# aweisberg/cassandra-accord

Hardware: AMD Instinct MI355X
Metric: txn-key conflict pairs resolved/sec (node) (higher is better)
Workload: dtype u32/u64 (integer); 1 GPU; config2: KeyDeps batch, 1M txns x 8 keys, zipf(0.99) over 1M keys, p_write 0.5, uncommitted window 10k, per-GPU CommandStore snapshot; key_distribution=zipf, keys_permuted=True, n_txn_per_gpu=1000000, pairs_per_gpu=8000000, dep_edges_per_gpu=35349420, parallelism=keyspace shards x1 (independent CommandStores)

## Files before the change

### cassandra-accord_amd/csrc/api.hip

```cpp
#include "dict.hpp"
#include <exception>
#include <thread>

namespace acc {
void keydeps_batch(acc_ctx *ctx, const acc_batch_in *in, acc_keydeps_view *view);
void keydeps_mixed(acc_ctx *ctx, const acc_range_batch_in *in, acc_keydeps_view *view, SharedDict *shared = nullptr);
void keydeps_merge(acc_ctx *ctx, const acc_merge_in *in, acc_merge_view *view);
void levelise(acc_ctx *ctx, const acc_graph_in *in, uint32_t *level, uint32_t *order, uint32_t *n_levels);
void rangedeps_batch(acc_ctx *ctx, const acc_range_batch_in *in, acc_rangedeps_view *view, const SharedDict *shared = nullptr);
void shard_pack(acc_ctx *ctx, const acc_batch_in *in, acc_frag_streams *out, bool ctx_alloc);
void shard_merge(acc_ctx *ctx, const acc_frag_recv *in, acc_merge_view *view);
void deps_merge(acc_ctx *ctx, const acc_deps_merge_in *in, acc_deps_merge_view *view);
void rmm_invert(acc_ctx *ctx, const acc_rmm_batch *in, acc_csr_view *out);
void rmm_slice(acc_ctx *ctx, const acc_rmm_batch *in, const acc_ranges_in *select, acc_slice_view *out);
void rangedeps_stab(acc_ctx *ctx, const acc_rmm_batch *rd, const acc_stab_in *q, acc_stab_view *out);
void rmm_without(acc_ctx *ctx, const acc_rmm_batch *in, const acc_ts_cols *txn, const acc_txn_sets *set_a,
                 const acc_txn_sets *set_b, acc_without_view *out);
void recovery_deps_reduce(acc_ctx *ctx, const acc_deps_merge_in *cw, const acc_deps_merge_in *anw, acc_recovery_deps_view *view);
void map_reduce_full(acc_ctx *ctx, const acc_batch_in *in, const acc_recovery_in *q, acc_keydeps_view *view);
void map_reduce_full_ranges(acc_ctx *ctx, const acc_range_cmds_in *c, const acc_recovery_ranges_in *q, acc_rangedeps_view *view);
void latest_deps_merge(acc_ctx *ctx, const acc_latest_in *in, acc_latest_view *view);
void deps_from_json(acc_ctx *ctx, const acc_json_in *in, acc_json_deps_view *view);
void deps_to_json(acc_ctx *ctx, const acc_json_out_in *in, acc_json_out *out);
void cfk_update(acc_ctx *ctx, acc_cfk *cfk, const acc_batch_in *in);
void cfk_apply(acc_ctx *ctx, const acc_cfk_snap *in, const acc_cfk_updates *up, acc_cfk_snap_view *view);
void cfk_snap_to_batch(acc_ctx *ctx, const acc_cfk_snap *in, acc_cfk_batch_view *view, bool trusted = false);
void max_conflicts(acc_ctx *ctx, const acc_conflicts_in *u, const acc_preaccept_in *q, acc_preaccept_out *out);
acc_maxconflicts *mc_new(int device, uint32_t end_inclusive);
void mc_free(acc_maxconflicts *m);
uint64_t mc_size(const acc_maxconflicts *m);
void mc_update(acc_ctx *ctx, acc_maxconflicts *m, const acc_conflicts_in *u);
void mc_get(acc_ctx *ctx, const acc_maxconflicts *m, const acc_preaccept_in *q, acc_preaccept_out *out);
void cfk_view(acc_cfk *cfk, acc_batch_in *out);
void cfk_apply_deps(acc_ctx *ctx, acc_cfk *cfk, const acc_cfk_updates *up);
void cfk_state(acc_cfk *cfk, acc_cfk_snap *out);
void cfk_missing(acc_cfk *cfk, acc_cfk_batch_view *out);
void cfk_free(acc_cfk *cfk);
void cfk_keydeps(acc_ctx *ctx, acc_cfk *cfk, const acc_cfk_queries *q, acc_keydeps_view *view);
acc_cfk *cfk_new(int device);
}

namespace {
int ctx_create(int device, const acc_opts *opts, acc_ctx **out_ctx);
void ctx_destroy(acc_ctx *ctx);
}

extern "C" {

const char *acc_version(void) { return "accord_amd 0.1 (gfx950)"; }

int acc_create(int device, const acc_opts *opts, acc_ctx **out_ctx) { return ctx_create(device, opts, out_ctx); }

void acc_destroy(acc_ctx *ctx) { ctx_destroy(ctx); }

}

namespace {

int ctx_create(int device, const acc_opts *opts, acc_ctx **out_ctx)
{
    if (!out_ctx) return ACC_E_ARG;
    *out_ctx = nullptr;
    acc_ctx *ctx = new (std::nothrow) acc_ctx();
    if (!ctx) return ACC_E_NOMEM;
    int rc = acc_guard(ctx, [&] {
        int count = 0;
        ACC_HIP(hipGetDeviceCount(&count));
        if (device < 0 || device >= count) acc::fail(ACC_E_ARG, "no such HIP device");
        ACC_HIP(hipSetDevice(device));
        ctx->device = device;
        if (opts) ctx->opts = *opts;
        ctx->flags = ctx->opts.flags;
        ACC_HIP(hipStreamCreateWithFlags(&ctx->stream, hipStreamNonBlocking));
        ACC_HIP(hipHostMalloc((void **)&ctx->pinned, acc_ctx::PINNED_WORDS * sizeof(uint64_t), hipHostMallocDefault));
    });
    if (rc != ACC_OK) {
        ctx_destroy(ctx);
        return rc;
    }
    *out_ctx = ctx;
    return ACC_OK;
}

void ctx_destroy(acc_ctx *ctx)
{
    if (!ctx) return;
    (void)hipSetDevice(ctx->device);
    if (ctx->stream) (void)hipStreamSynchronize(ctx->stream);
    for (auto &kv : ctx->bufs)
        if (kv.second.ptr) (void)hipFree(kv.second.ptr);
    for (void *p : ctx->graveyard) (void)hipFree(p);
    for (auto &p : ctx->pending) { (void)hipEventDestroy(p.start); (void)hipEventDestroy(p.stop); }
    for (auto e : ctx->event_pool) (void)hipEventDestroy(e);
    for (int i = 0; i < acc_ctx::NAUX; ++i) {
        if (ctx->aux[i]) { (void)hipStreamSynchronize(ctx->aux[i]); (void)hipStreamDestroy(ctx->aux[i]); }
        if (ctx->join_ev[i]) (void)hipEventDestroy(ctx->join_ev[i]);
    }
    if (ctx->fork_ev) (void)hipEventDestroy(ctx->fork_ev);
    if (ctx->pinned) (void)hipHostFree(ctx->pinned);
    if (ctx->stream) (void)hipStreamDestroy(ctx->stream);
    acc_ctx *child = ctx->child;
    delete ctx;
    ctx_destroy(child);
}

}

extern "C" {

const char *acc_last_error(const acc_ctx *ctx) { return ctx ? ctx->last_error.c_str() : "null context"; }

int acc_sync(acc_ctx *ctx)
{
    if (!ctx) return ACC_E_ARG;
    return acc_guard(ctx, [&] { ctx->sync(); });
}

void *acc_stream(acc_ctx *ctx) { return ctx ? (void *)ctx->stream : nullptr; }

int acc_keydeps_batch(acc_ctx *ctx, const acc_batch_in *in, acc_keydeps_view *out_view)
{
    if (!ctx) return ACC_E_ARG;
    return acc_guard(ctx, [&] {
        ACC_HIP(hipSetDevice(ctx->device));
        acc::keydeps_batch(ctx, in, out_view);
    });
}

int acc_keydeps_mixed(acc_ctx *ctx, const acc_range_batch_in *in, acc_keydeps_view *out_view)
{
    if (!ctx) return ACC_E_ARG;
    return acc_guard(ctx, [&] {
        ACC_HIP(hipSetDevice(ctx->device));
        acc::keydeps_mixed(ctx, in, out_view);
    });
}

int acc_map_reduce_full(acc_ctx *ctx, const acc_batch_in *snapshot, const acc_recovery_in *q, acc_keydeps_view *out_view)
{
    if (!ctx) return ACC_E_ARG;
    return acc_guard(ctx, [&] {
        ACC_HIP(hipSetDevice(ctx->device));
        acc::map_reduce_full(ctx, snapshot, q, out_view);
    });
}

int acc_map_reduce_full_ranges(acc_ctx *ctx, const acc_range_cmds_in *cmds, const acc_recovery_ranges_in *q,
                               acc_rangedeps_view *out_view)
{
    if (!ctx) return ACC_E_ARG;
    return acc_guard(ctx, [&] {
        ACC_HIP(hipSetDevice(ctx->device));
        acc::map_reduce_full_ranges(ctx, cmds, q, out_view);
    });
}

int acc_latest_deps_merge(acc_ctx *ctx, const acc_latest_in *in, acc_latest_view *out_view)
{
    if (!ctx) return ACC_E_ARG;
    return acc_guard(ctx, [&] {
        ACC_HIP(hipSetDevice(ctx->device));
        acc::latest_deps_merge(ctx, in, out_view);
    });
}

int acc_partial_deps_batch(acc_ctx *ctx, const acc_range_batch_in *in, acc_keydeps_view *key_view,
                           acc_rangedeps_view *range_view)
{
    if (!ctx) return ACC_E_ARG;
    return acc_guard(ctx, [&] {
        ACC_HIP(hipSetDevice(ctx->device));
        if (!key_view || !range_view) acc::fail(ACC_E_ARG, "null argument");
        const bool serial = (ctx->flags & ACC_OPT_PD_SERIAL) != 0;
        if (!ctx->child && !serial) {
            const acc_opts o = ctx->opts;
            const int rc = ctx_create(ctx->device, &o, &ctx->child);
            if (rc != ACC_OK) acc::fail(rc, "cannot create the RangeDeps half's context");
        }
        acc_ctx *const child = serial ? nullptr : ctx->child;
        acc::SharedDict sd;
        std::thread th;
        int rrc = ACC_OK;
        hipEvent_t ev = nullptr;
        struct Join {
            std::thread &t;
            hipEvent_t &e;
            ~Join() { if (t.joinable()) t.join(); if (e) (void)hipEventDestroy(e); }
        } join{ th, ev };
        if (child) {
            child->opts = ctx->opts;
            child->flags = ctx->flags;
            child->time_only = ctx->time_only;
            sd.ready = [&](const acc::SharedDict &d) {
                ACC_HIP(hipEventCreateWithFlags(&ev, hipEventDisableTiming));
                ACC_HIP(hipEventRecord(ev, ctx->stream));
                th = std::thread([&rrc, child, in, range_view, ev, d] {
                    rrc = acc_guard(child, [&] {
                        ACC_HIP(hipSetDevice(child->device));
                        ACC_HIP(hipStreamWaitEvent(child->stream, ev, 0));
                        acc::rangedeps_batch(child, in, range_view, &d);
                        child->sync();
                    });
                });
            };
        }
        acc::keydeps_mixed(ctx, in, key_view, &sd);
        if (th.joinable()) {
            th.join();
            if (rrc != ACC_OK) acc::fail(rrc, child->last_error.c_str());
            ctx->rd_view = child->rd_view;
            ctx->rd_valid = child->rd_valid;
            ctx->rd_ent_hint = child->rd_ent_hint;
            for (const auto &kv : child->stats) ctx->stat(kv.first.c_str(), kv.second);
            for (auto &sl : child->slots) {
                if (!sl.launches) continue;
                acc::TimingSlot &d = ctx->slots[ctx->slot(sl.name.c_str())];
                d.total_ms += sl.total_ms;
                d.launches += sl.launches;
                sl.total_ms = 0;
                sl.launches = 0;
            }
        } else {
            acc::rangedeps_batch(ctx, in, range_view, &sd);
        }
        ctx->kd_valid = true;
    });
}

int acc_deps_from_json(acc_ctx *ctx, const acc_json_in *in, acc_json_deps_view *out_view)
{
    if (!ctx) return ACC_E_ARG;
    return acc_guard(ctx, [&] {
        ACC_HIP(hipSetDevice(ctx->device));
        acc::deps_from_json(ctx, in, out_view);
    });
}

int acc_deps_to_json(acc_ctx *ctx, const acc_json_out_in *in, acc_json_out *out)
{
    if (!ctx) return ACC_E_ARG;
    return acc_guard(ctx, [&] {
        ACC_HIP(hipSetDevice(ctx->device));
        acc::deps_to_json(ctx, in, out);
    });
}

int acc_cfk_create(acc_ctx *ctx, acc_cfk **out)
{
    if (!ctx || !out) return ACC_E_ARG;
    *out = nullptr;
    return acc_guard(ctx, [&] { *out = acc::cfk_new(ctx->device); });
// ... 398 lines not shown
```

### cassandra-accord_amd/csrc/ctx.hpp

```cpp
#pragma once

#include <hip/hip_runtime.h>

#include <cstdint>
#include <cstdio>
#include <cstring>
#include <string>
#include <unordered_map>
#include <vector>

#include "../../include/accord_amd.h"

namespace acc {

struct Error {
    int code;
    std::string msg;
};

[[noreturn]] inline void fail(int code, const std::string &msg) { throw Error{code, msg}; }

#define ACC_HIP(expr)                                                                          \
    do {                                                                                       \
        hipError_t e_ = (expr);                                                                \
        if (e_ != hipSuccess)                                                                  \
            ::acc::fail(e_ == hipErrorOutOfMemory ? ACC_E_NOMEM : ACC_E_DEVICE,                \
                        std::string(#expr ": ") + hipGetErrorString(e_));                      \
    } while (0)

struct Buf {
    void *ptr = nullptr;
    size_t bytes = 0;
};

struct TimingSlot {
    std::string name;
    double total_ms = 0;
    uint64_t launches = 0;
};

struct PendingEvent {
    int slot;
    hipEvent_t start, stop;
};

}

struct acc_ctx {
    int device = 0;
    hipStream_t stream = nullptr;
    static constexpr int NAUX = 3;
    hipStream_t aux[NAUX] = {};
    hipEvent_t fork_ev = nullptr, join_ev[NAUX] = {};
    hipStream_t launch_stream = nullptr;
    size_t scan_cap = 0, scan_dirty[2] = {0, 0};
    int scan_par = 0;
    struct OsState {
        size_t cap = 0, dirty[2] = {0, 0};
        int par = 0;
    };
    std::unordered_map<std::string, OsState> os_state;
    uint32_t flags = 0;
    acc_opts opts{};
    std::string last_error;
    acc_ctx *child = nullptr;
    std::unordered_map<std::string, acc::Buf> bufs;
    std::vector<void *> graveyard;
    static constexpr size_t PINNED_WORDS = 1024, PINNED_SLOTS = 512;
    uint64_t *pinned = nullptr;
    std::vector<acc::TimingSlot> slots;
    std::unordered_map<std::string, int> slot_index;
    std::vector<acc::PendingEvent> pending;
    std::vector<hipEvent_t> event_pool;
    std::vector<std::string> time_only;
    bool timed(const char *name) const
    {
        if (!(flags & ACC_OPT_TIMING)) return false;
        if (time_only.empty()) return true;
        for (const auto &t : time_only)
            if (t == name) return true;
        return false;
    }
    std::vector<std::pair<std::string, uint64_t>> stats;
    void stat(const char *name, uint64_t value)
    {
        for (auto &kv : stats)
            if (kv.first == name) { kv.second = value; return; }
        stats.emplace_back(name, value);
    }
    acc_keydeps_view kd_view{};
    acc_merge_view merge_view{};
    acc_rangedeps_view rd_view{};
    acc_deps_merge_view dm_view{};
    bool dm_valid = false;
    uint64_t rd_ent_hint = 0;
    bool rd_valid = false;
    bool kd_valid = false;
    bool merge_valid = false;
    std::vector<uint64_t> latest_suff_off, latest_suff_s, latest_suff_e;

    std::string ns;

    template <class T>
    T *get(const char *name, size_t count)
    {
        return get_raw<T>(ns.empty() ? std::string(name) : ns + name, count);
    }
    template <class T>
    T *get_raw(const std::string &name, size_t count)
    {
        size_t bytes = count * sizeof(T);
        if (bytes == 0) bytes = 16;
        acc::Buf &b = bufs[name];
        if (b.bytes < bytes) {
            if (b.ptr) graveyard.push_back(b.ptr);
            b.ptr = nullptr;
            size_t want = bytes + (bytes < (4ull << 30) ? bytes / 2 : bytes / 8);
            ACC_HIP(hipMalloc(&b.ptr, want));
            b.bytes = want;
        }
        return static_cast<T *>(b.ptr);
    }

    void swap_buf(const char *name, void *&ptr, size_t &bytes)
    {
        acc::Buf &b = bufs[ns.empty() ? std::string(name) : ns + name];
        std::swap(b.ptr, ptr);
        std::swap(b.bytes, bytes);
    }

    const void *buf_ptr(const char *name) const
    {
        auto it = bufs.find(ns.empty() ? std::string(name) : ns + name);
        return it == bufs.end() ? nullptr : it->second.ptr;
    }

    hipEvent_t take_event()
    {
        if (!event_pool.empty()) {
            hipEvent_t e = event_pool.back();
            event_pool.pop_back();
            return e;
        }
        hipEvent_t e;
        ACC_HIP(hipEventCreate(&e));
        return e;
    }

    int slot(const char *name)
    {
        auto it = slot_index.find(name);
        if (it != slot_index.end()) return it->second;
        int i = (int)slots.size();
        slots.push_back({name, 0, 0});
        slot_index[name] = i;
        return i;
    }

    void resolve_timing()
    {
        for (auto &p : pending) {
            float ms = 0;
            ACC_HIP(hipEventElapsedTime(&ms, p.start, p.stop));
            slots[p.slot].total_ms += ms;
            slots[p.slot].launches += 1;
            event_pool.push_back(p.start);
            event_pool.push_back(p.stop);
        }
        pending.clear();
    }

    hipStream_t cur() const { return launch_stream ? launch_stream : stream; }

    void fork(int k)
    {
        if (!fork_ev) {
            ACC_HIP(hipEventCreateWithFlags(&fork_ev, hipEventDisableTiming));
            for (int i = 0; i < NAUX; ++i) {
                ACC_HIP(hipStreamCreateWithFlags(&aux[i], hipStreamNonBlocking));
                ACC_HIP(hipEventCreateWithFlags(&join_ev[i], hipEventDisableTiming));
            }
        }
        ACC_HIP(hipEventRecord(fork_ev, stream));
        for (int i = 0; i < k; ++i) ACC_HIP(hipStreamWaitEvent(aux[i], fork_ev, 0));
    }
    void join(int k)
    {
        for (int i = 0; i < k; ++i) {
            ACC_HIP(hipEventRecord(join_ev[i], aux[i]));
            ACC_HIP(hipStreamWaitEvent(stream, join_ev[i], 0));
        }
        launch_stream = nullptr;
    }

    void recover() noexcept
    {
        launch_stream = nullptr;
        for (int i = 0; i < NAUX; ++i)
            if (aux[i]) (void)hipStreamSynchronize(aux[i]);
        if (stream) (void)hipStreamSynchronize(stream);
    }

    void sync()
    {
        ACC_HIP(hipStreamSynchronize(stream));
        for (void *p : graveyard) ACC_HIP(hipFree(p));
        graveyard.clear();
        if (!pending.empty()) resolve_timing();
    }
};

namespace acc {

struct NsScope {
    acc_ctx *ctx;
    std::string saved;
    NsScope(acc_ctx *c, const char *prefix) : ctx(c), saved(c->ns) { ctx->ns = saved + prefix; }
    ~NsScope() { ctx->ns = saved; }
};

template <class K, class... Args>
inline void launch(acc_ctx *ctx, const char *name, K kernel, dim3 grid, dim3 block, size_t shmem, Args... args)
{
    if (grid.x == 0 || grid.y == 0 || grid.z == 0) return;
    PendingEvent pe{};
    const bool timed = ctx->timed(name);
    if (timed) {
        pe.slot = ctx->slot(name);
        pe.start = ctx->take_event();
        pe.stop = ctx->take_event();
        ACC_HIP(hipEventRecord(pe.start, ctx->cur()));
    }
    hipLaunchKernelGGL(kernel, grid, block, shmem, ctx->cur(), args...);
    ACC_HIP(hipGetLastError());
    if (timed) {
        ACC_HIP(hipEventRecord(pe.stop, ctx->cur()));
        ctx->pending.push_back(pe);
    }
}

inline unsigned grid_for(size_t n, unsigned per_block)
{
    size_t g = (n + per_block - 1) / per_block;
    return (unsigned)(g ? g : 1);
}

template <class T>
inline const T *stage_in(acc_ctx *ctx, const char *name, const T *src, size_t count, uint32_t mem)
{
    if (count == 0) return ctx->get<T>(name, 1);
    if (!src) fail(ACC_E_ARG, std::string("null input array: ") + name);
    if (mem == ACC_MEM_DEVICE) return src;
    T *d = ctx->get<T>(name, count);
    ACC_HIP(hipMemcpyAsync(d, src, count * sizeof(T), hipMemcpyHostToDevice, ctx->stream));
    return d;
}

}

template <class F>
inline int acc_guard(acc_ctx *ctx, F &&body)
{
    try {
        body();
        if (ctx) ctx->last_error.clear();
        return ACC_OK;
    } catch (const acc::Error &e) {
        if (ctx) { ctx->recover(); ctx->last_error = e.msg; }
        return e.code;
    } catch (const std::bad_alloc &) {
        if (ctx) { ctx->recover(); ctx->last_error = "host allocation failed"; }
        return ACC_E_NOMEM;
    } catch (...) {
        if (ctx) { ctx->recover(); ctx->last_error = "unknown failure"; }
        return ACC_E_STATE;
    }
}
```

### cassandra-accord_amd/csrc/dict.hpp

```cpp
#pragma once

#include "prims.hpp"
#include "ts.hpp"
#include <functional>

namespace acc {

struct Dictionary {
    uint32_t *rank = nullptr;
    uint32_t *txn_of_rank = nullptr;
    int rbits = 0;
    bool batch_sorted = false;
    bool fast = false;
    bool ties_pending = false;
    uint64_t hg[8] = {};
};

struct DenseRank {
    uint32_t *rank = nullptr;
    uint32_t *first = nullptr;
    const uint32_t *perm = nullptr;
    uint64_t *count_dev = nullptr;
    uint64_t count = 0;
};
DenseRank dense_rank(acc_ctx *ctx, const char *tag, size_t n, int nw, const uint64_t *const *words, const uint64_t *and_mask,
                     const uint64_t *xor_mask, bool want_first);

constexpr size_t PREP_G_WORDS = 8 + 64 * 8;
void prep_dictionary(acc_ctx *ctx, uint32_t n, size_t P, const uint64_t *tm, const uint64_t *tl, const int32_t *tn,
                     const uint64_t *em, const uint64_t *el, const int32_t *en, const uint8_t *status,
                     const uint32_t *key_off, const uint64_t *key_code, uint32_t *owner, uint64_t *g, Dictionary &out,
                     bool defer_ties = false);
void redo_general_dictionary(acc_ctx *ctx, uint32_t n, const uint64_t *tm, const uint64_t *tl, const int32_t *tn,
                             const uint64_t *em, const uint64_t *el, const int32_t *en, uint64_t *g, Dictionary &d);

enum : uint32_t {
    ERR_BAD_STATUS = 1u << 0,
    ERR_BAD_KIND = 1u << 1,
    ERR_LOCAL_ONLY = 1u << 2,
    ERR_KEYS_UNSORTED = 1u << 3,
    ERR_DUP_TXNID = 1u << 4,
    ERR_KEY_OFF = 1u << 5,
    ERR_KEY_TOTAL = 1u << 6,
};
void check_errors(uint64_t errs);

struct SharedDict {
    bool valid = false;
    Dictionary dict;
    const uint32_t *owner = nullptr;
    std::function<void(const SharedDict &)> ready;
};

}
```

### cassandra-accord_amd/csrc/dictionary.hip

```cpp
#include "dict.hpp"

namespace acc {

namespace {

constexpr int DMAXW = 3;

struct DWords {
    const uint64_t *w[DMAXW];
    uint64_t xor_mask[DMAXW];
    uint64_t and_mask[DMAXW];
};

__device__ __forceinline__ uint64_t dword(const DWords &d, int k, size_t i)
{
    return (d.w[k][i] & d.and_mask[k]) ^ d.xor_mask[k];
}

__global__ __launch_bounds__(BLOCK) void k_dict_masks(size_t n, DWords d, int nw, uint64_t *__restrict__ g)
{
    uint64_t m[DMAXW] = { 0, 0, 0 };
    uint64_t ref[DMAXW];
    for (int k = 0; k < nw; ++k) ref[k] = dword(d, k, 0);
    for (size_t i = (size_t)blockIdx.x * BLOCK + threadIdx.x; i < n; i += (size_t)gridDim.x * BLOCK)
// ... 6 lines not shown
        if (lane_id() == 0) part[threadIdx.x >> 6][k] = x;
    }
    __syncthreads();
    if (threadIdx.x < (unsigned)nw) {
        uint64_t x = 0;
        for (int q = 0; q < WAVES; ++q) x |= part[q][threadIdx.x];
        if (x) atomicOr((unsigned long long *)&g[threadIdx.x], (unsigned long long)x);
    }
}

struct DPlan {
    Runs r[DMAXW];
    int shift[DMAXW];
};

__global__ __launch_bounds__(BLOCK) void k_dict_compact(size_t n, DWords d, int nw, DPlan p, int sel, const uint32_t *__restrict__ perm,
                                                        uint64_t *__restrict__ out)
{
    const size_t i = (size_t)blockIdx.x * BLOCK + threadIdx.x;
    if (i >= n) return;
    const size_t src = perm ? perm[i] : i;
    if (sel >= 0) { out[i] = pext_runs(dword(d, sel, src), p.r[sel]); return; }
    uint64_t c = 0;
    for (int k = 0; k < nw; ++k)
        if (p.r[k].bits) c |= pext_runs(dword(d, k, src), p.r[k]) << p.shift[k];
    out[i] = c;
}

__global__ __launch_bounds__(BLOCK) void k_dict_flags(size_t n, const uint64_t *__restrict__ sorted_single, const uint32_t *__restrict__ perm,
                                                      DWords d, int nw, uint32_t *__restrict__ flag)
{
    const size_t i = (size_t)blockIdx.x * BLOCK + threadIdx.x;
    if (i >= n) return;
    uint32_t f = 1;
    if (i > 0) {
        if (sorted_single) f = sorted_single[i] != sorted_single[i - 1];
        else {
            const uint32_t a = perm[i], b = perm[i - 1];
            f = 0;
            for (int k = 0; k < nw; ++k) f |= dword(d, k, a) != dword(d, k, b);
        }
    }
    flag[i] = f;
}

__global__ __launch_bounds__(BLOCK) void k_dict_scatter(size_t n, const uint32_t *__restrict__ perm, const uint32_t *__restrict__ flag,
                                                        const uint32_t *__restrict__ incl, uint32_t *__restrict__ rank,
                                                        uint32_t *__restrict__ first, uint64_t *__restrict__ count)
{
    const size_t i = (size_t)blockIdx.x * BLOCK + threadIdx.x;
    if (i >= n) return;
    const uint32_t src = perm[i], r = incl[i] - 1;
    rank[src] = r;
    if (first && flag[i]) first[r] = src;
    if (i == n - 1) *count = incl[i];
}

}

DenseRank dense_rank(acc_ctx *ctx, const char *tag, size_t n, int nw, const uint64_t *const *words, const uint64_t *and_mask,
                     const uint64_t *xor_mask, bool want_first)
{
    if (nw < 1 || nw > DMAXW) fail(ACC_E_STATE, "internal: dense_rank supports 1..3 words");
    if (n >= 0xFFFFFFFFull) fail(ACC_E_CAP, "dictionary too large (>= 2^32 keys)");
    hipStream_t st = ctx->stream;
    char nm[64];
    auto name = [&](const char *s) { snprintf(nm, sizeof nm, "%s.%s", tag, s); return nm; };
    DenseRank out;
    out.rank = ctx->get<uint32_t>(name("rank"), n);
    out.first = want_first ? ctx->get<uint32_t>(name("first"), n) : nullptr;
    out.count_dev = ctx->get<uint64_t>(name("count"), 1);
    if (n == 0) {
        ACC_HIP(hipMemsetAsync(out.count_dev, 0, 8, st));
        out.count = 0;
        return out;
    }
    DWords d{};
    for (int k = 0; k < DMAXW; ++k) {
        d.w[k] = k < nw ? words[k] : nullptr;
        d.and_mask[k] = (k < nw && and_mask) ? and_mask[k] : ~0ull;
        d.xor_mask[k] = (k < nw && xor_mask) ? xor_mask[k] : 0ull;
    }
    uint64_t *g = ctx->get<uint64_t>(name("masks"), DMAXW);
    ACC_HIP(hipMemsetAsync(g, 0, DMAXW * 8, st));
    launch(ctx, "dict_masks", k_dict_masks, dim3(std::min<unsigned>(grid_for(n, BLOCK), 1024u)), dim3(BLOCK), 0, n, d, nw, g);
    ACC_HIP(hipMemcpyAsync(ctx->pinned + 32, g, DMAXW * 8, hipMemcpyDeviceToHost, st));
    ctx->sync();
    DPlan p{};
    int total = 0;
    for (int k = nw - 1; k >= 0; --k) {
        p.r[k] = make_runs(ctx->pinned[32 + k]);
        p.shift[k] = total;
        total += p.r[k].bits;
    }
    const unsigned gn = grid_for(n, BLOCK);
    uint32_t *flag = ctx->get<uint32_t>(name("flag"), n);
    uint32_t *incl = ctx->get<uint32_t>(name("incl"), n);
    const uint32_t *perm;
    if (total <= 64) {
        uint64_t *ck = ctx->get<uint64_t>(name("ckey"), n);
        launch(ctx, "dict_compact", k_dict_compact, dim3(gn), dim3(BLOCK), 0, n, d, nw, p, -1, (const uint32_t *)nullptr, ck);
        Sorted s = radix_sort(ctx, name("rs"), ck, nullptr, n, total);
        perm = s.vals;
        launch(ctx, "dict_flags", k_dict_flags, dim3(gn), dim3(BLOCK), 0, n, (const uint64_t *)s.keys, (const uint32_t *)nullptr,
               d, nw, flag);
    } else {
        uint64_t *wk = ctx->get<uint64_t>(name("wkey"), n);
        uint32_t *pb = ctx->get<uint32_t>(name("perm"), n);
        const uint32_t *cur = nullptr;
        for (int k = nw - 1; k >= 0; --k) {
            if (!p.r[k].bits) continue;
            launch(ctx, "dict_compact", k_dict_compact, dim3(gn), dim3(BLOCK), 0, n, d, nw, p, k, cur, wk);
            Sorted s = radix_sort(ctx, name("rs"), wk, cur, n, p.r[k].bits);
            ACC_HIP(hipMemcpyAsync(pb, s.vals, n * sizeof(uint32_t), hipMemcpyDeviceToDevice, st));
            cur = pb;
        }
        perm = cur;
        launch(ctx, "dict_flags", k_dict_flags, dim3(gn), dim3(BLOCK), 0, n, (const uint64_t *)nullptr, perm, d, nw, flag);
    }
    scan<uint32_t, OpAdd<uint32_t>>(ctx, flag, incl, n, false);
    launch(ctx, "dict_scatter", k_dict_scatter, dim3(gn), dim3(BLOCK), 0, n, perm, (const uint32_t *)flag, (const uint32_t *)incl,
           out.rank, out.first, out.count_dev);
    out.count = ~0ull;
    out.perm = perm;
    return out;
}


struct TsPlan {
    Runs r0, r1, r2;
    int b0, b1, b2;
};

template <int NW>
__device__ __forceinline__ void block_or_n(uint64_t (&v)[NW], uint64_t *dst)
{
    __shared__ uint64_t part[WAVES][NW];
#pragma unroll
    for (int w = 0; w < NW; ++w) {
        uint64_t x = v[w];
#pragma unroll
        for (int d = 32; d >= 1; d >>= 1) x |= shfl_idx(x, (int)(lane_id() ^ d));
        if (lane_id() == 0) part[threadIdx.x >> 6][w] = x;
    }
    __syncthreads();
    if (threadIdx.x < NW) {
        uint64_t x = 0;
#pragma unroll
        for (int q = 0; q < WAVES; ++q) x |= part[q][threadIdx.x];
        if (x) atomicOr((unsigned long long *)&dst[threadIdx.x], (unsigned long long)x);
    }
}

constexpr uint32_t PREP_SLOTS = 64;

__global__ __launch_bounds__(BLOCK) void k_prep_txn(uint32_t n, size_t P, const uint64_t *__restrict__ tm, const uint64_t *__restrict__ tl,
                                                    const int32_t *__restrict__ tn, const uint64_t *__restrict__ em,
                                                    const uint64_t *__restrict__ el, const int32_t *__restrict__ en,
                                                    const uint8_t *__restrict__ status, const uint32_t *__restrict__ key_off,
                                                    const uint64_t *__restrict__ key_code, uint32_t *__restrict__ owner,
                                                    uint32_t *__restrict__ bflag, uint64_t *__restrict__ g)
{
    __shared__ uint32_t ko[BLOCK + 1];
    const uint32_t tid = threadIdx.x;
    uint64_t m0 = 0, m1 = 0, m2 = 0, km = 0, errs = 0, unsorted = 0, ornk = 0;
    uint32_t differs = 0;
    const uint64_t r0 = tm[0], r1 = ts_w1(tl[0]), r2 = ts_w2(tn[0]);
    const uint64_t kref = P ? key_code[0] : 0;
    if (blockIdx.x == 0 && tid == 0 && key_off[n] != P) errs |= ERR_KEY_TOTAL;
    for (uint32_t t0 = blockIdx.x * BLOCK; t0 < n; t0 += gridDim.x * BLOCK) {
        const uint32_t t = t0 + tid;
        const uint32_t tcnt = min((uint32_t)BLOCK, n - t0);
        __syncthreads();
        if (tid < tcnt) ko[tid] = key_off[t];
        if (tid == 0) ko[tcnt] = key_off[t0 + tcnt];
        if (t < n) {
            const bool d = tm[t] != em[t] || ts_w1(tl[t]) != ts_w1(el[t]) || tn[t] != en[t];
            differs += d;
            bflag[t] = (uint32_t)d;
            m0 |= (tm[t] ^ r0) | (em[t] ^ r0);
            m1 |= (ts_w1(tl[t]) ^ r1) | (ts_w1(el[t]) ^ r1);
            m2 |= (ts_w2(tn[t]) ^ r2) | (ts_w2(en[t]) ^ r2);
            if (status[t] > 7) errs |= ERR_BAD_STATUS;
            uint32_t kind = (uint32_t)(tl[t] >> 1) & 7u;
            if (kind >= 6) errs |= ERR_BAD_KIND;
            else if (kind == 5) errs |= ERR_LOCAL_ONLY;
            if (t + 1 < n && ts_cmp(tm[t], tl[t], tn[t], tm[t + 1], tl[t + 1], tn[t + 1]) >= 0) unsorted = 1;
        }
        __syncthreads();
        const bool bad = tid < tcnt && ko[tid + 1] < ko[tid];
        if (bad) errs |= ERR_KEY_OFF;
        else if (tid < tcnt) ornk |= ko[tid + 1] - ko[tid];
        if (!__syncthreads_or(bad ? 1 : 0) && P) {
            const uint32_t a = (uint32_t)min((size_t)ko[0], P), b = (uint32_t)min((size_t)ko[tcnt], P);
            for (uint32_t j = a + tid; j < b; j += BLOCK) {
                uint32_t lo = 0, hi = tcnt;
                while (hi - lo > 1) { const uint32_t m = (lo + hi) >> 1; if (ko[m] <= j) lo = m; else hi = m; }
                owner[j] = t0 + lo;
                const uint64_t kc = key_code[j];
                km |= kc ^ kref;
                if (j > ko[lo] && key_code[j - 1] >= kc) errs |= ERR_KEYS_UNSORTED;
            }
        }
    }
    uint64_t *gs = g + 8 * (blockIdx.x % PREP_SLOTS);
    uint64_t v[7] = { m0, m1, m2, km, errs, unsorted, ornk };
    block_or_n<7>(v, gs);
    __shared__ uint32_t s_nd;
    if (tid == 0) s_nd = 0;
    __syncthreads();
    if (differs) atomicAdd(&s_nd, differs);
    __syncthreads();
    if (tid == 0 && s_nd) atomicAdd((unsigned long long *)&gs[7], (unsigned long long)s_nd);
}

__global__ __launch_bounds__(BLOCK) void k_b_compact(uint32_t n, const uint32_t *__restrict__ bflag, const uint32_t *__restrict__ bidx,
                                                     const uint64_t *__restrict__ em, const uint64_t *__restrict__ el,
                                                     const int32_t *__restrict__ en, const uint64_t *__restrict__ tm,
                                                     const uint64_t *__restrict__ tl, const int32_t *__restrict__ tn,
                                                     TsPlan plan, uint64_t *__restrict__ bkey, uint32_t *__restrict__ bsrc,
                                                     uint64_t *__restrict__ tkey)
{
    uint32_t t = blockIdx.x * BLOCK + threadIdx.x;
    if (t >= n) return;
    uint64_t c0 = pext_runs(tm[t], plan.r0), c1 = pext_runs(ts_w1(tl[t]), plan.r1), c2 = pext_runs(ts_w2(tn[t]), plan.r2);
    tkey[t] = (plan.b0 ? (c0 << (plan.b1 + plan.b2)) : 0) | (plan.b1 ? (c1 << plan.b2) : 0) | c2;
    if (bflag[t]) {
        c0 = pext_runs(em[t], plan.r0); c1 = pext_runs(ts_w1(el[t]), plan.r1); c2 = pext_runs(ts_w2(en[t]), plan.r2);
        uint32_t b = bidx[t];
        bkey[b] = (plan.b0 ? (c0 << (plan.b1 + plan.b2)) : 0) | (plan.b1 ? (c1 << plan.b2) : 0) | c2;
        bsrc[b] = t;
    }
}

__device__ __forceinline__ uint32_t lower_bound_u64(const uint64_t *a, uint32_t lo, uint32_t hi, uint64_t v)
{
    while (lo < hi) {
        uint32_t mid = (lo + hi) >> 1;
        if (a[mid] < v) lo = mid + 1; else hi = mid;
    }
    return lo;
}

__global__ __launch_bounds__(BLOCK) void k_rank_txn_sorted(uint32_t n, uint32_t nb, const uint64_t *__restrict__ tkey,
                                                           const uint64_t *__restrict__ sb, const uint32_t *__restrict__ bflag,
                                                           uint32_t *__restrict__ rank, uint32_t *__restrict__ txn_of_rank,
                                                           uint64_t *__restrict__ g)
{
    uint32_t t = blockIdx.x * BLOCK + threadIdx.x;
    uint64_t tie = 0;
    if (t < n) {
        uint32_t lb = lower_bound_u64(sb, 0, nb, tkey[t]);
        if (lb < nb && sb[lb] == tkey[t]) tie = 1;
        uint32_t r = t + lb;
        rank[t] = r;
        txn_of_rank[r] = t;
        if (!bflag[t]) rank[n + t] = r;
    }
    uint64_t v[1] = { tie };
    block_or_n<1>(v, g + 6);
}

__global__ __launch_bounds__(BLOCK) void k_rank_b_sorted(uint32_t n, uint32_t nb, const uint64_t *__restrict__ tkey,
                                                         const uint64_t *__restrict__ sb, const uint32_t *__restrict__ sperm,
                                                         const uint32_t *__restrict__ bsrc, uint32_t *__restrict__ rank,
                                                         uint64_t *__restrict__ g)
{
    uint32_t k = blockIdx.x * BLOCK + threadIdx.x;
    uint64_t tie = 0;
    if (k < nb) {
        if (k > 0 && sb[k] == sb[k - 1]) tie = 1;
        uint32_t t = bsrc[sperm[k]];
        rank[n + t] = k + lower_bound_u64(tkey, 0, n, sb[k]);
    }
    uint64_t v[1] = { tie };
    block_or_n<1>(v, g + 6);
}


__global__ __launch_bounds__(BLOCK) void k_ts_compact(uint32_t n, const uint64_t *__restrict__ tm, const uint64_t *__restrict__ tl,
                                                      const int32_t *__restrict__ tn, const uint64_t *__restrict__ em,
                                                      const uint64_t *__restrict__ el, const int32_t *__restrict__ en,
                                                      TsPlan plan, int word_sel, const uint32_t *__restrict__ perm,
                                                      uint64_t *__restrict__ out)
{
    size_t i = (size_t)blockIdx.x * BLOCK + threadIdx.x;
    if (i >= 2 * (size_t)n) return;
    size_t src = perm ? perm[i] : i;
    uint32_t t = (uint32_t)(src < n ? src : src - n);
    bool is_exec = src >= n;
    uint64_t w0 = is_exec ? em[t] : tm[t];
    uint64_t w1 = ts_w1(is_exec ? el[t] : tl[t]);
    uint64_t w2 = ts_w2(is_exec ? en[t] : tn[t]);
    uint64_t c0 = pext_runs(w0, plan.r0), c1 = pext_runs(w1, plan.r1), c2 = pext_runs(w2, plan.r2);
    uint64_t k;
    if (word_sel < 0) k = (plan.b0 ? (c0 << (plan.b1 + plan.b2)) : 0) | (plan.b1 ? (c1 << plan.b2) : 0) | c2;
    else k = word_sel == 0 ? c0 : word_sel == 1 ? c1 : c2;
    out[i] = k;
}

__global__ __launch_bounds__(BLOCK) void k_rank_flags(size_t m, const uint32_t *__restrict__ perm, const uint64_t *__restrict__ c0,
                                                      const uint64_t *__restrict__ c1, const uint64_t *__restrict__ c2,
                                                      const uint64_t *__restrict__ sorted_single, uint32_t *__restrict__ flag)
{
    size_t i = (size_t)blockIdx.x * BLOCK + threadIdx.x;
    if (i >= m) return;
    uint32_t f = 1;
    if (i > 0) {
        if (sorted_single) f = sorted_single[i] != sorted_single[i - 1];
        else {
            uint32_t a = perm[i], b = perm[i - 1];
            f = (c0[a] != c0[b]) || (c1[a] != c1[b]) || (c2[a] != c2[b]);
        }
    }
    flag[i] = f;
}

__global__ __launch_bounds__(BLOCK) void k_rank_scatter(size_t m, uint32_t n, const uint32_t *__restrict__ perm,
                                                        const uint32_t *__restrict__ incl, uint32_t *__restrict__ rank,
                                                        uint32_t *__restrict__ txn_of_rank)
{
    size_t i = (size_t)blockIdx.x * BLOCK + threadIdx.x;
    if (i >= m) return;
    uint32_t src = perm[i];
    uint32_t r = incl[i] - 1;
    rank[src] = r;
    if (src < n) txn_of_rank[r] = src;
}

__global__ __launch_bounds__(BLOCK) void k_dup_txn(uint32_t n, const uint32_t *__restrict__ rank, uint32_t *__restrict__ seen,
                                                   uint64_t *__restrict__ g)
{
    uint32_t t = blockIdx.x * BLOCK + threadIdx.x;
    uint64_t err = 0;
    if (t < n) {
        if (atomicAdd(&seen[rank[t]], 1u) != 0) err = ERR_DUP_TXNID;
    }
    uint64_t v[1] = { err };
    block_or_n<1>(v, g + 4);
}

__global__ __launch_bounds__(BLOCK) void k_exec_ties(uint32_t n, const uint32_t *__restrict__ rank, uint32_t *__restrict__ seen,
                                                     uint64_t *__restrict__ g)
{
    uint32_t t = blockIdx.x * BLOCK + threadIdx.x;
    uint64_t tie = 0;
    if (t < n && rank[n + t] != rank[t]) {
        if (atomicAdd(&seen[rank[n + t]], 1u) != 0) tie = 1;
    }
    uint64_t v[1] = { tie };
    block_or_n<1>(v, g + 6);
}


void check_errors(uint64_t errs)
{
    if (errs & ERR_KEY_TOTAL) fail(ACC_E_ARG, "key_off[n_txn] must equal n_pairs");
    if (errs & ERR_BAD_STATUS) fail(ACC_E_ARG, "invalid InternalStatus ordinal (> INVALID_OR_TRUNCATED)");
    if (errs & ERR_BAD_KIND) fail(ACC_E_ARG, "Kind.ofOrdinal: invalid kind ordinal in TxnId flags");
    if (errs & ERR_KEY_OFF) fail(ACC_E_ARG, "key_off must be non-decreasing");
    if (errs & ERR_KEYS_UNSORTED) fail(ACC_E_ARG, "keys of a txn must be sorted and unique (Keys.ofSortedUnique)");
    if (errs & ERR_DUP_TXNID) fail(ACC_E_ARG, "TxnIds of a batch must be distinct (CommandsForKey txns are sorted unique)");
    if (errs & ERR_LOCAL_ONLY) fail(ACC_E_STATE, "Kind.witnesses(): unhandled kind LocalOnly (AssertionError)");
}

static void general_ranks(acc_ctx *ctx, uint32_t n, const uint64_t *tm, const uint64_t *tl, const int32_t *tn,
                          const uint64_t *em, const uint64_t *el, const int32_t *en, const TsPlan &plan, uint64_t *g,
                          uint32_t *rank, uint32_t *txn_of_rank)
{
    hipStream_t st = ctx->stream;
    const size_t m = 2 * (size_t)n;
    uint32_t *flag = ctx->get<uint32_t>("rank_flag", m);
    uint32_t *incl = ctx->get<uint32_t>("rank_incl", m);
    const unsigned gm = grid_for(m, BLOCK);
    Sorted ts_sorted;
    if (plan.b0 + plan.b1 + plan.b2 <= 64) {
        uint64_t *ck = ctx->get<uint64_t>("ts_ckey", m);
        launch(ctx, "ts_compact", k_ts_compact, dim3(gm), dim3(BLOCK), 0, n, tm, tl, tn, em, el, en, plan, -1,
               (const uint32_t *)nullptr, ck);
        ts_sorted = radix_sort(ctx, "rs_ts", ck, nullptr, m, plan.b0 + plan.b1 + plan.b2);
        launch(ctx, "rank_flags", k_rank_flags, dim3(gm), dim3(BLOCK), 0, m, (const uint32_t *)ts_sorted.vals,
               (const uint64_t *)nullptr, (const uint64_t *)nullptr, (const uint64_t *)nullptr,
               (const uint64_t *)ts_sorted.keys, flag);
    } else {
        uint64_t *c[3] = { ctx->get<uint64_t>("ts_c0", m), ctx->get<uint64_t>("ts_c1", m), ctx->get<uint64_t>("ts_c2", m) };
        for (int w = 0; w < 3; ++w)
            launch(ctx, "ts_compact", k_ts_compact, dim3(gm), dim3(BLOCK), 0, n, tm, tl, tn, em, el, en, plan, w,
                   (const uint32_t *)nullptr, c[w]);
        uint64_t *tmpk = ctx->get<uint64_t>("ts_tmpk", m);
        uint32_t *permb = ctx->get<uint32_t>("ts_perm", m);
        const uint32_t *perm = nullptr;
        const int wbits[3] = { plan.b0, plan.b1, plan.b2 };
        for (int w = 2; w >= 0; --w) {
            const uint64_t *keys = c[w];
            if (perm) {
                launch(ctx, "ts_compact", k_ts_compact, dim3(gm), dim3(BLOCK), 0, n, tm, tl, tn, em, el, en, plan, w,
                       perm, tmpk);
                keys = tmpk;
            }
            Sorted s = radix_sort(ctx, "rs_ts", keys, perm, m, wbits[w]);
            ACC_HIP(hipMemcpyAsync(permb, s.vals, m * sizeof(uint32_t), hipMemcpyDeviceToDevice, st));
            perm = permb;
        }
        ts_sorted = { nullptr, permb };
        launch(ctx, "rank_flags", k_rank_flags, dim3(gm), dim3(BLOCK), 0, m, (const uint32_t *)permb,
               (const uint64_t *)c[0], (const uint64_t *)c[1], (const uint64_t *)c[2], (const uint64_t *)nullptr, flag);
    }
    scan<uint32_t, OpAdd<uint32_t>>(ctx, flag, incl, m, false);
    launch(ctx, "rank_scatter", k_rank_scatter, dim3(gm), dim3(BLOCK), 0, m, n, (const uint32_t *)ts_sorted.vals,
           (const uint32_t *)incl, rank, txn_of_rank);
    uint32_t *seen = ctx->get<uint32_t>("dup_seen", m);
    ACC_HIP(hipMemsetAsync(seen, 0, m * sizeof(uint32_t), st));
    launch(ctx, "dup_txn", k_dup_txn, dim3(grid_for(n, BLOCK)), dim3(BLOCK), 0, n, (const uint32_t *)rank, seen, g);
    launch(ctx, "exec_ties", k_exec_ties, dim3(grid_for(n, BLOCK)), dim3(BLOCK), 0, n, (const uint32_t *)rank, seen, g);
}

static TsPlan ts_plan(const uint64_t *hg)
{
    TsPlan plan;
    plan.r0 = make_runs(hg[0]); plan.r1 = make_runs(hg[1]); plan.r2 = make_runs(hg[2]);
    plan.b0 = plan.r0.bits; plan.b1 = plan.r1.bits; plan.b2 = plan.r2.bits;
    return plan;
}

void redo_general_dictionary(acc_ctx *ctx, uint32_t n, const uint64_t *tm, const uint64_t *tl, const int32_t *tn,
                             const uint64_t *em, const uint64_t *el, const int32_t *en, uint64_t *g, Dictionary &d)
{
    ACC_HIP(hipMemsetAsync(g + 6, 0, sizeof(uint64_t), ctx->stream));
    general_ranks(ctx, n, tm, tl, tn, em, el, en, ts_plan(d.hg), g, d.rank, d.txn_of_rank);
    d.fast = false;
    d.ties_pending = false;
    ctx->stat("keydeps.fast_dictionary", 0);
}

void prep_dictionary(acc_ctx *ctx, uint32_t n, size_t P, const uint64_t *tm, const uint64_t *tl, const int32_t *tn,
                     const uint64_t *em, const uint64_t *el, const int32_t *en, const uint8_t *status,
                     const uint32_t *key_off, const uint64_t *key_code, uint32_t *owner, uint64_t *g, Dictionary &out,
                     bool defer_ties)
{
    hipStream_t st = ctx->stream;
    static_assert(8 * PREP_SLOTS <= acc_ctx::PINNED_WORDS - acc_ctx::PINNED_SLOTS, "slot rows fit the pinned area");
    static_assert(PREP_G_WORDS == 8 + 8 * PREP_SLOTS, "g and the prep slots share one buffer");
    uint64_t *gslots = g + 8;
    ACC_HIP(hipMemsetAsync(g, 0, PREP_G_WORDS * sizeof(uint64_t), st));
    uint32_t *bflag = ctx->get<uint32_t>("bflag", n);
    launch(ctx, "prep_txn", k_prep_txn, dim3(grid_for(n, BLOCK)), dim3(BLOCK), 0, n, P, tm, tl, tn, em, el, en, status,
           key_off, key_code, owner, bflag, gslots);
    uint64_t hg[8] = { 0, 0, 0, 0, 0, 0, 0, 0 };
    {
        uint64_t *hs = ctx->pinned + acc_ctx::PINNED_SLOTS;
        ACC_HIP(hipMemcpyAsync(hs, gslots, 8 * PREP_SLOTS * sizeof(uint64_t), hipMemcpyDeviceToHost, st));
        ctx->sync();
        for (uint32_t r = 0; r < PREP_SLOTS; ++r) {
            for (int w = 0; w < 7; ++w) hg[w] |= hs[8 * r + w];
            hg[7] += hs[8 * r + 7];
        }
    }
    check_errors(hg[4]);
    const bool batch_sorted = hg[5] == 0;

    const TsPlan plan = ts_plan(hg);
    const size_t m = 2 * (size_t)n;
    uint32_t *rank = ctx->get<uint32_t>("rank", m);
    uint32_t *txn_of_rank = ctx->get<uint32_t>("txn_of_rank", m);
    const uint64_t nb = hg[7];
    bool fast_dict = batch_sorted && plan.b0 + plan.b1 + plan.b2 <= 64 && nb < n;
    out.ties_pending = false;
    if (fast_dict) {
        uint32_t *bidx = ctx->get<uint32_t>("bidx", (size_t)n + 1);
        scan<uint32_t, OpAdd<uint32_t>>(ctx, bflag, bidx, n, true, bidx + n);
        uint64_t *bkey = ctx->get<uint64_t>("bkey", nb);
        uint32_t *bsrc = ctx->get<uint32_t>("bsrc", nb);
        uint64_t *tkey = ctx->get<uint64_t>("tkey", n);
        launch(ctx, "b_compact", k_b_compact, dim3(grid_for(n, BLOCK)), dim3(BLOCK), 0, n, (const uint32_t *)bflag,
               (const uint32_t *)bidx, em, el, en, tm, tl, tn, plan, bkey, bsrc, tkey);
        Sorted sb = radix_sort(ctx, "rs_b", bkey, nullptr, nb, plan.b0 + plan.b1 + plan.b2);
        launch(ctx, "rank_txn_sorted", k_rank_txn_sorted, dim3(grid_for(n, BLOCK)), dim3(BLOCK), 0, n, (uint32_t)nb,
               (const uint64_t *)tkey, (const uint64_t *)sb.keys, (const uint32_t *)bflag, rank, txn_of_rank, g);
        launch(ctx, "rank_b_sorted", k_rank_b_sorted, dim3(grid_for(nb, BLOCK)), dim3(BLOCK), 0, n, (uint32_t)nb,
               (const uint64_t *)tkey, (const uint64_t *)sb.keys, (const uint32_t *)sb.vals, (const uint32_t *)bsrc, rank, g);
        if (defer_ties) {
            out.ties_pending = true;
        } else {
            ACC_HIP(hipMemcpyAsync(ctx->pinned, g + 6, sizeof(uint64_t), hipMemcpyDeviceToHost, st));
            ctx->sync();
            if (ctx->pinned[0]) {
                ACC_HIP(hipMemsetAsync(g + 6, 0, sizeof(uint64_t), st));
                fast_dict = false;
            }
        }
    }
    if (!fast_dict) general_ranks(ctx, n, tm, tl, tn, em, el, en, plan, g, rank, txn_of_rank);
    ctx->stat("keydeps.fast_dictionary", fast_dict ? 1 : 0);
    out.rank = rank;
    out.txn_of_rank = txn_of_rank;
    out.rbits = bits_for(m - 1);
    out.batch_sorted = batch_sorted;
    out.fast = fast_dict;
    memcpy(out.hg, hg, sizeof hg);
}

}
```

### cassandra-accord_amd/csrc/keydeps.hip

```cpp
#include "keydeps.hpp"

#include <vector>

namespace acc {


struct TxnInfoArgs {
    uint32_t n = 0;
    const uint8_t *status = nullptr;
    const uint64_t *tl = nullptr;
    uint4 *tinfo = nullptr;
    uint32_t *bigflag = nullptr;
};

__device__ __forceinline__ void txn_info_one(uint32_t t, uint32_t n, const uint32_t *rank, const uint8_t *status,
                                             const uint64_t *tl, const uint32_t *key_off, uint4 *tinfo, uint32_t *bigflag)
{
    if (bigflag) bigflag[t] = 0;
    const uint32_t kind = (uint32_t)(tl[t] >> 1) & 7u;
    tinfo[t] = make_uint4(rank[t], rank[n + t], (uint32_t)status[t] | (kind << 3), key_off[t]);
}

__global__ __launch_bounds__(BLOCK) void k_pair_keys(size_t P, const uint64_t *__restrict__ key_code,
                                                     const uint32_t *__restrict__ owner, const uint32_t *__restrict__ key_off,
                                                     const uint32_t *__restrict__ rank,
                                                     const uint32_t *__restrict__ perm, PairPlan plan,
                                                     int rank_only, uint64_t *__restrict__ out, TxnInfoArgs ti)
{
    size_t i = (size_t)blockIdx.x * BLOCK + threadIdx.x;
    if (ti.tinfo && i < ti.n) txn_info_one((uint32_t)i, ti.n, rank, ti.status, ti.tl, key_off, ti.tinfo, ti.bigflag);
    if (i >= P) return;
    size_t j = perm ? perm[i] : i;
    if (rank_only) { out[i] = rank[owner[j]]; return; }
    uint64_t kc = pext_runs(key_code[j], plan.rk);
    if (plan.mode == 4) {
        const uint32_t t = owner[j];
        out[i] = (kc << 32) | ((uint64_t)t << plan.sb) | (uint64_t)(j - key_off[t]);
        return;
    }
    out[i] = plan.mode == 1 ? ((kc << plan.rbits) | rank[owner[j]]) : plan.mode == 3 ? ((kc << 32) | i) : kc;
}

__global__ __launch_bounds__(BLOCK) void k_seg_flags_packed(size_t P, const uint64_t *__restrict__ sp, uint32_t *__restrict__ flag,
                                                            uint32_t *__restrict__ perm, int sb, const uint32_t *__restrict__ key_off,
                                                            uint32_t *__restrict__ pown)
{
    size_t p = (size_t)blockIdx.x * BLOCK + threadIdx.x;
    if (p >= P) return;
    const uint64_t x = sp[p];
    flag[p] = p == 0 || (x >> 32) != (sp[p - 1] >> 32);
    if (sb < 0) { perm[p] = (uint32_t)x; return; }
    const uint32_t t = (uint32_t)x >> sb, slot = (uint32_t)x & ((1u << sb) - 1u);
    perm[p] = key_off[t] + slot;
    pown[p] = t;
}

__global__ __launch_bounds__(BLOCK) void k_seg_flags(size_t P, const uint64_t *__restrict__ skeys, int key_shift,
                                                     uint32_t *__restrict__ flag)
{
    size_t p = (size_t)blockIdx.x * BLOCK + threadIdx.x;
    if (p >= P) return;
    flag[p] = p == 0 || (skeys[p] >> key_shift) != (skeys[p - 1] >> key_shift);
}

__global__ __launch_bounds__(BLOCK) void k_txn_info(uint32_t n, const uint32_t *__restrict__ rank, const uint8_t *__restrict__ status,
                                                    const uint64_t *__restrict__ tl, const uint32_t *__restrict__ key_off,
                                                    uint4 *__restrict__ tinfo, uint32_t *__restrict__ bigflag)
{
    uint32_t t = blockIdx.x * BLOCK + threadIdx.x;
    if (t < n) txn_info_one(t, n, rank, status, tl, key_off, tinfo, bigflag);
}

__global__ __launch_bounds__(BLOCK) void k_pair_tinfo(size_t P, const uint32_t *__restrict__ owner, const uint4 *__restrict__ tinfo,
                                                      uint4 *__restrict__ ptinfo)
{
    size_t j = (size_t)blockIdx.x * BLOCK + threadIdx.x;
    if (j < P) ptinfo[j] = tinfo[owner[j]];
}

__global__ __launch_bounds__(BLOCK) void k_pair_pos(size_t P, const uint32_t *__restrict__ perm, uint32_t *__restrict__ pair_pos)
{
    size_t p = (size_t)blockIdx.x * BLOCK + threadIdx.x;
    if (p < P) pair_pos[perm[p]] = (uint32_t)p;
}


constexpr int NLIST = 6;
constexpr int NCNT = 9;
constexpr int NRD = 8;
__device__ __forceinline__ bool cnt_is_max(int q) { return q == 7; }

__device__ __forceinline__ uint32_t kind_class(uint32_t kind)
{
    return kind == 0 ? 0u : kind == 1 ? 1u : (kind == 3 || kind == 4) ? 2u : 3u;
}
__device__ __forceinline__ uint32_t wk_classes(uint32_t wk)
{
    return (wk & 1u) | (((wk >> 1) & 1u) << 1) | (((wk >> 3) & 1u) << 2);
}

__device__ __forceinline__ uint32_t v2_code(uint32_t rank, uint32_t exec, uint32_t info)
{
    uint32_t st = info & 7u, kind = info >> 3, cls = kind_class(kind);
    bool u = st >= 1 && st <= 3, c = st >= 4 && st <= 6;
    uint32_t list = cls < 3 ? (u ? cls : c ? 3 + cls : 7u) : 7u;
    uint32_t bc = (c && cls < 3 && exec != rank) ? 1u : 0u;
    uint32_t ucw = (c && kind == 1 && exec == rank) ? 1u : 0u;
    return list | (bc << 3) | (ucw << 4);
}

constexpr int V2_ITEMS = 4;
constexpr int V2_TILE = BLOCK * V2_ITEMS;

__device__ __forceinline__ void v2_codes4(size_t P, size_t base, const uint32_t *__restrict__ s_rank, const uint32_t *__restrict__ s_exec,
                                          const uint8_t *__restrict__ s_info, uint32_t (&code)[V2_ITEMS], uint32_t (&rk)[V2_ITEMS],
                                          uint32_t &bqm)
{
    uint4 r = *reinterpret_cast<const uint4 *>(s_rank + base);
    uint4 e = *reinterpret_cast<const uint4 *>(s_exec + base);
    uint32_t inf = *reinterpret_cast<const uint32_t *>(s_info + base);
    rk[0] = r.x; rk[1] = r.y; rk[2] = r.z; rk[3] = r.w;
    const uint32_t ex[4] = { e.x, e.y, e.z, e.w };
    bqm = 0;
#pragma unroll
    for (int i = 0; i < V2_ITEMS; ++i) {
        code[i] = base + i < P ? v2_code(rk[i], ex[i], (inf >> (8 * i)) & 0xFFu) : 7u;
        bqm |= (base + i < P && ex[i] != rk[i] ? 1u : 0u) << i;
    }
}

__global__ __launch_bounds__(BLOCK) void k_cfk_gather4(size_t P, uint32_t *__restrict__ perm, const uint4 *__restrict__ ptinfo,
                                                       const uint64_t *__restrict__ sp, int sb, const uint4 *__restrict__ tinfo,
                                                       uint32_t *__restrict__ seg_flag, uint32_t *__restrict__ s_rank,
                                                       uint32_t *__restrict__ s_exec, uint8_t *__restrict__ s_info,
                                                       uint32_t *__restrict__ pair_pos, uint32_t *__restrict__ tile_sums,
                                                       uint32_t ntiles)
{
    __shared__ uint32_t lds[WAVES];
    const size_t base = (size_t)blockIdx.x * V2_TILE + (size_t)threadIdx.x * V2_ITEMS;
    uint32_t c[NCNT] = {};
    if (base < P) {
        uint32_t j[V2_ITEMS], fl[V2_ITEMS];
        uint4 ti[V2_ITEMS];
        if (sp) {
            uint64_t x[V2_ITEMS];
            const uint64_t xp = base > 0 ? sp[base - 1] : 0;
#pragma unroll
            for (int i = 0; i < V2_ITEMS; ++i) x[i] = base + i < P ? sp[base + i] : 0;
            const uint32_t smask = (1u << sb) - 1u;
#pragma unroll
            for (int i = 0; i < V2_ITEMS; ++i) {
                const bool in = base + i < P;
                const uint64_t prev = i == 0 ? xp : x[i - 1];
                fl[i] = in && (base + i == 0 || (x[i] >> 32) != (prev >> 32)) ? 1u : 0u;
                ti[i] = in ? tinfo[(uint32_t)x[i] >> sb] : make_uint4(0u, 0u, 0u, 0u);
            }
#pragma unroll
            for (int i = 0; i < V2_ITEMS; ++i) j[i] = ti[i].w + ((uint32_t)x[i] & smask);
            if (base + V2_ITEMS <= P) {
                *reinterpret_cast<uint4 *>(seg_flag + base) = make_uint4(fl[0], fl[1], fl[2], fl[3]);
                *reinterpret_cast<uint4 *>(perm + base) = make_uint4(j[0], j[1], j[2], j[3]);
            } else {
#pragma unroll
                for (int i = 0; i < V2_ITEMS; ++i)
                    if (base + i < P) { seg_flag[base + i] = fl[i]; perm[base + i] = j[i]; }
            }
        } else {
#pragma unroll
            for (int i = 0; i < V2_ITEMS; ++i) {
                const bool in = base + i < P;
                j[i] = in ? perm[base + i] : 0u;
                fl[i] = in ? seg_flag[base + i] : 0u;
            }
#pragma unroll
            for (int i = 0; i < V2_ITEMS; ++i) ti[i] = base + i < P ? ptinfo[j[i]] : make_uint4(0u, 0u, 0u, 0u);
        }
        uint32_t inf = 0;
#pragma unroll
        for (int i = 0; i < V2_ITEMS; ++i) {
            const size_t p = base + i;
            if (p >= P) break;
            if (pair_pos) pair_pos[j[i]] = (uint32_t)p;
            c[8] += fl[i] != 0;
            inf |= (ti[i].z & 0xFFu) << (8 * i);
            const uint32_t code = v2_code(ti[i].x, ti[i].y, ti[i].z & 0xFFu);
            const uint32_t l = code & 7u;
#pragma unroll
            for (int q = 0; q < NLIST; ++q) c[q] += l == (uint32_t)q;
            c[6] += (code >> 3) & 1u;
            if ((code >> 4) & 1u) c[7] = (uint32_t)p + 1;
        }
        *reinterpret_cast<uint4 *>(s_rank + base) = make_uint4(ti[0].x, ti[1].x, ti[2].x, ti[3].x);
        *reinterpret_cast<uint4 *>(s_exec + base) = make_uint4(ti[0].y, ti[1].y, ti[2].y, ti[3].y);
        *reinterpret_cast<uint32_t *>(s_info + base) = inf;
    }
#pragma unroll
    for (int q = 0; q < NCNT; ++q) {
        uint32_t total;
        if (!cnt_is_max(q)) block_exclusive(c[q], OpAdd<uint32_t>(), lds, total);
        else block_exclusive(c[q], OpMax<uint32_t>(), lds, total);
        if (threadIdx.x == 0) tile_sums[(size_t)q * ntiles + blockIdx.x] = total;
    }
}

constexpr int RW_CBC = 6, RW_LUCW = 7;
constexpr uint32_t RD_W = 32;

__global__ __launch_bounds__(BLOCK) void k_v2_apply(size_t P, const uint32_t *__restrict__ s_rank, const uint32_t *__restrict__ s_exec,
                                                    const uint8_t *__restrict__ s_info, const uint32_t *__restrict__ seg_flag,
                                                    const uint32_t *__restrict__ tile_pref, const uint32_t *__restrict__ totals,
                                                    uint32_t ntiles, int rbits, V2Cols o, uint32_t *__restrict__ seg_incl,
                                                    uint32_t *__restrict__ seg_start, const uint32_t *__restrict__ perm,
                                                    const uint64_t *__restrict__ key_code, uint64_t *__restrict__ seg_key,
                                                    const uint64_t *__restrict__ sp, Runs krun, uint64_t rk_mask,
                                                    uint32_t *__restrict__ bases, uint64_t *__restrict__ z0, uint32_t nz0,
                                                    uint64_t *__restrict__ z1, uint32_t nz1, const uint64_t *__restrict__ g,
                                                    uint64_t *__restrict__ stage)
{
    __shared__ uint32_t lds[WAVES];
    if (blockIdx.x == 0) {
        if (threadIdx.x == 0) {
            uint32_t b = 0;
            for (int l = 0; l < NLIST; ++l) { bases[l] = b; b += totals[l]; }
            bases[NLIST] = b;
        }
        for (uint32_t i = threadIdx.x; i < nz0; i += BLOCK) z0[i] = 0;
        for (uint32_t i = threadIdx.x; i < nz1; i += BLOCK) z1[i] = 0;
        if (threadIdx.x < 3) stage[threadIdx.x] = g[4 + threadIdx.x];
    }
    const size_t base = (size_t)blockIdx.x * V2_TILE + (size_t)threadIdx.x * V2_ITEMS;
    uint32_t code[V2_ITEMS] = { 7u, 7u, 7u, 7u }, rk[V2_ITEMS] = {};
    uint32_t c[NCNT] = {};
    uint32_t fl[V2_ITEMS] = {};
    uint64_t kc[V2_ITEMS] = {};
    uint32_t bqm = 0;
    if (base < P) {
        v2_codes4(P, base, s_rank, s_exec, s_info, code, rk, bqm);
#pragma unroll
        for (int i = 0; i < V2_ITEMS; ++i) {
            uint32_t l = code[i] & 7u;
#pragma unroll
            for (int q = 0; q < NLIST; ++q) c[q] += l == (uint32_t)q;
            c[6] += (code[i] >> 3) & 1u;
            if ((code[i] >> 4) & 1u) c[7] = (uint32_t)(base + i) + 1;
            fl[i] = base + i < P ? seg_flag[base + i] : 0u;
            c[8] += fl[i] != 0;
        }
        if (seg_key && sp) {
            const uint64_t kconst = key_code[0] & ~rk_mask;
#pragma unroll
            for (int i = 0; i < V2_ITEMS; ++i)
                if (fl[i]) {
                    const uint64_t c = sp[base + i] >> 32;
                    uint64_t w = kconst;
                    for (int r = 0; r < krun.n; ++r) {
                        const uint64_t m = krun.len[r] >= 64 ? ~0ull : ((1ull << krun.len[r]) - 1);
                        w |= ((c >> krun.dst[r]) & m) << krun.lo[r];
                    }
                    kc[i] = w;
                }
        } else if (seg_key) {
            uint32_t pi[V2_ITEMS] = {};
            if (base + V2_ITEMS <= P) {
                const uint4 pv = *reinterpret_cast<const uint4 *>(perm + base);
                pi[0] = pv.x; pi[1] = pv.y; pi[2] = pv.z; pi[3] = pv.w;
            } else {
                for (int i = 0; i < V2_ITEMS; ++i) if (base + i < P) pi[i] = perm[base + i];
            }
#pragma unroll
            for (int i = 0; i < V2_ITEMS; ++i) if (fl[i]) kc[i] = key_code[pi[i]];
        }
    }
    uint32_t run[NCNT];
#pragma unroll
    for (int q = 0; q < NCNT; ++q) {
        uint32_t total;
        uint32_t pre = tile_pref[(size_t)q * ntiles + blockIdx.x];
        if (!cnt_is_max(q)) run[q] = pre + block_exclusive(c[q], OpAdd<uint32_t>(), lds, total);
        else { uint32_t e = block_exclusive(c[q], OpMax<uint32_t>(), lds, total); run[q] = e > pre ? e : pre; }
    }
    static_assert(RD_W == 8 * V2_ITEMS, "eight threads per directory chunk");
    {
        uint32_t pl[NRD] = {};
#pragma unroll
        for (int i = 0; i < V2_ITEMS; ++i) {
            const uint32_t l = code[i] & 7u;
#pragma unroll
            for (int q = 0; q < NLIST; ++q) pl[q] |= (l == (uint32_t)q ? 1u : 0u) << i;
            pl[6] |= ((code[i] >> 3) & 1u) << i;
            pl[7] |= ((code[i] >> 4) & 1u) << i;
        }
        const uint32_t sh = V2_ITEMS * (threadIdx.x & 7u);
#pragma unroll
        for (int q = 0; q < NRD; ++q) {
            uint32_t x = pl[q] << sh;
            x |= __shfl_xor(x, 1, 64);
            x |= __shfl_xor(x, 2, 64);
            x |= __shfl_xor(x, 4, 64);
            pl[q] = x;
        }
        if ((threadIdx.x & 7u) == 0 && base < P) {
            uint4 *ch = o.rdir + 4 * (base / RD_W);
            ch[0] = make_uint4(run[0], run[1], run[2], run[3]);
            ch[1] = make_uint4(run[4], run[5], run[6], run[7]);
            ch[2] = make_uint4(pl[0], pl[1], pl[2], pl[3]);
            ch[3] = make_uint4(pl[4], pl[5], pl[6], pl[7]);
        }
    }
    if (base >= P) return;
    uint32_t lb[NLIST];
    {
        uint32_t b = 0;
#pragma unroll
        for (int l = 0; l < NLIST; ++l) { lb[l] = b; b += totals[l]; }
    }
    uint32_t segi[V2_ITEMS];
#pragma unroll
    for (int i = 0; i < V2_ITEMS; ++i) {
        const size_t p = base + i;
        if (p >= P) break;
        if (fl[i]) {
            seg_start[run[8]] = (uint32_t)p;
            if (seg_key) seg_key[run[8]] = kc[i];
        }
        run[8] += fl[i] != 0;
        segi[i] = run[8];
        if (p == P - 1) seg_start[run[8]] = (uint32_t)P;
    }
    if (base + V2_ITEMS <= P) *reinterpret_cast<uint4 *>(seg_incl + base) = make_uint4(segi[0], segi[1], segi[2], segi[3]);
    else for (int i = 0; i < V2_ITEMS; ++i) if (base + i < P) seg_incl[base + i] = segi[i];
#pragma unroll
    for (int i = 0; i < V2_ITEMS; ++i) {
        size_t p = base + i;
        if (p >= P) break;
        uint32_t l = code[i] & 7u;
        uint32_t r = rk[i];
        if (l < NLIST) {
            uint32_t idx = 0;
#pragma unroll
            for (int q = 0; q < NLIST; ++q) if ((uint32_t)q == l) idx = lb[q] + run[q];
            o.list_rank[idx] = r;
#pragma unroll
            for (int q = 0; q < NLIST; ++q) run[q] += (uint32_t)q == l;
        }
        if ((code[i] >> 3) & 1u) {
            uint32_t b = run[6]++;
            uint32_t seg = segi[i] - 1, e = s_exec[p];
            o.bc_rank[b] = r;
            o.bc_exec[b] = e;
            o.bc_kind[b] = (uint8_t)(s_info[p] >> 3);
            o.bc_pm_in[b] = ((uint64_t)seg << 32) | ((uint64_t)e + 1);
            o.bc_key[b] = ((uint64_t)seg << rbits) | e;
        }
        if ((code[i] >> 4) & 1u) run[7] = (uint32_t)p + 1;
        if (p == P - 1 && P % RD_W == 0) {
            uint4 *ch = o.rdir + 4 * (P / RD_W);
            ch[0] = make_uint4(run[0], run[1], run[2], run[3]);
            ch[1] = make_uint4(run[4], run[5], run[6], run[7]);
            ch[2] = make_uint4(0u, 0u, 0u, 0u);
            ch[3] = make_uint4(0u, 0u, 0u, 0u);
        }
    }
}

__global__ __launch_bounds__(BLOCK) void k_v2_bcs_cols(uint32_t nbc, const uint64_t *__restrict__ skeys, const uint32_t *__restrict__ svals,
                                                       const uint8_t *__restrict__ bc_kind, uint64_t rmask,
                                                       uint32_t *__restrict__ bcs_exec, uint64_t *__restrict__ lastw_in)
{
    uint32_t i = blockIdx.x * BLOCK + threadIdx.x;
    if (i >= nbc) return;
    bcs_exec[i] = (uint32_t)(skeys[i] & rmask);
    lastw_in[i] = bc_kind[svals[i]] == 1 ? i + 1 : 0;
}

__device__ __forceinline__ uint32_t rd_cbc(const uint4 *rdir, uint32_t p);

constexpr int V2TS_ITEMS = 32;
__global__ __launch_bounds__(BLOCK) void k_v2_tile_scans(const uint32_t *__restrict__ in, uint32_t *__restrict__ out, uint32_t nt,
                                                         uint32_t *__restrict__ totals)
{
    __shared__ uint32_t red[WAVES];
    const uint32_t q = blockIdx.x, tid = threadIdx.x;
    const bool mx = q == 7;
    const uint32_t *a = in + (size_t)q * nt;
    uint32_t *o = out + (size_t)q * nt;
    uint32_t carry = 0;
    for (uint32_t base = 0; base < nt; base += BLOCK * V2TS_ITEMS) {
        uint32_t v[V2TS_ITEMS];
        uint32_t acc = 0;
#pragma unroll
        for (int i = 0; i < V2TS_ITEMS; ++i) {
            const uint32_t idx = base + tid * V2TS_ITEMS + i;
            v[i] = idx < nt ? a[idx] : 0u;
            acc = mx ? max(acc, v[i]) : acc + v[i];
        }
        uint32_t tot;
        const uint32_t pre = mx ? block_exclusive(acc, OpMax<uint32_t>(), red, tot) : block_exclusive(acc, OpAdd<uint32_t>(), red, tot);
        uint32_t run = mx ? max(carry, pre) : carry + pre;
#pragma unroll
        for (int i = 0; i < V2TS_ITEMS; ++i) {
            const uint32_t idx = base + tid * V2TS_ITEMS + i;
            if (idx < nt) o[idx] = run;
            run = mx ? max(run, v[i]) : run + v[i];
        }
        carry = mx ? max(carry, tot) : carry + tot;
    }
    if (tid == 0) totals[q] = carry;
}

struct V2View {
    const uint32_t *perm, *pair_pos, *seg_incl, *seg_start, *s_rank, *s_exec;
    const uint8_t *s_info;
    const uint4 *rdir;
    const uint32_t *list_rank, *bases;
    const uint32_t *bc_rank, *bc_exec;
    const uint64_t *bc_pm;
    const uint8_t *bc_kind;
    const uint32_t *bcs_exec;
    const uint64_t *bcs_lastw;
    const uint4 *tinfo;
    const uint32_t *irec32;
    const uint4 *rec;
};

struct Row { uint32_t c[8]; };

__device__ __forceinline__ Row ld_row(const V2View &v, uint32_t p)
{
    const uint4 *ch = v.rdir + 4 * (size_t)(p / RD_W);
    const uint4 a = ch[0], b = ch[1], c = ch[2], d = ch[3];
    const uint32_t r = p % RD_W, mask = (1u << r) - 1u;
    Row o;
    o.c[0] = a.x + __popc(c.x & mask); o.c[1] = a.y + __popc(c.y & mask);
    o.c[2] = a.z + __popc(c.z & mask); o.c[3] = a.w + __popc(c.w & mask);
    o.c[4] = b.x + __popc(d.x & mask); o.c[5] = b.y + __popc(d.y & mask);
    o.c[6] = b.z + __popc(d.z & mask);
    const uint32_t w = d.w & mask;
    o.c[7] = w ? (p - r) + (31u - (uint32_t)__clz(w)) + 1u : b.w;
    return o;
}
__device__ __forceinline__ uint32_t rd_cbc(const uint4 *rdir, uint32_t p)
{
    const uint32_t *ch = reinterpret_cast<const uint32_t *>(rdir) + 16 * (size_t)(p / RD_W);
    const uint32_t r = p % RD_W;
    return ch[RW_CBC] + __popc(ch[8 + RW_CBC] & ((1u << r) - 1u));
}
__device__ __forceinline__ uint32_t ld_cbc(const V2View &v, uint32_t p) { return rd_cbc(v.rdir, p); }

struct V2Query {
    uint32_t trank, info, wk, wc, s0, pos, posm, m, bstart, bend;
    bool bq, has_m;
    Row r0, rp, rm;
};

__device__ __forceinline__ V2Query v2_query(const V2View &v, uint32_t p)
{
    V2Query q;
    const Row rpp = ld_row(v, p);
    const uint32_t seg = v.seg_incl[p] - 1;
    q.trank = v.s_rank[p];
    const uint32_t S = v.s_exec[p];
    q.info = v.s_info[p];
    q.s0 = v.seg_start[seg];
    const uint32_t s1 = v.seg_start[seg + 1];
    q.wk = witnesses(q.info >> 3);
    q.wc = wk_classes(q.wk);
    q.bq = S != q.trank;
    const uint32_t lu0 = rpp.c[RW_LUCW];
    const bool spec = !q.bq && lu0 > q.s0;
    q.r0 = ld_row(v, q.s0);
    const uint32_t b1 = ld_cbc(v, s1);
    uint32_t mu = 0;
    Row rms = q.r0;
    if (spec) { mu = v.s_rank[lu0 - 1]; rms = ld_row(v, lu0 - 1); }
    const uint32_t b0 = q.r0.c[RW_CBC];
    if (!q.bq && b1 == b0) {
        q.pos = p;
        q.rp = rpp;
        q.has_m = spec;
        q.m = mu;
        q.posm = spec ? lu0 - 1 : q.s0;
        q.rm = rms;
        q.bend = q.rm.c[RW_CBC];
        q.bstart = q.bend;
        return q;
    }
    q.pos = q.bq ? lower_bound_u32(v.s_rank, p + 1, s1, S) : p;
    q.rp = q.bq ? ld_row(v, q.pos) : rpp;
    const uint32_t lu = q.rp.c[RW_LUCW];
    const bool has_mu = lu > q.s0;
    if (q.bq) mu = has_mu ? v.s_rank[lu - 1] : 0;
    bool has_mb = false;
    uint32_t mb = 0;
    if (b1 > b0) {
        uint32_t i = lower_bound_u32(v.bcs_exec, b0, b1, S);
        if (i > b0) {
            uint32_t w = (uint32_t)v.bcs_lastw[i - 1];
            if (w > b0) { has_mb = true; mb = v.bcs_exec[w - 1]; }
        }
    }
    q.has_m = has_mu || has_mb;
    q.m = (has_mb && (!has_mu || mb > mu)) ? mb : mu;
    if (!q.has_m) q.posm = q.s0;
    else if (has_mu && q.m == mu) q.posm = lu - 1;
    else q.posm = lower_bound_u32(v.s_rank, q.s0, q.pos, q.m);
    q.rm = q.posm == q.s0 ? q.r0 : (spec && q.posm == lu0 - 1) ? rms : ld_row(v, q.posm);
    q.bend = q.rm.c[RW_CBC];
    q.bstart = q.has_m ? lower_bound_lo32(v.bc_pm, b0, q.bend, q.m + 1) : q.bend;
    return q;
}

constexpr uint32_t NO_M = 0xFFFFFFFFu;
constexpr uint32_t INLINE_M = 0xFFFFFFFEu;
constexpr uint32_t REC_INLINE = 15;
constexpr uint32_t IREC_W = 8;
constexpr uint32_t IREC_N = 7;
constexpr uint32_t REC_INLINE_FLAG = 0x80000000u;

__device__ __forceinline__ uint32_t inl_entry(const uint32_t *irec32, const uint4 *rec, uint32_t idx)
{
    const uint32_t j = idx >> 4, off = idx & 15u;
    return off < IREC_N ? irec32[IREC_W * (size_t)j + off] : reinterpret_cast<const uint32_t *>(rec)[16 * (size_t)j + off - IREC_N];
}

__device__ __forceinline__ void inl_put(uint32_t (&buf)[16], uint32_t &n, uint32_t x)
// ... 1488 lines not shown
                        const uint32_t l = i | jj;
                        const EntT xa = buf[i], ya = buf[l];
                        const bool up = (i & k) == 0;
                        if ((xa > ya) == up) { buf[i] = ya; buf[l] = xa; }
                    }
                }
                __builtin_amdgcn_wave_barrier();
                __builtin_amdgcn_fence(__ATOMIC_RELEASE, "wavefront");
            }
        }
    }
    __builtin_amdgcn_wave_barrier();
    __builtin_amdgcn_fence(__ATOMIC_RELEASE, "wavefront");
    ST_PH(4);
    uint32_t distinct = 0;
    if (ok && e != 0) stA[grp][(uint32_t)__popcll(nzb & lt)] = (uint16_t)(Kd + e_incl);
    for (uint32_t q0 = 0; q0 < wE; q0 += G) {
        const uint32_t q = q0 + sub;
        const bool in = ok && q < E;
        const EntT x = in ? buf[q] : (EntT)0;
        const EntT pv = (in && q > 0) ? buf[q - 1] : (EntT)0;
        const uint32_t kj = (uint32_t)(x & ((1u << KB) - 1u));
        const bool nw = in && (q == 0 || (x >> KB) != (pv >> KB));
        const uint64_t bal = __ballot(nw) & gmask;
        const uint32_t idx = distinct + (uint32_t)__popcll(bal & lt) + (nw ? 1u : 0u) - 1u;
        uint64_t peers = __ballot(in) & gmask;
#pragma unroll
        for (uint32_t bb = 0; bb < KB; ++bb) {
            const uint64_t m = __ballot((kj >> bb) & 1u);
            peers &= ((kj >> bb) & 1u) ? m : ~m;
        }
        const uint32_t before = (uint32_t)__popcll(peers & lt);
        if (in) {
            stA[grp][Kd + kbase[grp][kj] + kc[grp][kj] + before] = (uint16_t)idx;
            if (nw) s.dep_scr[(size_t)t * ST_SLOT + idx] = s.txn_of_rank[(uint32_t)(x >> KB)];
        }
        __builtin_amdgcn_wave_barrier();
        if (in && before == 0) kc[grp][kj] += (uint32_t)__popcll(peers);
        __builtin_amdgcn_wave_barrier();
        __builtin_amdgcn_fence(__ATOMIC_RELEASE, "wavefront");
        distinct += (uint32_t)__popcll(bal);
    }
    if (ok && sub == 0) s.u_cnt_out[t] = distinct;
    ST_PH(5);
    if (!valid) return;
    if (ok) {
        for (uint32_t q = sub; q < (uint32_t)A; q += G) s.arena[aoff + q] = (int32_t)stA[grp][q];
        if (e != 0) s.key_idx[koff + (uint32_t)__popcll(nzb & lt)] = sub;
    }
#ifdef ACC_PHASE_PROF
    ST_PH(6);
    if (lane == 0 && !LIST) {
        unsigned long long *row = g_st_prof + 8 * (size_t)tile;
        for (int i = 0; i < 6; ++i) row[i] = ph[i + 1] - ph[i];
        row[7] = 1;
    }
#endif
}

__global__ __launch_bounds__(BLOCK) void k_v3_neflag(uint32_t n, const uint64_t *__restrict__ u_cnt, uint32_t *__restrict__ flag)
{
    const uint32_t t = blockIdx.x * BLOCK + threadIdx.x;
    if (t < n) flag[t] = u_cnt[t] != 0;
}

__global__ __launch_bounds__(BLOCK) void k_v3_nelist(uint32_t n, const uint32_t *__restrict__ flag, const uint32_t *__restrict__ pos,
                                                     const uint32_t *__restrict__ cnt, const uint64_t *__restrict__ u_off,
                                                     uint32_t *__restrict__ ne_t, uint64_t *__restrict__ ne_uoff)
{
    const uint32_t t = blockIdx.x * BLOCK + threadIdx.x;
    if (t < n && flag[t]) { ne_t[pos[t]] = t; ne_uoff[pos[t]] = u_off[t]; }
    if (t == 0) ne_uoff[*cnt] = u_off[n];
}

constexpr uint32_t UC_CHUNK = 4096;

__device__ __forceinline__ uint32_t last_le(const uint64_t *a, uint32_t n, uint64_t x)
{
    uint32_t lo = 0, hi = n;
    while (hi - lo > 1) { const uint32_t m = (lo + hi) >> 1; if (a[m] <= x) lo = m; else hi = m; }
    return lo;
}

__global__ __launch_bounds__(BLOCK) void k_v3_ucompact(uint32_t n, const uint64_t *__restrict__ u_off,
                                                       const uint64_t *__restrict__ arena_off, const uint64_t *__restrict__ kd_off,
                                                       const uint32_t *__restrict__ bigflag, const uint32_t *__restrict__ key_off,
                                                       const uint64_t *__restrict__ vdep_off, const uint32_t *__restrict__ dep_scr,
                                                       const uint32_t *__restrict__ dep_big,
                                                       const uint32_t *__restrict__ tmap, const uint32_t *__restrict__ n_dev,
                                                       uint32_t *__restrict__ dep_txn, const uint64_t *__restrict__ u_all,
                                                       uint64_t *__restrict__ totals)
{
    __shared__ uint64_t uo[BLOCK + 1];
    __shared__ uint64_t src[BLOCK];
    __shared__ uint32_t s_t[2];
    const uint32_t tid = threadIdx.x;
    if (tid == 0 && blockIdx.x == gridDim.x - 1) {
        totals[0] = arena_off[n]; totals[1] = kd_off[n]; totals[2] = u_all[n];
    }
    if (tmap) n = *n_dev;
    const uint64_t total = u_off[n];
    const uint64_t c0 = (uint64_t)blockIdx.x * UC_CHUNK;
    if (c0 >= total) return;
    const uint64_t c1 = min(total, c0 + UC_CHUNK);
    if (tid == 0) { s_t[0] = last_le(u_off, n, c0); s_t[1] = last_le(u_off, n, c1 - 1); }
    __syncthreads();
    const uint32_t tlo = s_t[0], thi = s_t[1];
    auto source = [&](uint32_t j) {
        const uint32_t t = tmap ? tmap[j] : j;
        return bigflag[t] ? (vdep_off[key_off[t]] | (1ull << 63)) : (uint64_t)t * ST_SLOT;
    };
    if (thi - tlo >= 8 * BLOCK) {
        for (uint64_t i = c0 + tid; i < c1; i += BLOCK) {
            uint32_t lo = tlo, hi = thi + 1;
            while (hi - lo > 1) { const uint32_t m = (lo + hi) >> 1; if (u_off[m] <= i) lo = m; else hi = m; }
            const uint64_t sb = source(lo), off = i - u_off[lo];
            dep_txn[i] = (sb >> 63) ? dep_big[(sb & ~(1ull << 63)) + off] : dep_scr[sb + off];
        }
        return;
    }
    for (uint32_t tw = tlo; tw <= thi; tw += BLOCK) {
        const uint32_t nt = min((uint32_t)BLOCK, thi + 1 - tw);
        __syncthreads();
        if (tid < nt) {
            uo[tid] = u_off[tw + tid];
            src[tid] = source(tw + tid);
        }
        if (tid == 0) uo[nt] = u_off[tw + nt];
        __syncthreads();
        const uint64_t lo = max(c0, uo[0]), hi = min(c1, uo[nt]);
        constexpr int U = 4;
        for (uint64_t i0 = lo + tid; i0 < hi; i0 += U * BLOCK) {
            uint32_t x[U];
            bool big[U];
#pragma unroll
            for (int u = 0; u < U; ++u) {
                const uint64_t i = i0 + (uint64_t)u * BLOCK;
                x[u] = 0; big[u] = false;
                if (i < hi) {
                    const uint32_t a = last_le(uo, nt, i);
                    const uint64_t sb = src[a], off = i - uo[a];
                    big[u] = (sb >> 63) != 0;
                    x[u] = big[u] ? dep_big[(sb & ~(1ull << 63)) + off] : dep_scr[sb + off];
                }
            }
#pragma unroll
            for (int u = 0; u < U; ++u)
                if (i0 + (uint64_t)u * BLOCK < hi) dep_txn[i0 + (uint64_t)u * BLOCK] = x[u];
        }
    }
}


struct PairSort {
    Sorted ps{ nullptr, nullptr };
    const uint64_t *sp_m4 = nullptr;
    int key_shift = 0;
    uint32_t *seg_flag = nullptr;
    bool flags_done = false;
    bool tinfo_done = false;
};

static PairSort sort_pairs(acc_ctx *ctx, CfkBuild &cb)
{
    const uint32_t n = cb.n;
    const size_t P = cb.P;
    const uint32_t *key_off = cb.key_off;
    const uint64_t *key_code = cb.key_code;
    const uint32_t *owner = cb.owner, *rank = cb.dict.rank;
    const int rbits = cb.dict.rbits;
    PairPlan &pp = cb.pp;
    pp.rk = make_runs(cb.dict.hg[3]);
    pp.rbits = rbits;
    pp.sb = std::max(1, bits_for(cb.dict.hg[6]));
    uint64_t *pkey = ctx->get<uint64_t>("pair_key", P);
    const unsigned gP = grid_for(P, BLOCK);
    PairSort s;
    s.seg_flag = ctx->get<uint32_t>("seg_flag", P);
    if (cb.dict.batch_sorted && pp.rk.bits <= 32) {
        const bool m4 = bits_for((uint64_t)n - 1) + pp.sb <= 32;
        pp.mode = m4 ? 4 : 3;
        TxnInfoArgs ti;
        ti.n = n; ti.status = cb.status; ti.tl = cb.tl; ti.tinfo = cb.tinfo; ti.bigflag = cb.bigflag;
        launch(ctx, "pair_keys", k_pair_keys, dim3(grid_for(std::max<size_t>(P, n), BLOCK)), dim3(BLOCK), 0, P, key_code,
               owner, key_off, rank, (const uint32_t *)nullptr, pp, 0, pkey, ti);
        s.tinfo_done = true;
        const uint64_t *sp = radix_sort_keys(ctx, "rs_pair", pkey, P, 32, pp.rk.bits);
        uint32_t *perm = ctx->get<uint32_t>("pair_perm", P + V2_ITEMS);
        if (m4) s.sp_m4 = sp;
        else launch(ctx, "seg_flags", k_seg_flags_packed, dim3(gP), dim3(BLOCK), 0, P, sp, s.seg_flag, perm, -1, key_off,
                    (uint32_t *)nullptr);
        s.ps = { nullptr, perm };
        s.flags_done = true;
    } else if (cb.dict.batch_sorted) {
        pp.mode = 0;
        launch(ctx, "pair_keys", k_pair_keys, dim3(gP), dim3(BLOCK), 0, P, key_code, owner, key_off, rank,
               (const uint32_t *)nullptr, pp, 0, pkey, TxnInfoArgs{});
        s.ps = radix_sort(ctx, "rs_pair", pkey, nullptr, P, pp.rk.bits);
    } else if (pp.rk.bits + rbits <= 64) {
        pp.mode = 1;
        launch(ctx, "pair_keys", k_pair_keys, dim3(gP), dim3(BLOCK), 0, P, key_code, owner, key_off, rank,
               (const uint32_t *)nullptr, pp, 0, pkey, TxnInfoArgs{});
        s.ps = radix_sort(ctx, "rs_pair", pkey, nullptr, P, pp.rk.bits + rbits);
        s.key_shift = rbits;
    } else {
        pp.mode = 2;
        launch(ctx, "pair_keys", k_pair_keys, dim3(gP), dim3(BLOCK), 0, P, key_code, owner, key_off, rank,
               (const uint32_t *)nullptr, pp, 1, pkey, TxnInfoArgs{});
        Sorted byrank = radix_sort(ctx, "rs_pair_r", pkey, nullptr, P, rbits);
        launch(ctx, "pair_keys", k_pair_keys, dim3(gP), dim3(BLOCK), 0, P, key_code, owner, key_off, rank,
               (const uint32_t *)byrank.vals, pp, 0, pkey, TxnInfoArgs{});
        s.ps = radix_sort(ctx, "rs_pair", pkey, byrank.vals, P, pp.rk.bits);
    }
    return s;
}

static void build_columns(acc_ctx *ctx, CfkBuild &cb, const PairSort &s, bool tinfo_done)
{
    const uint32_t n = cb.n;
    const size_t P = cb.P;
    const uint32_t *rank = cb.dict.rank;
    const PairPlan &pp = cb.pp;
    const unsigned gP = grid_for(P, BLOCK);
    const uint32_t nt = (uint32_t)((P + V2_TILE - 1) / V2_TILE);
    uint4 *ptinfo = s.sp_m4 ? nullptr : ctx->get<uint4>("pair_tinfo", P);
    uint32_t *tile_sums = ctx->get<uint32_t>("v2_tile_sums", (size_t)NCNT * nt);
    uint32_t *tile_pref = ctx->get<uint32_t>("v2_tile_pref", (size_t)NCNT * nt);
    uint32_t *totals = ctx->get<uint32_t>("v2_totals", 16);
    uint64_t rk_mask = 0;
    for (int r = 0; r < pp.rk.n; ++r) rk_mask |= (pp.rk.len[r] >= 64 ? ~0ull : ((1ull << pp.rk.len[r]) - 1)) << pp.rk.lo[r];
    if (!tinfo_done)
        launch(ctx, "txn_info", k_txn_info, dim3(grid_for(n, BLOCK)), dim3(BLOCK), 0, n, rank, cb.status, cb.tl, cb.key_off,
               cb.tinfo, cb.bigflag);
    if (!s.sp_m4)
        launch(ctx, "pair_tinfo", k_pair_tinfo, dim3(gP), dim3(BLOCK), 0, P, (const uint32_t *)cb.owner, (const uint4 *)cb.tinfo,
               ptinfo);
    launch(ctx, "cfk_gather", k_cfk_gather4, dim3(nt), dim3(BLOCK), 0, P, s.ps.vals, (const uint4 *)ptinfo, s.sp_m4, pp.sb,
           (const uint4 *)cb.tinfo, s.seg_flag, cb.s_rank, cb.s_exec, cb.s_info,
           cb.opts.seg_keys ? cb.pair_pos : (uint32_t *)nullptr, tile_sums, nt);
    launch(ctx, "v2_tile_scans", k_v2_tile_scans, dim3(NCNT), dim3(BLOCK), 0, (const uint32_t *)tile_sums, tile_pref, nt, totals);
    launch(ctx, "v2_apply", k_v2_apply, dim3(nt), dim3(BLOCK), 0, P, (const uint32_t *)cb.s_rank, (const uint32_t *)cb.s_exec,
           (const uint8_t *)cb.s_info, (const uint32_t *)s.seg_flag, (const uint32_t *)tile_pref, (const uint32_t *)totals, nt,
           cb.dict.rbits, cb.cols, cb.seg_incl, cb.seg_start, (const uint32_t *)s.ps.vals, cb.key_code, cb.seg_key, s.sp_m4,
           pp.rk, rk_mask, cb.bases, cb.tot, 4u, cb.gstat, (uint32_t)GSTAT_N, (const uint64_t *)cb.g,
           reinterpret_cast<uint64_t *>(totals) + 4);
    ACC_HIP(hipMemcpyAsync(ctx->pinned, totals, 8 * sizeof(uint64_t), hipMemcpyDeviceToHost, ctx->stream));
    ctx->sync();
}

static void need_pair_pos(acc_ctx *ctx, CfkBuild &cb)
{
    if (cb.have_pair_pos) return;
    launch(ctx, "pair_pos", k_pair_pos, dim3(grid_for(cb.P, BLOCK)), dim3(BLOCK), 0, cb.P, (const uint32_t *)cb.perm, cb.pair_pos);
    cb.have_pair_pos = true;
}

CfkBuild build_cfk(acc_ctx *ctx, const acc_batch_in *in, CfkOpts opts)
{
    if (!in) fail(ACC_E_ARG, "null argument");
    if (in->mem != ACC_MEM_HOST && in->mem != ACC_MEM_DEVICE) fail(ACC_E_ARG, "mem must be ACC_MEM_HOST or ACC_MEM_DEVICE");
    CfkBuild cb;
    cb.opts = opts;
    const uint32_t n = cb.n = in->n_txn;
    const size_t P = cb.P = (size_t)in->n_pairs;
    if (P >= 0xFFFFFFFFull) fail(ACC_E_ARG, "n_pairs must be < 2^32");
    hipStream_t st = ctx->stream;
    ctx->kd_valid = false;

    cb.key_off = stage_in(ctx, "in_key_off", in->key_off, (size_t)n + 1, in->mem);
    if (n == 0 || P == 0) {
        uint64_t *arena_off = ctx->get<uint64_t>("arena_off", (size_t)n + 1);
        uint64_t *kd_off = ctx->get<uint64_t>("kd_off", (size_t)n + 1);
        uint64_t *u_off = ctx->get<uint64_t>("u_off", (size_t)n + 1);
        ACC_HIP(hipMemsetAsync(arena_off, 0, ((size_t)n + 1) * 8, st));
        ACC_HIP(hipMemsetAsync(kd_off, 0, ((size_t)n + 1) * 8, st));
        ACC_HIP(hipMemsetAsync(u_off, 0, ((size_t)n + 1) * 8, st));
        ctx->kd_view = acc_keydeps_view{ n, 0, 0, 0, 0, arena_off, ctx->get<int32_t>("arena", 1), kd_off,
                                         ctx->get<uint32_t>("key_idx", 1), u_off, ctx->get<uint32_t>("dep_txn", 1) };
        ctx->kd_valid = true;
        ctx->sync();
        return cb;
    }
    cb.tm = stage_in(ctx, "in_tm", in->txn_id.msb, n, in->mem);
    cb.tl = stage_in(ctx, "in_tl", in->txn_id.lsb, n, in->mem);
    cb.tn = stage_in(ctx, "in_tn", in->txn_id.node, n, in->mem);
    cb.em = stage_in(ctx, "in_em", in->execute_at.msb, n, in->mem);
    cb.el = stage_in(ctx, "in_el", in->execute_at.lsb, n, in->mem);
    cb.en = stage_in(ctx, "in_en", in->execute_at.node, n, in->mem);
    cb.status = stage_in(ctx, "in_status", in->status, n, in->mem);
    cb.key_code = stage_in(ctx, "in_key_code", in->key_code, P, in->mem);

    cb.g = ctx->get<uint64_t>("g", PREP_G_WORDS);
    cb.owner = ctx->get<uint32_t>("owner", P);
    prep_dictionary(ctx, n, P, cb.tm, cb.tl, cb.tn, cb.em, cb.el, cb.en, cb.status, cb.key_off, cb.key_code, cb.owner, cb.g,
                    cb.dict, true);

    cb.tinfo = ctx->get<uint4>("tinfo", n);
    cb.bigflag = ctx->get<uint32_t>("v3_bigflag", n);
    const PairSort ps = sort_pairs(ctx, cb);
    cb.perm = ps.ps.vals;
    if (!ps.flags_done)
        launch(ctx, "seg_flags", k_seg_flags, dim3(grid_for(P, BLOCK)), dim3(BLOCK), 0, P, (const uint64_t *)ps.ps.keys,
               ps.key_shift, ps.seg_flag);

    cb.seg_incl = ctx->get<uint32_t>("seg_incl", P + V2_ITEMS);
    cb.seg_start = ctx->get<uint32_t>("seg_start", P + 1);
    cb.seg_key = opts.seg_keys ? ctx->get<uint64_t>("seg_key", P + 1) : nullptr;
    cb.s_rank = ctx->get<uint32_t>("s_rank", P + V2_ITEMS);
    cb.s_exec = ctx->get<uint32_t>("s_exec", P + V2_ITEMS);
    cb.s_info = ctx->get<uint8_t>("s_info", P + V2_ITEMS);
    cb.pair_pos = ctx->get<uint32_t>("pair_pos", P);
    cb.have_pair_pos = opts.seg_keys;
    cb.bases = ctx->get<uint32_t>("v2_bases", 16);
    cb.cols.rdir = ctx->get<uint4>("v2_rdir", 4 * (P / RD_W + 1));
    cb.cols.list_rank = ctx->get<uint32_t>("v2_list_rank", P);
    cb.cols.bc_rank = ctx->get<uint32_t>("v2_bc_rank", P);
    cb.cols.bc_exec = ctx->get<uint32_t>("v2_bc_exec", P);
    cb.cols.bc_kind = ctx->get<uint8_t>("v2_bc_kind", P);
    cb.cols.bc_pm_in = ctx->get<uint64_t>("v2_bc_pm_in", P);
    cb.cols.bc_key = ctx->get<uint64_t>("v2_bc_key", P);
    cb.tot = ctx->get<uint64_t>("v3_tot", 4);
    cb.gstat = ctx->get<uint64_t>("v2_gstat", GSTAT_N + 6);
    build_columns(ctx, cb, ps, ps.tinfo_done);
    if (cb.dict.ties_pending && ctx->pinned[6]) {
        check_errors(ctx->pinned[4]);
        redo_general_dictionary(ctx, n, cb.tm, cb.tl, cb.tn, cb.em, cb.el, cb.en, cb.g, cb.dict);
        build_columns(ctx, cb, ps, false);
    }
    cb.dict.ties_pending = false;
    memcpy(cb.htot, ctx->pinned, sizeof cb.htot);
    check_errors(ctx->pinned[4]);
    cb.ties = ctx->pinned[6] != 0;
    ctx->stat("keydeps.path_replay", cb.ties || (ctx->flags & ACC_OPT_FORCE_REPLAY) ? 1 : 0);
    ctx->stat("keydeps.exec_ties", cb.ties ? 1 : 0);
    ctx->stat("keydeps.batch_sorted", cb.dict.batch_sorted ? 1 : 0);
    ctx->stat("keydeps.pair_sort_mode", (uint64_t)cb.pp.mode);
    cb.cfk = true;
    return cb;
}

static void global_fallback(acc_ctx *ctx, CfkBuild &cb, const V2View &vv, const V2Out &wo, uint64_t nfb, uint64_t efb)
{
    hipStream_t st = ctx->stream;
    const int rbits = cb.dict.rbits;
    const uint32_t *key_off = cb.key_off, *txn_of_rank = cb.dict.txn_of_rank, *fb_list = wo.fb_list, *vcnz = wo.cnz;
    const uint64_t *vdep_off = wo.dep_off, *arena_off = wo.arena_off;
    uint32_t *const dep_scr = wo.dep_scratch;
    uint64_t *const u_cnt = wo.u_cnt;
    int32_t *const arena = wo.arena;
    need_pair_pos(ctx, cb);
    uint64_t *vcnt = ctx->get<uint64_t>("cnt", cb.P);
    uint64_t *fb_e = ctx->get<uint64_t>("v2_fb_e", nfb);
    uint64_t *fb_off = ctx->get<uint64_t>("v2_fb_off", nfb + 1);
    uint64_t *fb_maxk = ctx->get<uint64_t>("v2_fb_maxk", 1);
    ACC_HIP(hipMemsetAsync(fb_maxk, 0, sizeof(uint64_t), st));
    launch(ctx, "v2_fb_sizes", k_fb_sizes, dim3(grid_for(nfb, BLOCK)), dim3(BLOCK), 0, (uint32_t)nfb,
           (const uint32_t *)fb_list, key_off, (const uint64_t *)vdep_off, fb_e, fb_maxk);
    scan<uint64_t, OpAdd<uint64_t>>(ctx, fb_e, fb_off, nfb, true, fb_off + nfb);
    ACC_HIP(hipMemcpyAsync(ctx->pinned, fb_maxk, sizeof(uint64_t), hipMemcpyDeviceToHost, st));
    ctx->sync();
    const int bbits = bits_for(nfb - 1);
    const int kbits = std::max(1, bits_for(ctx->pinned[0] - 1));
    if (bbits + rbits + kbits > 64) fail(ACC_E_CAP, "too many oversized txns for the global KeyDeps path");
    uint64_t *gkey = ctx->get<uint64_t>("v2_gkey", efb);
    launch(ctx, "v2_big_gather", k_v2_big_gather, dim3((unsigned)((nfb + WAVES - 1) / WAVES)), dim3(BLOCK), 0,
           (uint32_t)nfb, (const uint32_t *)fb_list, (const uint64_t *)fb_off, vv, (const uint64_t *)vcnt, key_off,
           rbits, kbits, gkey);
    Sorted s1 = radix_sort(ctx, "rs_big1", gkey, nullptr, efb, bbits + rbits + kbits);
    uint32_t *nflag = ctx->get<uint32_t>("v2_big_nflag", efb);
    uint32_t *nincl = ctx->get<uint32_t>("v2_big_nincl", efb);
    launch(ctx, "v2_big_newflag", k_v2_big_newflag, dim3(grid_for(efb, BLOCK)), dim3(BLOCK), 0, efb,
           (const uint64_t *)s1.keys, kbits, nflag);
    scan<uint32_t, OpAdd<uint32_t>>(ctx, nflag, nincl, efb, false);
    uint32_t *idx1 = ctx->get<uint32_t>("v2_big_idx1", efb);
    uint64_t *key2 = ctx->get<uint64_t>("v2_big_key2", efb);
    launch(ctx, "v2_big_rank", k_v2_big_rank, dim3(grid_for(efb, BLOCK)), dim3(BLOCK), 0, efb, (const uint64_t *)s1.keys,
           (const uint32_t *)nincl, (const uint32_t *)fb_list, (const uint64_t *)fb_off, rbits, kbits, key_off,
           (const uint64_t *)vdep_off, (const uint32_t *)txn_of_rank, dep_scr, u_cnt, idx1, key2);
    Sorted s2 = radix_sort(ctx, "rs_big2", key2, nullptr, efb, bbits + kbits + rbits);
    launch(ctx, "v2_big_arena", k_v2_big_arena, dim3(grid_for(efb, BLOCK)), dim3(BLOCK), 0, efb,
           (const uint32_t *)s2.vals, (const uint64_t *)s2.keys, (const uint32_t *)idx1, (const uint32_t *)fb_list,
           (const uint64_t *)fb_off, rbits, kbits, key_off, (const uint32_t *)vcnz, (const uint64_t *)arena_off, arena);
}

static void keydeps_runs(acc_ctx *ctx, CfkBuild &cb, acc_keydeps_view *view)
{
    hipStream_t st = ctx->stream;
    const uint32_t n = cb.n;
    const size_t P = cb.P;
    const unsigned gP = grid_for(P, BLOCK);
    const int rbits = cb.dict.rbits, segbits = bits_for(P);
    const uint32_t *key_off = cb.key_off, *owner = cb.owner, *txn_of_rank = cb.dict.txn_of_rank;
    const V2Cols &cols = cb.cols;
    uint32_t *const bigflag = cb.bigflag;
    uint64_t *const tot = cb.tot, *const gstat = cb.gstat;
    const uint32_t nbc = cb.htot[6];
    if (segbits + rbits > 64) fail(ACC_E_ARG, "batch too large for the (segment, executeAt) composite key");
    Sorted bcs = radix_sort(ctx, "rs_bc", cols.bc_key, nullptr, nbc, segbits + rbits);
    uint32_t *bcs_exec = ctx->get<uint32_t>("v2_bcs_exec", nbc);
    uint64_t *bcs_lw_in = ctx->get<uint64_t>("v2_bcs_lw_in64", nbc), *bcs_lw64 = ctx->get<uint64_t>("v2_bcs_lastw64", nbc);
    launch(ctx, "v2_bcs_cols", k_v2_bcs_cols, dim3(grid_for(nbc, BLOCK)), dim3(BLOCK), 0, nbc, (const uint64_t *)bcs.keys,
           (const uint32_t *)bcs.vals, (const uint8_t *)cols.bc_kind, (uint64_t)((1ull << rbits) - 1), bcs_exec, bcs_lw_in);
    uint64_t *bc_pm64 = ctx->get<uint64_t>("v2_bc_pm64", nbc);
    {
        const uint64_t *si[2] = { bcs_lw_in, cols.bc_pm_in };
        uint64_t *so[2] = { bcs_lw64, bc_pm64 };
        const size_t sn[2] = { nbc, nbc };
        scan_multi<uint64_t, OpMax<uint64_t>>(ctx, 2, si, so, sn, false, (uint64_t *const *)nullptr);
    }

    V2View vv{};
    vv.perm = cb.perm; vv.pair_pos = cb.pair_pos; vv.seg_incl = cb.seg_incl; vv.seg_start = cb.seg_start;
    vv.s_rank = cb.s_rank; vv.s_exec = cb.s_exec; vv.s_info = cb.s_info; vv.rdir = cols.rdir; vv.tinfo = cb.tinfo;
    vv.list_rank = cols.list_rank; vv.bases = cb.bases; vv.bc_rank = cols.bc_rank; vv.bc_exec = cols.bc_exec; vv.bc_pm = bc_pm64;
    vv.bc_kind = cols.bc_kind; vv.bcs_exec = bcs_exec; vv.bcs_lastw = bcs_lw64;
    if (P >= 0x80000000ull) fail(ACC_E_CAP, "n_pairs must be < 2^31 (count-pass record format)");
    RecOut ro;
    ro.rec = ctx->get<uint4>("v2_rec", 4 * P);
    ro.irec = ctx->get<uint4>("v2_irec", 2 * P);
    uint4 *rec = ro.rec;
    vv.irec32 = reinterpret_cast<const uint32_t *>(ro.irec);
    vv.rec = ro.rec;

    uint32_t *bpos = ctx->get<uint32_t>("v3_bpos", n);
    uint64_t *blk_e = ctx->get<uint64_t>("v3_blk_e", gP);
    uint32_t *psz = ctx->get<uint32_t>("v3_psz", P);
#ifdef ACC_PHASE_PROF
    const size_t ct_rows = (size_t)gP * WAVES;
    unsigned long long *ct_buf = prof_arm(ctx, "v2_ct_prof", HIP_SYMBOL(g_ct_prof), 8 * ct_rows, st);
#endif
    launch(ctx, "v2_count", k_v2_count, dim3(gP), dim3(BLOCK), 0, P, vv, (const uint32_t *)owner, ro, bigflag, blk_e);
#ifdef ACC_PHASE_PROF
    {
        const std::vector<unsigned long long> h = prof_read(ct_buf, 8 * ct_rows, st);
        double sum[8] = {}, mx[3] = {};
        size_t w = 0;
        for (size_t r = 0; r < ct_rows; ++r) {
            if (!(h[8 * r + 7] >> 32)) continue;
            ++w;
            for (int i = 0; i < 7; ++i) sum[i] += (double)h[8 * r + i];
            sum[7] += (double)(h[8 * r + 7] & 0xFFFFFFFFu);
            for (int i = 0; i < 3; ++i) mx[i] = std::max(mx[i], (double)h[8 * r + i]);
        }
        const double d = w ? (double)w : 1.0;
        fprintf(stderr, "[ct_phase] waves=%zu avg cycles: query %.0f r3count %.0f inline+write %.0f | max %.0f %.0f %.0f | "
                "per pair: bumped %.4f seg-with-bc %.4f posM-search %.4f r3-candidates %.3f run-records %.4f\n",
                w, sum[0] / d, sum[1] / d, sum[2] / d, mx[0], mx[1], mx[2], sum[3] / P, sum[4] / P, sum[5] / P, sum[6] / P,
                sum[7] / P);
    }
#endif
    const uint32_t raw_cap = ST_RAW;
    uint64_t *kd_off = ctx->get<uint64_t>("kd_off", (size_t)n + 1);
    uint64_t *arena_off = ctx->get<uint64_t>("arena_off", (size_t)n + 1);
    uint64_t *szA = ctx->get<uint64_t>("v3_szA", n), *szK = ctx->get<uint64_t>("v3_szK", n);
    uint64_t *eb = ctx->get<uint64_t>("v3_eb", n), *dB = ctx->get<uint64_t>("v3_dB", (size_t)n + 1);
    uint32_t *runflag = ctx->get<uint32_t>("v3_runflag", n);
    launch(ctx, "v3_mark", k_v3_mark, dim3(grid_for((size_t)n * MK_G, BLOCK)), dim3(BLOCK), 0, n, key_off,
           (const uint32_t *)ro.irec, (const uint4 *)rec, psz, raw_cap, bigflag, szA, szK, tot + 2, eb, runflag);
    uint64_t *blk_pre = ctx->get<uint64_t>("v3_blk_pre", gP);
    {
        const uint64_t *si[4] = { szA, szK, blk_e, eb };
        uint64_t *so[4] = { arena_off, kd_off, blk_pre, dB }, *stot[4] = { arena_off + n, kd_off + n, tot, dB + n };
        const size_t sn[4] = { n, n, gP, n };
        scan_multi<uint64_t, OpAdd<uint64_t>>(ctx, 4, si, so, sn, true, stot);
    }
    scan<uint32_t, OpAdd<uint32_t>>(ctx, bigflag, bpos, n, true, reinterpret_cast<uint32_t *>(tot + 1));
    uint32_t *blist = ctx->get<uint32_t>("v3_blist", n);
    launch(ctx, "v3_compact", k_v3_compact, dim3(grid_for(n, BLOCK)), dim3(BLOCK), 0, n, (const uint32_t *)bigflag,
           (const uint32_t *)bpos, blist);
    uint32_t *rpos = ctx->get<uint32_t>("v3_rpos", n), *rlist = ctx->get<uint32_t>("v3_rlist", n);
    scan<uint32_t, OpAdd<uint32_t>>(ctx, runflag, rpos, n, true, reinterpret_cast<uint32_t *>(tot + 3));
    launch(ctx, "v3_compact", k_v3_compact, dim3(grid_for(n, BLOCK)), dim3(BLOCK), 0, n, (const uint32_t *)runflag,
           (const uint32_t *)rpos, rlist);
    ACC_HIP(hipMemcpyAsync(ctx->pinned, tot, 4 * sizeof(uint64_t), hipMemcpyDeviceToHost, st));
    ctx->sync();
    const uint64_t E = ctx->pinned[0];
    const uint32_t nbig = (uint32_t)ctx->pinned[1];
    const bool any16 = ctx->pinned[2] != 0;
    const uint32_t nrun = (uint32_t)ctx->pinned[3];
    if (E >= 0xFFFFFFFFull) fail(ACC_E_CAP, "more than 2^32-1 dependency entries in one batch");
    uint64_t *u_off = ctx->get<uint64_t>("u_off", (size_t)n + 1);
    uint64_t *u_cnt = ctx->get<uint64_t>("u_cnt", n);
    uint64_t *vdep_off = nullptr;
    uint32_t *dep_scr = nullptr;
    uint64_t nfb = 0, efb = 0, nmed = 0, nbig2 = 0;
    ctx->stat("keydeps.huge_txns", 0);
    V2Out wo{};
    bool win_ok = false;
#ifdef ACC_PHASE_PROF
    unsigned long long *win_buf = nullptr;
#endif
    uint64_t *vcnt = nullptr;
    uint32_t *med_list = nullptr, *big_list = nullptr, *fb_list = nullptr;
    auto sort_tiers = [&](bool with_med) {
        if (with_med)
            launch(ctx, "v2_write_med", k_v2_write_big<MED_CAP, BLOCK>, dim3(std::min<unsigned>(nbig, 2048)), dim3(BLOCK), 0,
                   (const uint32_t *)med_list, vv, (const uint64_t *)vcnt, wo);
        launch(ctx, "v2_write_big", k_v2_write_big<BIG_E, 512>, dim3(std::min<unsigned>(nbig, 1024)), dim3(512), 0,
               (const uint32_t *)big_list, vv, (const uint64_t *)vcnt, wo);
        launch(ctx, "v2_write_huge", k_v2_write_big<HUGE_E, 1024>, dim3(std::min<unsigned>(nbig, 64)), dim3(1024), 0,
               (const uint32_t *)wo.huge_list, vv, (const uint64_t *)vcnt, wo);
    };
    uint32_t *dep_st = ctx->get<uint32_t>("v3_dep_stream", (size_t)n * ST_SLOT);
    int32_t *const arena = ctx->get<int32_t>("arena", P + E);
    uint32_t *const key_idx = ctx->get<uint32_t>("key_idx", P);
    uint32_t *const dep_txn = ctx->get<uint32_t>("dep_txn", std::max<uint64_t>(E, 1));
    auto finish = [&]() {
        scan<uint64_t, OpAdd<uint64_t>>(ctx, u_cnt, u_off, n, true, u_off + n);
        const uint32_t *tmap = nullptr, *ne_cnt = nullptr;
        const uint64_t *uo = u_off;
        if (cb.opts.sparse) {
            uint32_t *flag = ctx->get<uint32_t>("v3_ne_flag", n), *pos = ctx->get<uint32_t>("v3_ne_pos", n);
            uint32_t *cnt = ctx->get<uint32_t>("v3_ne_cnt", 1), *ne_t = ctx->get<uint32_t>("v3_ne_t", n);
            uint64_t *ne_uoff = ctx->get<uint64_t>("v3_ne_uoff", (size_t)n + 1);
            launch(ctx, "v3_neflag", k_v3_neflag, dim3(grid_for(n, BLOCK)), dim3(BLOCK), 0, n, (const uint64_t *)u_cnt, flag);
            scan<uint32_t, OpAdd<uint32_t>>(ctx, flag, pos, n, true, cnt);
            launch(ctx, "v3_nelist", k_v3_nelist, dim3(grid_for(n, BLOCK)), dim3(BLOCK), 0, n, (const uint32_t *)flag,
                   (const uint32_t *)pos, (const uint32_t *)cnt, (const uint64_t *)u_off, ne_t, ne_uoff);
            tmap = ne_t; ne_cnt = cnt; uo = ne_uoff;
        }
        launch(ctx, "v3_ucompact", k_v3_ucompact, dim3((unsigned)((E + UC_CHUNK - 1) / UC_CHUNK) + 1), dim3(BLOCK), 0, n,
               uo, (const uint64_t *)arena_off, (const uint64_t *)kd_off, (const uint32_t *)bigflag, key_off,
               (const uint64_t *)vdep_off, (const uint32_t *)dep_st, (const uint32_t *)dep_scr,
               tmap, ne_cnt, dep_txn, (const uint64_t *)u_off, gstat + GSTAT_N);
        ACC_HIP(hipMemcpyAsync(ctx->pinned, gstat, (GSTAT_N + 6) * sizeof(uint64_t), hipMemcpyDeviceToHost, st));
        ctx->sync();
    };
    if (nbig) {
        const unsigned gB = (nbig + WAVES - 1) / WAVES;
        vdep_off = ctx->get<uint64_t>("dep_off", P + 1);
        vcnt = ctx->get<uint64_t>("cnt", P);
        uint32_t *vcnz = ctx->get<uint32_t>("cnz", P + 1);
        dep_scr = ctx->get<uint32_t>("v2_dep_scratch", std::max<uint64_t>(E, 1));
        med_list = ctx->get<uint32_t>("v2_med_list", nbig);
        big_list = ctx->get<uint32_t>("v2_big_list", nbig);
        fb_list = ctx->get<uint32_t>("v2_fb_list", nbig);
        V3Big bg;
        bg.blist = blist; bg.key_off = key_off; bg.psz = psz; bg.dB = dB; bg.arena_off = arena_off; bg.kd_off = kd_off;
        bg.vdep_off = vdep_off; bg.vcnt = vcnt; bg.vcnz = vcnz; bg.u_cnt = u_cnt; bg.arena = arena; bg.key_idx = key_idx;
        const bool big_ok = rbits + 6 <= 31;
        win_ok = big_ok && !(ctx->flags & ACC_OPT_NO_WINDOW_TIER);
        launch(ctx, "v3_route", k_v3_route, dim3(grid_for(nbig, BLOCK)), dim3(BLOCK), 0, nbig, (const uint32_t *)blist,
               key_off, (const uint64_t *)eb, (int)big_ok, (int)win_ok, med_list, big_list, fb_list,
               ctx->get<uint32_t>("v2_w8_list", nbig), ctx->get<uint32_t>("v2_w16_list", nbig), gstat);
        launch(ctx, "v3_bigfill", k_v3_bigfill, dim3(gB), dim3(BLOCK), 0, nbig, bg);
        wo.key_off = key_off; wo.dep_off = vdep_off; wo.arena_off = arena_off; wo.cnz = vcnz; wo.txn_of_rank = txn_of_rank;
        wo.arena = arena; wo.dep_scratch = dep_scr; wo.u_cnt = u_cnt; wo.gstat = gstat;
        wo.rec = rec; wo.irec32 = vv.irec32; wo.med_list = med_list; wo.big_list = big_list; wo.fb_list = fb_list;
        wo.huge_list = ctx->get<uint32_t>("v2_huge_list", nbig);
        ctx->fork(nrun ? 2 : 1);
        ctx->launch_stream = ctx->aux[0];
        if (win_ok) {
#ifdef ACC_PHASE_PROF
            win_buf = prof_arm(ctx, "v2_win_prof", HIP_SYMBOL(g_win_prof), 10, ctx->aux[0]);
#endif
            launch(ctx, "v2_write_win", k_v2_write_win<8>, dim3(std::min<unsigned>(nbig, 2048)), dim3(BLOCK), 0,
                   (const uint32_t *)ctx->get<uint32_t>("v2_w8_list", nbig), (const uint64_t *)(gstat + 7), vv,
                   (const uint64_t *)vcnt, wo);
            if (any16)
                launch(ctx, "v2_write_win16", k_v2_write_win<16>, dim3(std::min<unsigned>(nbig, 256)), dim3(BLOCK), 0,
                       (const uint32_t *)ctx->get<uint32_t>("v2_w16_list", nbig), (const uint64_t *)(gstat + 8), vv,
                       (const uint64_t *)vcnt, wo);
        } else if (big_ok) {
            sort_tiers(true);
        } else {
            launch(ctx, "v2_write_medium", k_v2_write_medium, dim3(std::min<unsigned>(gB, 2048)), dim3(BLOCK), 0,
                   (const uint64_t *)gstat, (const uint32_t *)med_list, vv, (const uint64_t *)vcnt, wo);
        }
        ctx->launch_stream = nullptr;
    }
    {
        constexpr int st_nt = 256;
        const uint32_t tt = (uint32_t)st_nt / ST_G;
        const uint32_t nblocks = (n + tt - 1) / tt;
        const uint32_t ntiles = nblocks * (uint32_t)(st_nt / 64);
        V3Stream sp;
        sp.v = vv; sp.err = gstat + 5;
        sp.key_off = key_off; sp.bigflag = bigflag; sp.list = nullptr; sp.txn_of_rank = txn_of_rank;
        sp.rec = rec; sp.irec = ro.irec;
        sp.arena_off = arena_off; sp.kd_off = kd_off; sp.u_cnt_out = u_cnt; sp.arena = arena; sp.key_idx = key_idx;
        sp.dep_scr = dep_st; sp.n = n; sp.ntiles = ntiles;
#ifdef ACC_PHASE_PROF
        const size_t prof_rows = (size_t)ntiles;
        unsigned long long *prof_buf = prof_arm(ctx, "v3_prof", HIP_SYMBOL(g_st_prof), 8 * prof_rows, st);
#endif
        if (nrun) {
            if (!nbig) ctx->fork(2);
            V3Stream sr = sp;
            sr.list = rlist; sr.n = nrun;
            const uint32_t rblocks = (nrun + tt - 1) / tt;
            ctx->launch_stream = ctx->aux[1];
            if (rbits <= 28) launch(ctx, "v3_stream_runs", k_v3_stream<uint32_t, st_nt, ST_G, ST_N2, true, true>, dim3(rblocks), dim3(st_nt), 0, sr);
            else launch(ctx, "v3_stream_runs", k_v3_stream<uint64_t, st_nt, ST_G, ST_N2, true, true>, dim3(rblocks), dim3(st_nt), 0, sr);
            ctx->launch_stream = nullptr;
        }
        if (rbits <= 28) launch(ctx, "v3_stream", k_v3_stream<uint32_t, st_nt, ST_G, ST_N2, false, false>, dim3(nblocks), dim3(st_nt), 0, sp);
        else launch(ctx, "v3_stream", k_v3_stream<uint64_t, st_nt, ST_G, ST_N2, false, false>, dim3(nblocks), dim3(st_nt), 0, sp);
#ifdef ACC_PHASE_PROF
        {
            const std::vector<unsigned long long> h = prof_read(prof_buf, 8 * prof_rows, st);
            double sum[6] = {}, mx[6] = {};
            size_t w = 0;
            for (size_t r = 0; r < prof_rows; ++r) {
                if (!h[8 * r + 7]) continue;
                ++w;
                for (int i = 0; i < 6; ++i) { sum[i] += (double)h[8 * r + i]; mx[i] = std::max(mx[i], (double)h[8 * r + i]); }
            }
            const double d = w ? (double)w : 1.0;
            fprintf(stderr, "[st_phase] waves=%zu avg cycles: setup %.0f records %.0f gather %.0f sort %.0f emit-lds %.0f lookback+copy %.0f | max: %.0f %.0f %.0f %.0f %.0f %.0f\n",
                    w, sum[0] / d, sum[1] / d, sum[2] / d, sum[3] / d, sum[4] / d, sum[5] / d, mx[0], mx[1], mx[2], mx[3], mx[4], mx[5]);
        }
#endif
    }
    if (nbig || nrun) ctx->join(nrun ? 2 : 1);
#ifdef ACC_PHASE_PROF
    if (nbig && win_ok) {
        const std::vector<unsigned long long> h = prof_read(win_buf, 10, st);
        const double nt = h[6] ? (double)h[6] : 1.0;
        fprintf(stderr, "[win_phase] txns=%llu avg cycles per txn (thread 0 of each block): runs+lowend %.0f gather %.0f "
                "below-sort %.0f prefix %.0f span-writes %.0f rank-map %.0f list-wait %.0f | avg E %.1f span words %.1f below %.1f\n",
                h[6], h[0] / nt, h[1] / nt, h[2] / nt, h[3] / nt, h[4] / nt, h[5] / nt, h[9] / nt, h[7] / nt,
                (double)(h[8] >> 32) / nt, (double)(h[8] & 0xFFFFFFFFull) / nt);
    }
#endif
    finish();
    if (ctx->pinned[5]) fail(ACC_E_STATE, "internal: stream gather count differs from the count pass");
    if (ctx->pinned[2]) fail(ACC_E_STATE, "internal: v2 gather count differs from the count pass");
    if (nbig && win_ok && (ctx->pinned[0] || ctx->pinned[1])) {
        sort_tiers(ctx->pinned[0] != 0);
        finish();
        if (ctx->pinned[2]) fail(ACC_E_STATE, "internal: v2 gather count differs from the count pass");
    }
    if (nbig) {
        nmed = ctx->pinned[0]; nbig2 = ctx->pinned[1];
        nfb = ctx->pinned[3]; efb = ctx->pinned[4];
        ctx->stat("keydeps.huge_txns", ctx->pinned[6]);
        ctx->stat("keydeps.window_txns", ctx->pinned[7] + ctx->pinned[8]);
    }
    if (nfb) {
        global_fallback(ctx, cb, vv, wo, nfb, efb);
        finish();
    }
    ctx->stat("keydeps.stream_txns", n - nbig);
    ctx->stat("keydeps.stream_run_txns", nrun);
    ctx->stat("keydeps.big_path_txns", nbig);
    ctx->stat("keydeps.medium_txns", nmed);
    ctx->stat("keydeps.big_txns", nbig2);
    ctx->stat("keydeps.fallback_txns", nfb);
    ctx->stat("keydeps.fallback_entries", efb);
    ctx->stat("keydeps.bumped_committed", nbc);
    *view = acc_keydeps_view{ n, ctx->pinned[GSTAT_N], ctx->pinned[GSTAT_N + 1], ctx->pinned[GSTAT_N + 2], E, arena_off,
                              arena, kd_off, key_idx, u_off, dep_txn };
    ctx->kd_view = *view;
    ctx->kd_valid = true;
}

void keydeps_of(acc_ctx *ctx, CfkBuild &cb, acc_keydeps_view *view)
{
    if (!cb.cfk) {
        *view = ctx->kd_view;
    } else if (cb.ties || (ctx->flags & ACC_OPT_FORCE_REPLAY)) {
        need_pair_pos(ctx, cb);
        keydeps_replay(ctx, cb, view);
    } else {
        keydeps_runs(ctx, cb, view);
    }
}

void keydeps_batch(acc_ctx *ctx, const acc_batch_in *in, acc_keydeps_view *view)
{
    if (!in || !view) fail(ACC_E_ARG, "null argument");
    CfkBuild cb = build_cfk(ctx, in, CfkOpts{});
    keydeps_of(ctx, cb, view);
}


uint32_t cfk_nseg(acc_ctx *ctx, const CfkBuild &cb)
{
    ACC_HIP(hipMemcpyAsync(ctx->pinned, cb.seg_incl + cb.P - 1, sizeof(uint32_t), hipMemcpyDeviceToHost, ctx->stream));
    ctx->sync();
    return (uint32_t)(ctx->pinned[0] & 0xFFFFFFFFu);
}

CfkBuild cfk_snapshot(acc_ctx *ctx, const acc_batch_in *in)
{
    CfkOpts opts;
    opts.seg_keys = true;
    CfkBuild cb = build_cfk(ctx, in, opts);
    ctx->kd_valid = false;
    if (cb.cfk) cb.nseg = cfk_nseg(ctx, cb);
    return cb;
}

}
```

### cassandra-accord_amd/csrc/keydeps.hpp

```cpp
#pragma once

#include "dict.hpp"

namespace acc {

struct PairPlan {
    Runs rk;
    int rbits;
    int mode;
    int sb;
};

struct V2Cols {
    uint4 *rdir;
    uint32_t *list_rank;
    uint32_t *bc_rank, *bc_exec;
    uint8_t *bc_kind;
    uint64_t *bc_pm_in;
    uint64_t *bc_key;
};

__device__ __forceinline__ uint32_t lower_bound_u32(const uint32_t *a, uint32_t lo, uint32_t hi, uint32_t v)
{
    while (lo < hi) {
// ... 8 lines not shown
    while (lo < hi) {
        const uint32_t m = (lo + hi) >> 1;
        if ((uint32_t)a[m] < v) lo = m + 1; else hi = m;
    }
    return lo;
}

__device__ __forceinline__ uint64_t shfl_xor64(uint64_t v, int m)
{
    uint32_t lo = __shfl_xor((uint32_t)v, m, 64), hi = __shfl_xor((uint32_t)(v >> 32), m, 64);
    return ((uint64_t)hi << 32) | lo;
}

__device__ __forceinline__ void wave_bitonic_lds(uint64_t *buf, uint32_t n2)
{
    const uint32_t lane = lane_id();
    for (uint32_t k = 2; k <= n2; k <<= 1) {
        for (uint32_t jj = k >> 1; jj > 0; jj >>= 1) {
            for (uint32_t i = lane; i < n2; i += 64) {
                uint32_t l = i ^ jj;
                if (l > i) {
                    uint64_t a = buf[i], b = buf[l];
                    bool up = (i & k) == 0;
                    if ((a > b) == up) { buf[i] = b; buf[l] = a; }
                }
            }
            __builtin_amdgcn_wave_barrier();
            __builtin_amdgcn_fence(__ATOMIC_RELEASE, "wavefront");
        }
    }
}


struct CfkView {
    const uint32_t *seg_start, *s_rank, *s_exec, *seg_incl, *pair_pos, *owner, *rank;
    const uint8_t *s_info;
    const uint32_t *cl_start, *cl_exec, *lastw;
    const uint32_t *pmax;
    const uint32_t *cum_u, *u_pos;
    const uint64_t *tl;
    uint32_t n;
    const uint32_t *vseg;
};

struct Query {
    uint32_t s0, pos, scan_start, ub, ue, trank, wk;
    bool p1, has_m;
    uint32_t m;
};

__device__ __forceinline__ Query make_query_ts(const CfkView &v, uint32_t t, uint32_t seg);

__device__ __forceinline__ Query make_query(const CfkView &v, uint32_t j)
{
    return make_query_ts(v, v.owner[j], v.vseg ? v.vseg[j] : v.seg_incl[v.pair_pos[j]] - 1);
}

__device__ __forceinline__ Query make_query_ts(const CfkView &v, uint32_t t, uint32_t seg)
{
    Query q;
    uint32_t s0 = v.seg_start[seg], s1 = v.seg_start[seg + 1];
    uint32_t S = v.rank[v.n + t];
    q.trank = v.rank[t];
    q.p1 = S != q.trank;
    q.wk = witnesses((uint32_t)(v.tl[t] >> 1) & 7u);
    q.s0 = s0;
    q.pos = lower_bound_u32(v.s_rank, s0, s1, S);
    uint32_t c0 = v.cl_start[seg], c1 = v.cl_start[seg + 1];
    uint32_t from = c0, to = c1;
    long i = -1;
    bool found = false;
    while (from < to) {
        uint32_t mid = (from + to) >> 1;
        uint32_t e = v.cl_exec[mid];
        if (S < e) to = mid;
        else if (S > e) from = mid + 1;
        else { i = (long)mid - 1; found = true; break; }
    }
    if (!found) i = (long)to - 1;
    q.has_m = false;
    q.m = 0;
    if (i >= (long)c0) {
        uint32_t w = v.lastw[i];
        if (w != 0 && w - 1 >= c0) { q.has_m = true; q.m = v.cl_exec[w - 1]; }
    }
    q.scan_start = q.has_m ? lower_bound_u32(v.pmax, s0, q.pos, q.m + 1) : s0;
    q.ub = v.cum_u[s0];
    q.ue = v.cum_u[q.scan_start];
    return q;
}

template <bool EMIT, bool FIRST = false>
__device__ __forceinline__ uint32_t run_query(const CfkView &v, const Query &q, uint32_t *__restrict__ out)
{
    uint32_t c = 0;
    for (uint32_t u = q.ub; u < q.ue; ++u) {
        uint32_t p = v.u_pos[u];
        uint32_t kind = v.s_info[p] >> 3;
        if (!((q.wk >> kind) & 1u)) continue;
        uint32_t r = v.s_rank[p];
        if (q.p1 && r == q.trank) continue;
        if (EMIT) out[c] = r;
        else if (FIRST && c == 0) out[0] = r;
        ++c;
    }
    for (uint32_t p = q.scan_start; p < q.pos; ++p) {
        uint32_t info = v.s_info[p];
        uint32_t st = info & 7u, kind = info >> 3;
        if (!((q.wk >> kind) & 1u)) continue;
        if (st == 0 || st == 7) continue;
        if (st >= 4 && st <= 6 && q.has_m && v.s_exec[p] < q.m) continue;
        uint32_t r = v.s_rank[p];
        if (q.p1 && r == q.trank) continue;
        if (EMIT) out[c] = r;
        else if (FIRST && c == 0) out[0] = r;
        ++c;
    }
    return c;
}


struct CfkOpts {
    bool seg_keys = false;
    bool sparse = false;
};

struct CfkBuild {
    bool cfk = false;
    CfkOpts opts;
    uint32_t n = 0;
    size_t P = 0;
    const uint64_t *tm = nullptr, *tl = nullptr, *em = nullptr, *el = nullptr;
    const int32_t *tn = nullptr, *en = nullptr;
    const uint8_t *status = nullptr;
    const uint32_t *key_off = nullptr;
    const uint64_t *key_code = nullptr;
    Dictionary dict;
    uint32_t *owner = nullptr;
    uint64_t *g = nullptr;
    bool ties = false;
    PairPlan pp{};
    uint32_t *perm = nullptr;
    uint32_t *pair_pos = nullptr;
    bool have_pair_pos = false;
    uint32_t *seg_incl = nullptr;
    uint32_t *seg_start = nullptr;
    uint64_t *seg_key = nullptr;
    uint32_t nseg = 0;
    uint32_t *s_rank = nullptr, *s_exec = nullptr;
    uint8_t *s_info = nullptr;
    uint4 *tinfo = nullptr;
    uint32_t *bigflag = nullptr;
    uint32_t htot[16] = {};
    V2Cols cols{};
    uint32_t *bases = nullptr;
    uint64_t *tot = nullptr;
    uint64_t *gstat = nullptr;
    bool v1 = false;
    CfkView v1view{};
};

CfkBuild build_cfk(acc_ctx *ctx, const acc_batch_in *in, CfkOpts opts);
void keydeps_of(acc_ctx *ctx, CfkBuild &cb, acc_keydeps_view *view);
uint32_t cfk_nseg(acc_ctx *ctx, const CfkBuild &cb);
CfkBuild cfk_snapshot(acc_ctx *ctx, const acc_batch_in *in);
CfkView build_v1_cfk(acc_ctx *ctx, const CfkBuild &cb, bool multi_only = false);
void keydeps_replay(acc_ctx *ctx, CfkBuild &cb, acc_keydeps_view *view);

}
```

### cassandra-accord_amd/csrc/prims.hpp

```cpp
#pragma once

#include "ctx.hpp"

#include <algorithm>
#include <vector>

namespace acc {

constexpr int BLOCK = 256;
constexpr int WAVES = BLOCK / 64;


__device__ __forceinline__ uint32_t lane_id() { return threadIdx.x & 63u; }

template <class T>
__device__ __forceinline__ T shfl_up(T v, unsigned d)
{
    if constexpr (sizeof(T) == 8) {
        uint64_t u = (uint64_t)v;
        uint32_t lo = __shfl_up((uint32_t)u, d, 64), hi = __shfl_up((uint32_t)(u >> 32), d, 64);
        return (T)(((uint64_t)hi << 32) | lo);
    } else {
        return (T)__shfl_up((uint32_t)v, d, 64);
    }
// ... 145 lines not shown
    }
    return x;
}

template <class T, int NT = BLOCK>
__device__ void block_bitonic(T *a, uint32_t n2)
{
    for (uint32_t k = 2; k <= n2; k <<= 1) {
        for (uint32_t jj = k >> 1; jj > 0; jj >>= 1) {
            for (uint32_t i = threadIdx.x; i < n2; i += NT) {
                const uint32_t l = i ^ jj;
                if (l > i) {
                    const T x = a[i], y = a[l];
                    const bool up = (i & k) == 0;
                    if ((x > y) == up) { a[i] = y; a[l] = x; }
                }
            }
            __syncthreads();
        }
    }
}


constexpr uint64_t SCAN_AGG = 1ull << 62, SCAN_INC = 2ull << 62, SCAN_VAL = (1ull << 62) - 1;

__device__ __forceinline__ void scan_status_store(uint64_t *p, uint64_t w)
{
    __hip_atomic_store(p, w, __ATOMIC_RELAXED, __HIP_MEMORY_SCOPE_AGENT);
}
__device__ __forceinline__ uint64_t scan_status_load(const uint64_t *p)
{
    return __hip_atomic_load(p, __ATOMIC_RELAXED, __HIP_MEMORY_SCOPE_AGENT);
}

constexpr int SCAN_MAXA = 4;
template <class T>
struct ScanArgs {
    const T *in[SCAN_MAXA];
    T *out[SCAN_MAXA];
    T *total[SCAN_MAXA];
    uint64_t n[SCAN_MAXA];
    uint32_t cum[SCAN_MAXA + 1];
    int k;
};

template <class T, class Op, int ITEMS>
__global__ __launch_bounds__(BLOCK) void k_scan_1p(ScanArgs<T> a, int exclusive, uint32_t *__restrict__ ticket,
                                                 uint64_t *__restrict__ status, uint64_t *__restrict__ other, uint32_t other_n)
{
    constexpr int TILE = BLOCK * ITEMS;
    __shared__ T tile[TILE + TILE / 32];
    __shared__ T lds[WAVES];
    __shared__ uint32_t s_b;
    __shared__ T s_prefix;
    const uint32_t tid = threadIdx.x, lane = lane_id();
    if (other_n) {
        const uint32_t chunk = (other_n + gridDim.x - 1) / gridDim.x;
        const uint32_t lo = blockIdx.x * chunk, hi = min(other_n, lo + chunk);
        for (uint32_t i = lo + tid; i < hi; i += BLOCK) other[i] = 0;
    }
    if (tid == 0) s_b = atomicAdd(ticket, 1u);
    __syncthreads();
    const uint32_t tk = s_b;
    int ai = 0;
#pragma unroll
    for (int q = 1; q < SCAN_MAXA; ++q) ai += (q < a.k && tk >= a.cum[q]) ? 1 : 0;
    const uint32_t b = tk - a.cum[ai];
    const T *__restrict__ in = a.in[ai];
    T *__restrict__ out = a.out[ai];
    T *__restrict__ total_out = a.total[ai];
    const size_t n = a.n[ai];
    uint64_t *const st = status + a.cum[ai];
    const size_t base = (size_t)b * TILE;
    Op op;
#pragma unroll
    for (int i = 0; i < ITEMS; ++i) {
        const uint32_t li = i * BLOCK + tid;
        const size_t g = base + li;
        tile[li + li / 32] = g < n ? in[g] : Op::identity();
    }
    __syncthreads();
    T v[ITEMS];
    T acc = Op::identity();
#pragma unroll
    for (int i = 0; i < ITEMS; ++i) {
        const uint32_t li = tid * ITEMS + i;
        v[i] = tile[li + li / 32];
        acc = op(acc, v[i]);
    }
    T total;
    T run = block_exclusive(acc, op, lds, total);
    if (b == 0) {
        if (tid == 0) scan_status_store(&st[0], (uint64_t)total | SCAN_INC);
    } else {
        if (tid == 0) scan_status_store(&st[b], (uint64_t)total | SCAN_AGG);
        if (tid < 64) {
            T pre = Op::identity();
            int64_t j = (int64_t)b - 1;
            while (true) {
                const int64_t idx = j - (int64_t)lane;
                uint64_t w = (uint64_t)Op::identity() | SCAN_INC;
                if (idx >= 0) {
                    w = scan_status_load(&st[idx]);
                    while ((w >> 62) == 0) {
                        __builtin_amdgcn_s_sleep(1);
                        w = scan_status_load(&st[idx]);
                    }
                }
                const uint64_t inc = __ballot((w >> 62) == 2);
                const uint32_t stop = inc ? (uint32_t)__builtin_ctzll(inc) : 63u;
                T x = lane <= stop ? (T)(w & SCAN_VAL) : Op::identity();
#pragma unroll
                for (int d = 32; d >= 1; d >>= 1) x = op(x, shfl_xor(x, d));
                pre = op(pre, x);
                if (inc) break;
                j -= 64;
            }
            if (tid == 0) {
                scan_status_store(&st[b], (uint64_t)op(pre, total) | SCAN_INC);
                s_prefix = pre;
            }
        }
        __syncthreads();
        run = op(s_prefix, run);
    }
#pragma unroll
    for (int i = 0; i < ITEMS; ++i) {
        const uint32_t li = tid * ITEMS + i;
        const T incl = op(run, v[i]);
        tile[li + li / 32] = exclusive ? run : incl;
        if (total_out && base + li == n - 1) *total_out = incl;
        run = incl;
    }
    __syncthreads();
#pragma unroll
    for (int i = 0; i < ITEMS; ++i) {
        const uint32_t li = i * BLOCK + tid;
        const size_t g = base + li;
        if (g < n) out[g] = tile[li + li / 32];
    }
}

template <class T, class Op>
void scan_multi(acc_ctx *ctx, int k, const T *const *in, T *const *out, const size_t *n, bool exclusive, T *const *total_out)
{
    constexpr int ITEMS = sizeof(T) == 8 ? 16 : 32;
    constexpr size_t TILE = (size_t)BLOCK * ITEMS;
    if (k < 1 || k > SCAN_MAXA) fail(ACC_E_STATE, "internal: scan_multi array count");
    ScanArgs<T> a{};
    size_t nb = 0;
    int m = 0;
    for (int i = 0; i < k; ++i) {
        if (n[i] == 0) {
            if (total_out && total_out[i]) ACC_HIP(hipMemsetAsync(total_out[i], 0, sizeof(T), ctx->stream));
            continue;
        }
        a.in[m] = in[i]; a.out[m] = out[i]; a.total[m] = total_out ? total_out[i] : nullptr; a.n[m] = n[i];
        a.cum[m] = (uint32_t)nb;
        nb += (n[i] + TILE - 1) / TILE;
        if (nb > 0xFFFFFFF0ull) fail(ACC_E_CAP, "scan too large");
        ++m;
    }
    if (m == 0) return;
    a.k = m;
    for (int i = m; i <= SCAN_MAXA; ++i) a.cum[i] = (uint32_t)nb;
    if (ctx->launch_stream) fail(ACC_E_STATE, "internal: scan launched on a side stream");
    const size_t need = nb + 1;
    uint64_t *buf[2];
    if (need > ctx->scan_cap) {
        for (int i = 0; i < 2; ++i) {
            buf[i] = ctx->get_raw<uint64_t>(i ? "scan_status1" : "scan_status0", need);
            ACC_HIP(hipMemsetAsync(buf[i], 0, need * sizeof(uint64_t), ctx->stream));
        }
        ctx->scan_cap = need;
        ctx->scan_dirty[0] = ctx->scan_dirty[1] = 0;
    } else {
        for (int i = 0; i < 2; ++i) buf[i] = ctx->get_raw<uint64_t>(i ? "scan_status1" : "scan_status0", need);
    }
    const int p = ctx->scan_par;
    uint64_t *status = buf[p];
    uint32_t *ticket = reinterpret_cast<uint32_t *>(status + nb);
    launch(ctx, "scan", k_scan_1p<T, Op, ITEMS>, dim3((unsigned)nb), dim3(BLOCK), 0, a, (int)exclusive, ticket, status,
           buf[p ^ 1], (uint32_t)ctx->scan_dirty[p ^ 1]);
    ctx->scan_dirty[p] = need;
    ctx->scan_dirty[p ^ 1] = 0;
    ctx->scan_par = p ^ 1;
}

template <class T, class Op>
void scan(acc_ctx *ctx, const T *in, T *out, size_t n, bool exclusive, T *total_out = nullptr)
{
    T *const tot[1] = { total_out };
    scan_multi<T, Op>(ctx, 1, &in, &out, &n, exclusive, tot);
}

static __global__ __launch_bounds__(BLOCK) void k_sum_u32(const uint32_t *__restrict__ in, size_t n, uint64_t *__restrict__ out)
{
    __shared__ uint64_t lds[WAVES];
    uint64_t x = 0;
    for (size_t i = (size_t)blockIdx.x * BLOCK + threadIdx.x; i < n; i += (size_t)gridDim.x * BLOCK) x += in[i];
    uint64_t total;
    block_exclusive(x, OpAdd<uint64_t>(), lds, total);
    if (threadIdx.x == 0 && total) atomicAdd((unsigned long long *)out, (unsigned long long)total);
}

inline void sum_u32(acc_ctx *ctx, const uint32_t *in, size_t n, uint64_t *out)
{
    ACC_HIP(hipMemsetAsync(out, 0, 8, ctx->stream));
    if (n) launch(ctx, "sum_u32", k_sum_u32, dim3((unsigned)std::min<size_t>(1024, (n + BLOCK - 1) / BLOCK)), dim3(BLOCK), 0,
                  in, n, out);
}


struct Runs {
    static constexpr int MAX_RUNS = 12;
    int n = 0;
    int bits = 0;
    uint8_t lo[MAX_RUNS] = {}, len[MAX_RUNS] = {}, dst[MAX_RUNS] = {};
};

inline Runs make_runs(uint64_t mask)
{
    Runs r;
    int b = 0;
    int count = 0;
    for (int i = 0; i < 64;) {
        if (!((mask >> i) & 1)) { ++i; continue; }
        int j = i;
        while (j < 64 && ((mask >> j) & 1)) ++j;
        ++count;
        i = j;
    }
    if (count > Runs::MAX_RUNS) {
        int lo = __builtin_ctzll(mask), hi = 63 - __builtin_clzll(mask);
        r.n = 1; r.lo[0] = (uint8_t)lo; r.len[0] = (uint8_t)(hi - lo + 1); r.dst[0] = 0; r.bits = hi - lo + 1;
        return r;
    }
    for (int i = 0; i < 64;) {
        if (!((mask >> i) & 1)) { ++i; continue; }
        int j = i;
        while (j < 64 && ((mask >> j) & 1)) ++j;
        r.lo[r.n] = (uint8_t)i; r.len[r.n] = (uint8_t)(j - i); r.dst[r.n] = (uint8_t)b;
        b += j - i; ++r.n;
        i = j;
    }
    r.bits = b;
    return r;
}

__device__ __forceinline__ uint64_t pext_runs(uint64_t w, const Runs &r)
{
    uint64_t o = 0;
    for (int i = 0; i < r.n; ++i) {
        uint64_t m = r.len[i] >= 64 ? ~0ull : ((1ull << r.len[i]) - 1);
        o |= ((w >> r.lo[i]) & m) << r.dst[i];
    }
    return o;
}


constexpr int RS_ITEMS = 16;
constexpr int RS_TILE = BLOCK * RS_ITEMS;
constexpr int RS_ITEMS_S = 4;
constexpr int RS_TILE_S = BLOCK * RS_ITEMS_S;
constexpr size_t rs_small_n() { return (size_t)256 << 10; }

static __global__ __launch_bounds__(BLOCK) void k_rs_hist(const uint64_t *__restrict__ keys, size_t n, int shift,
                                                   uint32_t *__restrict__ hist, uint32_t ntiles)
{
    __shared__ uint32_t h[256];
    h[threadIdx.x] = 0;
    __syncthreads();
    const size_t base = (size_t)blockIdx.x * RS_TILE;
#pragma unroll 4
    for (int k = 0; k < RS_ITEMS; ++k) {
        size_t e = base + (size_t)k * BLOCK + threadIdx.x;
        if (e < n) atomicAdd(&h[(keys[e] >> shift) & 255u], 1u);
    }
    __syncthreads();
    hist[(size_t)threadIdx.x * ntiles + blockIdx.x] = h[threadIdx.x];
}

static __global__ __launch_bounds__(BLOCK) void k_rs_colscan(uint32_t *__restrict__ hist, uint32_t ntiles,
                                                      uint32_t *__restrict__ total)
{
    __shared__ uint32_t red[WAVES];
    uint32_t *col = hist + (size_t)blockIdx.x * ntiles;
    constexpr uint32_t PER = 8;
    uint32_t carry = 0;
    for (uint32_t base = 0; base < ntiles; base += BLOCK * PER) {
        const uint32_t i0 = base + threadIdx.x * PER;
        uint32_t v[PER], sum = 0;
#pragma unroll
        for (uint32_t j = 0; j < PER; ++j) { v[j] = i0 + j < ntiles ? col[i0 + j] : 0u; sum += v[j]; }
        uint32_t tot;
        uint32_t run = carry + block_exclusive(sum, OpAdd<uint32_t>(), red, tot);
#pragma unroll
        for (uint32_t j = 0; j < PER; ++j) if (i0 + j < ntiles) { col[i0 + j] = run; run += v[j]; }
        carry += tot;
    }
    if (threadIdx.x == 0) total[blockIdx.x] = carry;
}

static __global__ __launch_bounds__(BLOCK) void k_rs_scatter(const uint64_t *__restrict__ kin, const uint32_t *__restrict__ vin,
                                                      uint64_t *__restrict__ kout, uint32_t *__restrict__ vout,
                                                      size_t n, int shift, const uint32_t *__restrict__ colpre,
                                                      const uint32_t *__restrict__ dtotal, uint32_t ntiles, int iota_vals)
{
    __shared__ uint64_t sk[RS_TILE];
    __shared__ uint32_t sv[RS_TILE];
    __shared__ uint32_t cnt[WAVES][256];
    __shared__ uint32_t wpre[WAVES][256];
    __shared__ uint32_t run[256], lbase[256], gbase[256];
    __shared__ uint32_t red[WAVES];
    const uint32_t tid = threadIdx.x, lane = lane_id(), wave = tid >> 6;
    const uint64_t lt_mask = (lane == 0) ? 0ull : ((~0ull) >> (64 - lane));
    const size_t hi = (size_t)tid * ntiles + blockIdx.x;
    const uint32_t dt = dtotal[tid];
    const uint32_t c0 = colpre[hi];
    const uint32_t c1 = blockIdx.x + 1 < ntiles ? colpre[hi + 1] : dt;
    uint32_t all;
    const uint32_t dbase = block_exclusive(dt, OpAdd<uint32_t>(), red, all);
    const uint32_t g0 = dbase + c0;
    uint32_t tile_total;
    const uint32_t lb = block_exclusive(c1 - c0, OpAdd<uint32_t>(), red, tile_total);
    lbase[tid] = lb;
    gbase[tid] = g0;
    run[tid] = lb;
#pragma unroll
    for (int w = 0; w < WAVES; ++w) cnt[w][tid] = 0;
    __syncthreads();
    const size_t base = (size_t)blockIdx.x * RS_TILE;
    for (int k = 0; k < RS_ITEMS; ++k) {
        size_t e = base + (size_t)k * BLOCK + tid;
        bool valid = e < n;
        uint64_t key = valid ? kin[e] : 0;
        uint32_t val = valid ? (iota_vals ? (uint32_t)e : vin[e]) : 0;
        uint32_t d = (uint32_t)(key >> shift) & 255u;
        uint64_t peers = __ballot(valid);
#pragma unroll
        for (int b = 0; b < 8; ++b) {
            uint64_t bal = __ballot((d >> b) & 1u);
            peers &= ((d >> b) & 1u) ? bal : ~bal;
        }
        uint32_t rank = (uint32_t)__popcll(peers & lt_mask);
        if (valid && rank == 0) cnt[wave][d] = (uint32_t)__popcll(peers);
        __syncthreads();
        {
            uint32_t r = run[tid];
#pragma unroll
            for (int w = 0; w < WAVES; ++w) {
                wpre[w][tid] = r;
                r += cnt[w][tid];
                cnt[w][tid] = 0;
            }
            run[tid] = r;
        }
        __syncthreads();
        if (valid) {
            uint32_t dst = wpre[wave][d] + rank;
            sk[dst] = key;
// ... 66 lines not shown
    __shared__ uint32_t sv[KO ? 1 : (BLOCK * ITEMS)];
    __shared__ uint32_t cnt[WAVES][256];
    __shared__ uint32_t wpre[WAVES][256];
    __shared__ uint32_t run[256], lbase[256], gbase[256];
    __shared__ uint32_t red[WAVES];
    __shared__ uint32_t s_b;
    const uint32_t tid = threadIdx.x, lane = lane_id(), wave = tid >> 6;
    const uint64_t lt_mask = (lane == 0) ? 0ull : ((~0ull) >> (64 - lane));
    if (tid == 0) s_b = atomicAdd(ticket, 1u);
    run[tid] = 0;
#pragma unroll
    for (int w = 0; w < WAVES; ++w) cnt[w][tid] = 0;
    __syncthreads();
    const uint32_t b = s_b;
    const size_t base = (size_t)b * (BLOCK * ITEMS);
    uint64_t key[ITEMS];
    uint32_t val[ITEMS], lr[ITEMS], pk[ITEMS];
#pragma unroll
    for (int k = 0; k < ITEMS; ++k) {
        const size_t e = base + (size_t)k * BLOCK + tid;
        const bool valid = e < n;
        key[k] = valid ? kin[e] : 0;
        if constexpr (!KO) val[k] = valid ? (iota_vals ? (uint32_t)e : vin[e]) : 0;
    }
#pragma unroll
    for (int k = 0; k < ITEMS; ++k) {
        const bool valid = base + (size_t)k * BLOCK + tid < n;
        const uint32_t d = (uint32_t)(key[k] >> shift) & 255u;
        uint64_t peers = __ballot(valid);
#pragma unroll
        for (int bb = 0; bb < 8; ++bb) {
            const uint64_t bal = __ballot((d >> bb) & 1u);
            peers &= ((d >> bb) & 1u) ? bal : ~bal;
        }
        const uint32_t rank = (uint32_t)__popcll(peers & lt_mask);
        pk[k] = rank | ((uint32_t)__popcll(peers) << 16);
        if (valid && rank == 0) atomicAdd(&run[d], (uint32_t)__popcll(peers));
    }
    __syncthreads();
    const uint32_t c = run[tid];
    uint32_t *st = status + (size_t)b * 256;
    os_store(&st[tid], b == 0 ? (c | OS_INC) : (c | OS_AGG));
    uint32_t tile_total;
    const uint32_t lb = block_exclusive(c, OpAdd<uint32_t>(), red, tile_total);
    run[tid] = 0;
    lbase[tid] = lb;
    __syncthreads();
#pragma unroll
    for (int k = 0; k < ITEMS; ++k) {
        const bool valid = base + (size_t)k * BLOCK + tid < n;
        const uint32_t d = (uint32_t)(key[k] >> shift) & 255u;
        const uint32_t rank = pk[k] & 0xFFFFu;
        if (valid && rank == 0) cnt[wave][d] = pk[k] >> 16;
        __syncthreads();
        {
            uint32_t r = run[tid];
#pragma unroll
            for (int w = 0; w < WAVES; ++w) {
                wpre[w][tid] = r;
                r += cnt[w][tid];
                cnt[w][tid] = 0;
            }
            run[tid] = r;
        }
        __syncthreads();
        lr[k] = wpre[wave][d] + rank;
    }
#pragma unroll
    for (int k = 0; k < ITEMS; ++k) {
        const size_t e = base + (size_t)k * BLOCK + tid;
        if (e < n) {
            const uint32_t d = (uint32_t)(key[k] >> shift) & 255u;
            const uint32_t dst = lbase[d] + lr[k];
            sk[dst] = key[k];
            if constexpr (!KO) sv[dst] = val[k];
        }
    }
    uint32_t all;
    const uint32_t dbase = block_exclusive(dtotal[tid], OpAdd<uint32_t>(), red, all);
    uint32_t pre = 0;
    if (b > 0) {
#ifndef ACC_OS_LB
#define ACC_OS_LB 8
#endif
        constexpr int LB = ACC_OS_LB;
        for (int64_t j = (int64_t)b - 1;; j -= LB) {
            uint32_t w[LB];
#pragma unroll
            for (int u = 0; u < LB; ++u) w[u] = j - u >= 0 ? os_load(&status[(size_t)(j - u) * 256 + tid]) : OS_INC;
            bool done = false;
#pragma unroll
            for (int u = 0; u < LB; ++u) {
                if (done) continue;
                while ((w[u] >> 30) == 0) {
                    __builtin_amdgcn_s_sleep(1);
                    w[u] = os_load(&status[(size_t)(j - u) * 256 + tid]);
                }
                pre += w[u] & OS_VAL;
                done = (w[u] >> 30) == 2;
            }
            if (done) break;
        }
        os_store(&st[tid], (pre + c) | OS_INC);
    }
    gbase[tid] = dbase + pre;
    __syncthreads();
    for (uint32_t i = tid; i < tile_total; i += BLOCK) {
        const uint64_t k2 = sk[i];
        const uint32_t d = (uint32_t)(k2 >> shift) & 255u;
        const uint32_t dst = gbase[d] + (i - lbase[d]);
        kout[dst] = k2;
        if constexpr (!KO) vout[dst] = sv[i];
    }
}

static __global__ void k_iota(uint32_t *__restrict__ out, size_t n)
{
    size_t i = (size_t)blockIdx.x * blockDim.x + threadIdx.x;
    if (i < n) out[i] = (uint32_t)i;
}

[[maybe_unused]] static __global__ __launch_bounds__(BLOCK) void k_widen_u32(size_t n, const uint32_t *__restrict__ in, uint64_t *__restrict__ out)
{
    const size_t p = (size_t)blockIdx.x * BLOCK + threadIdx.x;
    if (p < n) out[p] = in[p];
}

[[maybe_unused]] static __global__ __launch_bounds__(BLOCK) void k_permute_u64(size_t n, const uint32_t *__restrict__ perm,
                                                              const uint64_t *__restrict__ in, uint64_t *__restrict__ out)
{
    const size_t p = (size_t)blockIdx.x * BLOCK + threadIdx.x;
    if (p < n) out[p] = in[perm[p]];
}

struct Sorted {
    uint64_t *keys;
    uint32_t *vals;
};

struct OsWords {
    uint32_t *cur, *other;
    uint32_t other_n;
    acc_ctx::OsState *st;
    size_t words;
    void commit() const
    {
        st->dirty[st->par] = words;
        st->dirty[st->par ^ 1] = 0;
        st->par ^= 1;
    }
};
static inline OsWords os_words(acc_ctx *ctx, const char *tag, size_t words)
{
    if (ctx->launch_stream) fail(ACC_E_STATE, "internal: radix sort launched on a side stream");
    if (words >= 0xFFFFFFFFull) fail(ACC_E_CAP, "internal: radix sort status beyond 2^32 words");
    acc_ctx::OsState &s = ctx->os_state[ctx->ns + tag];
    char n0[56], n1[56];
    snprintf(n0, sizeof n0, "%s_os0", tag);
    snprintf(n1, sizeof n1, "%s_os1", tag);
    uint32_t *b[2] = { ctx->get<uint32_t>(n0, std::max(words, s.cap)), ctx->get<uint32_t>(n1, std::max(words, s.cap)) };
    if (words > s.cap) {
        for (int i = 0; i < 2; ++i) ACC_HIP(hipMemsetAsync(b[i], 0, words * sizeof(uint32_t), ctx->stream));
        s.cap = words;
        s.dirty[0] = s.dirty[1] = 0;
    }
    return OsWords{ b[s.par], b[s.par ^ 1], (uint32_t)s.dirty[s.par ^ 1], &s, words };
}

static inline Sorted radix_sort(acc_ctx *ctx, const char *tag, const uint64_t *keys, const uint32_t *vals, size_t n, int bits)
{
    char nk0[40], nk1[40], nv0[40], nv1[40], nh[40], th[48], ts[48];
    snprintf(th, sizeof th, "%s.hist", tag);
    snprintf(ts, sizeof ts, "%s.scatter", tag);
    snprintf(nk0, sizeof nk0, "%s_k0", tag); snprintf(nk1, sizeof nk1, "%s_k1", tag);
    snprintf(nv0, sizeof nv0, "%s_v0", tag); snprintf(nv1, sizeof nv1, "%s_v1", tag);
    snprintf(nh, sizeof nh, "%s_hist", tag);
    uint64_t *k[2] = { ctx->get<uint64_t>(nk0, n), ctx->get<uint64_t>(nk1, n) };
    uint32_t *v[2] = { ctx->get<uint32_t>(nv0, n), ctx->get<uint32_t>(nv1, n) };
    int passes = (bits + 7) / 8;
    if (n == 0) return { k[0], v[0] };
    if (passes == 0) {
        ACC_HIP(hipMemcpyAsync(k[0], keys, n * sizeof(uint64_t), hipMemcpyDeviceToDevice, ctx->stream));
        if (vals) ACC_HIP(hipMemcpyAsync(v[0], vals, n * sizeof(uint32_t), hipMemcpyDeviceToDevice, ctx->stream));
        else launch(ctx, "iota", k_iota, dim3(grid_for(n, BLOCK)), dim3(BLOCK), 0, v[0], n);
        return { k[0], v[0] };
    }
    if (n < (size_t)OS_VAL && passes <= OS_MAXP) {
        const bool small = n < rs_small_n();
        const uint32_t ntiles = (uint32_t)((n + (small ? RS_TILE_S : RS_TILE) - 1) / (small ? RS_TILE_S : RS_TILE));
        const size_t words = (size_t)passes * 256 + passes + (size_t)passes * ntiles * 256;
        const OsWords ow = os_words(ctx, tag, words);
        uint32_t *ghist = ow.cur, *tickets = ow.cur + (size_t)passes * 256, *status = tickets + passes;
        snprintf(th, sizeof th, "%s.ghist", tag);
        launch(ctx, th, k_rs_ghist, dim3(std::min<unsigned>(ntiles, 1024u)), dim3(BLOCK), 0, keys, n, 0, passes, ghist, ow.other,
               ow.other_n);
        ow.commit();
        const uint64_t *kin = keys;
        const uint32_t *vin = vals;
        int cur = 0;
        for (int p = 0; p < passes; ++p) {
            if (small)
                launch(ctx, ts, k_rs_onesweep<false, RS_ITEMS_S>, dim3(ntiles), dim3(BLOCK), 0, kin, vin, k[cur], v[cur], n, 8 * p,
                       (const uint32_t *)(ghist + (size_t)p * 256), status + (size_t)p * ntiles * 256, tickets + p,
                       (p == 0 && !vals) ? 1 : 0);
            else
                launch(ctx, ts, k_rs_onesweep<false, RS_ITEMS>, dim3(ntiles), dim3(BLOCK), 0, kin, vin, k[cur], v[cur], n, 8 * p,
                       (const uint32_t *)(ghist + (size_t)p * 256), status + (size_t)p * ntiles * 256, tickets + p,
                       (p == 0 && !vals) ? 1 : 0);
            kin = k[cur];
            vin = v[cur];
            cur ^= 1;
        }
        return { (uint64_t *)kin, (uint32_t *)vin };
    }
    const uint32_t ntiles = (uint32_t)((n + RS_TILE - 1) / RS_TILE);
    uint32_t *hist = ctx->get<uint32_t>(nh, (size_t)256 * ntiles);
    char nt[48];
    snprintf(nt, sizeof nt, "%s_dtot", tag);
    uint32_t *dtot = ctx->get<uint32_t>(nt, 256);
    const uint64_t *kin = keys;
    const uint32_t *vin = vals;
    int cur = 0;
    for (int p = 0; p < passes; ++p) {
        int shift = 8 * p;
        launch(ctx, th, k_rs_hist, dim3(ntiles), dim3(BLOCK), 0, kin, n, shift, hist, ntiles);
        launch(ctx, "rs_colscan", k_rs_colscan, dim3(256), dim3(BLOCK), 0, hist, ntiles, dtot);
        launch(ctx, ts, k_rs_scatter, dim3(ntiles), dim3(BLOCK), 0, kin, vin, k[cur], v[cur], n, shift,
               (const uint32_t *)hist, (const uint32_t *)dtot, ntiles, (p == 0 && !vals) ? 1 : 0);
        kin = k[cur];
        vin = v[cur];
        cur ^= 1;
    }
    return { (uint64_t *)kin, (uint32_t *)vin };
}

static inline uint64_t *radix_sort_keys(acc_ctx *ctx, const char *tag, const uint64_t *keys, size_t n, int lo, int bits)
{
    char nk0[40], nk1[40], th[48], ts[48];
    snprintf(nk0, sizeof nk0, "%s_k0", tag); snprintf(nk1, sizeof nk1, "%s_k1", tag);
    snprintf(th, sizeof th, "%s.ghist", tag);
    snprintf(ts, sizeof ts, "%s.scatter", tag);
    uint64_t *k[2] = { ctx->get<uint64_t>(nk0, n), ctx->get<uint64_t>(nk1, n) };
    const int passes = (bits + 7) / 8;
    if (n >= (size_t)OS_VAL || passes > OS_MAXP) fail(ACC_E_CAP, "internal: keys-only radix sort beyond its limits");
    if (n == 0 || passes == 0) {
        if (n) ACC_HIP(hipMemcpyAsync(k[0], keys, n * sizeof(uint64_t), hipMemcpyDeviceToDevice, ctx->cur()));
        return k[0];
    }
    const bool small = n < rs_small_n();
    const uint32_t ntiles = (uint32_t)((n + (small ? RS_TILE_S : RS_TILE) - 1) / (small ? RS_TILE_S : RS_TILE));
    const size_t words = (size_t)passes * 256 + passes + (size_t)passes * ntiles * 256;
    const OsWords ow = os_words(ctx, tag, words);
    uint32_t *ghist = ow.cur, *tickets = ow.cur + (size_t)passes * 256, *status = tickets + passes;
    launch(ctx, th, k_rs_ghist, dim3(std::min<unsigned>(ntiles, 1024u)), dim3(BLOCK), 0, keys, n, lo, passes, ghist, ow.other,
           ow.other_n);
    ow.commit();
    const uint64_t *kin = keys;
    int cur = 0;
    for (int p = 0; p < passes; ++p) {
        if (small)
            launch(ctx, ts, k_rs_onesweep<true, RS_ITEMS_S>, dim3(ntiles), dim3(BLOCK), 0, kin, (const uint32_t *)nullptr, k[cur],
                   (uint32_t *)nullptr, n, lo + 8 * p, (const uint32_t *)(ghist + (size_t)p * 256),
                   status + (size_t)p * ntiles * 256, tickets + p, 0);
        else
            launch(ctx, ts, k_rs_onesweep<true, RS_ITEMS>, dim3(ntiles), dim3(BLOCK), 0, kin, (const uint32_t *)nullptr, k[cur],
                   (uint32_t *)nullptr, n, lo + 8 * p, (const uint32_t *)(ghist + (size_t)p * 256),
                   status + (size_t)p * ntiles * 256, tickets + p, 0);
        kin = k[cur];
        cur ^= 1;
    }
    return (uint64_t *)kin;
}

inline int bits_for(uint64_t max_value)
{
    return max_value == 0 ? 0 : 64 - __builtin_clzll(max_value);
}

#ifdef ACC_PHASE_PROF
template <class Sym>
inline unsigned long long *prof_arm(acc_ctx *ctx, const char *name, const Sym &symbol, size_t words, hipStream_t st)
{
    unsigned long long *buf = ctx->get<unsigned long long>(name, words);
    ACC_HIP(hipMemsetAsync(buf, 0, words * sizeof(unsigned long long), st));
    ACC_HIP(hipMemcpyToSymbolAsync(symbol, &buf, sizeof buf, 0, hipMemcpyHostToDevice, st));
    return buf;
}
inline std::vector<unsigned long long> prof_read(const unsigned long long *buf, size_t words, hipStream_t st)
{
    std::vector<unsigned long long> h(words);
    ACC_HIP(hipMemcpyAsync(h.data(), buf, words * sizeof(unsigned long long), hipMemcpyDeviceToHost, st));
    ACC_HIP(hipStreamSynchronize(st));
    return h;
}
#endif

}
```

### cassandra-accord_amd/csrc/ts.hpp

```cpp
#pragma once

#include <hip/hip_runtime.h>
#include <stdint.h>

namespace acc {

constexpr uint64_t IDENTITY_LSB = 0xFFFFFFFFFFFF001EULL;

__device__ __forceinline__ uint64_t ts_w1(uint64_t lsb) { return lsb & IDENTITY_LSB; }
__device__ __forceinline__ uint64_t ts_w2(int32_t node) { return (uint64_t)((uint32_t)node ^ 0x80000000u); }

__device__ __forceinline__ int ts_cmp(uint64_t am, uint64_t al, int32_t an, uint64_t bm, uint64_t bl, int32_t bn)
{
    if (am != bm) return am < bm ? -1 : 1;
    uint64_t a1 = ts_w1(al), b1 = ts_w1(bl);
    if (a1 != b1) return a1 < b1 ? -1 : 1;
    if (an != bn) return an < bn ? -1 : 1;
    return 0;
}

__device__ __forceinline__ uint32_t witnesses(uint32_t kind)
{
    switch (kind) {
    case 0: case 2: return 1u << 1;
    case 1: case 3: return (1u << 0) | (1u << 1);
    case 4:         return (1u << 0) | (1u << 1) | (1u << 3) | (1u << 4);
    default:        return 0;
    }
}

}
```

Before: 3.276 billion txn-key pairs/s.

## Build bumped-committed sorted columns on a side lane concurrent with main pipeline

Splits dictionary prep from dictionary build and counts bumped-committed key entries in the prep kernel. The bumped-committed (key, executeAt) sort keys are then built directly from the sorted bumped list and sorted on an auxiliary stream lane, overlapping with the main keydeps work. Scan and radix-sort state is duplicated per lane so these primitives can run on that lane. This adds event fork/join bookkeeping, a deferred graveyard free while the lane is open, and a consistency check between the two counts.

```diff
diff --git a/cassandra-accord_amd/csrc/api.hip b/cassandra-accord_amd/csrc/api.hip
--- a/cassandra-accord_amd/csrc/api.hip
+++ b/cassandra-accord_amd/csrc/api.hip
@@ -97,6 +97,7 @@
         if (ctx->join_ev[i]) (void)hipEventDestroy(ctx->join_ev[i]);
     }
     if (ctx->fork_ev) (void)hipEventDestroy(ctx->fork_ev);
+    if (ctx->lane_ev) (void)hipEventDestroy(ctx->lane_ev);
     if (ctx->pinned) (void)hipHostFree(ctx->pinned);
     if (ctx->stream) (void)hipStreamDestroy(ctx->stream);
     acc_ctx *child = ctx->child;
diff --git a/cassandra-accord_amd/csrc/ctx.hpp b/cassandra-accord_amd/csrc/ctx.hpp
--- a/cassandra-accord_amd/csrc/ctx.hpp
+++ b/cassandra-accord_amd/csrc/ctx.hpp
@@ -52,9 +52,15 @@
     static constexpr int NAUX = 3;
     hipStream_t aux[NAUX] = {};
     hipEvent_t fork_ev = nullptr, join_ev[NAUX] = {};
+    hipEvent_t lane_ev = nullptr;
+    bool lane_open = false;
     hipStream_t launch_stream = nullptr;
-    size_t scan_cap = 0, scan_dirty[2] = {0, 0};
-    int scan_par = 0;
+    struct ScanState {
+        size_t cap = 0, dirty[2] = {0, 0};
+        int par = 0;
+    };
+    ScanState scan_st[2];
+    int scan_lane() const { return !launch_stream ? 0 : launch_stream == aux[0] ? 1 : -1; }
     struct OsState {
         size_t cap = 0, dirty[2] = {0, 0};
         int par = 0;
@@ -66,7 +72,7 @@
     acc_ctx *child = nullptr;
     std::unordered_map<std::string, acc::Buf> bufs;
     std::vector<void *> graveyard;
-    static constexpr size_t PINNED_WORDS = 1024, PINNED_SLOTS = 512;
+    static constexpr size_t PINNED_WORDS = 1536, PINNED_SLOTS = 512;
     uint64_t *pinned = nullptr;
     std::vector<acc::TimingSlot> slots;
     std::unordered_map<std::string, int> slot_index;
@@ -176,6 +182,7 @@
     {
         if (!fork_ev) {
             ACC_HIP(hipEventCreateWithFlags(&fork_ev, hipEventDisableTiming));
+            ACC_HIP(hipEventCreateWithFlags(&lane_ev, hipEventDisableTiming));
             for (int i = 0; i < NAUX; ++i) {
                 ACC_HIP(hipStreamCreateWithFlags(&aux[i], hipStreamNonBlocking));
                 ACC_HIP(hipEventCreateWithFlags(&join_ev[i], hipEventDisableTiming));
@@ -193,17 +200,24 @@
         launch_stream = nullptr;
     }
 
+    void lane_fork() { fork(1); lane_open = true; }
+    void lane_join() { if (lane_open) { join(1); lane_open = false; } }
+    void lane_mark() { ACC_HIP(hipEventRecord(lane_ev, aux[0])); }
+    void lane_wait() { ACC_HIP(hipStreamWaitEvent(stream, lane_ev, 0)); }
+
     void recover() noexcept
     {
         launch_stream = nullptr;
         for (int i = 0; i < NAUX; ++i)
             if (aux[i]) (void)hipStreamSynchronize(aux[i]);
         if (stream) (void)hipStreamSynchronize(stream);
+        lane_open = false;
     }
 
     void sync()
     {
         ACC_HIP(hipStreamSynchronize(stream));
+        if (lane_open) return;
         for (void *p : graveyard) ACC_HIP(hipFree(p));
         graveyard.clear();
         if (!pending.empty()) resolve_timing();
diff --git a/cassandra-accord_amd/csrc/dict.hpp b/cassandra-accord_amd/csrc/dict.hpp
--- a/cassandra-accord_amd/csrc/dict.hpp
+++ b/cassandra-accord_amd/csrc/dict.hpp
@@ -14,6 +14,10 @@
     bool fast = false;
     bool ties_pending = false;
     uint64_t hg[8] = {};
+    uint64_t nbc = 0;
+    bool fast_ok = false;
+    uint32_t nb = 0;
+    const uint32_t *sb_vals = nullptr, *bsrc = nullptr;
 };
 
 struct DenseRank {
@@ -26,7 +30,13 @@
 DenseRank dense_rank(acc_ctx *ctx, const char *tag, size_t n, int nw, const uint64_t *const *words, const uint64_t *and_mask,
                      const uint64_t *xor_mask, bool want_first);
 
-constexpr size_t PREP_G_WORDS = 8 + 64 * 8;
+constexpr uint32_t PREP_SLOTS = 64, PREP_ROW = 16;
+constexpr size_t PREP_G_WORDS = 8 + (size_t)PREP_SLOTS * PREP_ROW;
+void prep_batch(acc_ctx *ctx, uint32_t n, size_t P, const uint64_t *tm, const uint64_t *tl, const int32_t *tn,
+                const uint64_t *em, const uint64_t *el, const int32_t *en, const uint8_t *status, const uint32_t *key_off,
+                const uint64_t *key_code, uint32_t *owner, uint64_t *g, Dictionary &out);
+void build_dictionary(acc_ctx *ctx, uint32_t n, const uint64_t *tm, const uint64_t *tl, const int32_t *tn,
+                      const uint64_t *em, const uint64_t *el, const int32_t *en, uint64_t *g, Dictionary &out, bool defer_ties);
 void prep_dictionary(acc_ctx *ctx, uint32_t n, size_t P, const uint64_t *tm, const uint64_t *tl, const int32_t *tn,
                      const uint64_t *em, const uint64_t *el, const int32_t *en, const uint8_t *status,
                      const uint32_t *key_off, const uint64_t *key_code, uint32_t *owner, uint64_t *g, Dictionary &out,
diff --git a/cassandra-accord_amd/csrc/dictionary.hip b/cassandra-accord_amd/csrc/dictionary.hip
--- a/cassandra-accord_amd/csrc/dictionary.hip
+++ b/cassandra-accord_amd/csrc/dictionary.hip
@@ -182,7 +182,6 @@
     }
 }
 
-constexpr uint32_t PREP_SLOTS = 64;
 
 __global__ __launch_bounds__(BLOCK) void k_prep_txn(uint32_t n, size_t P, const uint64_t *__restrict__ tm, const uint64_t *__restrict__ tl,
                                                     const int32_t *__restrict__ tn, const uint64_t *__restrict__ em,
@@ -195,6 +194,7 @@
     const uint32_t tid = threadIdx.x;
     uint64_t m0 = 0, m1 = 0, m2 = 0, km = 0, errs = 0, unsorted = 0, ornk = 0;
     uint32_t differs = 0;
+    unsigned long long bckeys = 0;
     const uint64_t r0 = tm[0], r1 = ts_w1(tl[0]), r2 = ts_w2(tn[0]);
     const uint64_t kref = P ? key_code[0] : 0;
     if (blockIdx.x == 0 && tid == 0 && key_off[n] != P) errs |= ERR_KEY_TOTAL;
@@ -204,6 +204,7 @@
         __syncthreads();
         if (tid < tcnt) ko[tid] = key_off[t];
         if (tid == 0) ko[tcnt] = key_off[t0 + tcnt];
+        bool bc = false;
         if (t < n) {
             const bool d = tm[t] != em[t] || ts_w1(tl[t]) != ts_w1(el[t]) || tn[t] != en[t];
             differs += d;
@@ -215,12 +216,16 @@
             uint32_t kind = (uint32_t)(tl[t] >> 1) & 7u;
             if (kind >= 6) errs |= ERR_BAD_KIND;
             else if (kind == 5) errs |= ERR_LOCAL_ONLY;
+            bc = bumped_committed(status[t], kind, d);
             if (t + 1 < n && ts_cmp(tm[t], tl[t], tn[t], tm[t + 1], tl[t + 1], tn[t + 1]) >= 0) unsorted = 1;
         }
         __syncthreads();
         const bool bad = tid < tcnt && ko[tid + 1] < ko[tid];
         if (bad) errs |= ERR_KEY_OFF;
-        else if (tid < tcnt) ornk |= ko[tid + 1] - ko[tid];
+        else if (tid < tcnt) {
+            ornk |= ko[tid + 1] - ko[tid];
+            if (bc) bckeys += ko[tid + 1] - ko[tid];
+        }
         if (!__syncthreads_or(bad ? 1 : 0) && P) {
             const uint32_t a = (uint32_t)min((size_t)ko[0], P), b = (uint32_t)min((size_t)ko[tcnt], P);
             for (uint32_t j = a + tid; j < b; j += BLOCK) {
@@ -233,15 +238,18 @@
             }
         }
     }
-    uint64_t *gs = g + 8 * (blockIdx.x % PREP_SLOTS);
+    uint64_t *gs = g + PREP_ROW * (blockIdx.x % PREP_SLOTS);
     uint64_t v[7] = { m0, m1, m2, km, errs, unsorted, ornk };
     block_or_n<7>(v, gs);
     __shared__ uint32_t s_nd;
-    if (tid == 0) s_nd = 0;
+    __shared__ unsigned long long s_bck;
+    if (tid == 0) { s_nd = 0; s_bck = 0; }
     __syncthreads();
     if (differs) atomicAdd(&s_nd, differs);
+    if (bckeys) atomicAdd(&s_bck, bckeys);
     __syncthreads();
     if (tid == 0 && s_nd) atomicAdd((unsigned long long *)&gs[7], (unsigned long long)s_nd);
+    if (tid == 0 && s_bck) atomicAdd((unsigned long long *)&gs[8], s_bck);
 }
 
 __global__ __launch_bounds__(BLOCK) void k_b_compact(uint32_t n, const uint32_t *__restrict__ bflag, const uint32_t *__restrict__ bidx,
@@ -463,40 +471,57 @@
     ctx->stat("keydeps.fast_dictionary", 0);
 }
 
-void prep_dictionary(acc_ctx *ctx, uint32_t n, size_t P, const uint64_t *tm, const uint64_t *tl, const int32_t *tn,
-                     const uint64_t *em, const uint64_t *el, const int32_t *en, const uint8_t *status,
-                     const uint32_t *key_off, const uint64_t *key_code, uint32_t *owner, uint64_t *g, Dictionary &out,
-                     bool defer_ties)
+void prep_batch(acc_ctx *ctx, uint32_t n, size_t P, const uint64_t *tm, const uint64_t *tl, const int32_t *tn,
+                const uint64_t *em, const uint64_t *el, const int32_t *en, const uint8_t *status, const uint32_t *key_off,
+                const uint64_t *key_code, uint32_t *owner, uint64_t *g, Dictionary &out)
 {
     hipStream_t st = ctx->stream;
-    static_assert(8 * PREP_SLOTS <= acc_ctx::PINNED_WORDS - acc_ctx::PINNED_SLOTS, "slot rows fit the pinned area");
-    static_assert(PREP_G_WORDS == 8 + 8 * PREP_SLOTS, "g and the prep slots share one buffer");
+    static_assert(PREP_ROW * PREP_SLOTS <= acc_ctx::PINNED_WORDS - acc_ctx::PINNED_SLOTS, "slot rows fit the pinned area");
+    static_assert(PREP_G_WORDS == 8 + PREP_ROW * PREP_SLOTS, "g and the prep slots share one buffer");
+    static_assert(PREP_ROW >= 9, "seven OR words and two sums per slot row");
     uint64_t *gslots = g + 8;
     ACC_HIP(hipMemsetAsync(g, 0, PREP_G_WORDS * sizeof(uint64_t), st));
     uint32_t *bflag = ctx->get<uint32_t>("bflag", n);
     launch(ctx, "prep_txn", k_prep_txn, dim3(grid_for(n, BLOCK)), dim3(BLOCK), 0, n, P, tm, tl, tn, em, el, en, status,
            key_off, key_code, owner, bflag, gslots);
-    uint64_t hg[8] = { 0, 0, 0, 0, 0, 0, 0, 0 };
+    uint64_t hg[8] = { 0, 0, 0, 0, 0, 0, 0, 0 }, nbc = 0;
     {
         uint64_t *hs = ctx->pinned + acc_ctx::PINNED_SLOTS;
-        ACC_HIP(hipMemcpyAsync(hs, gslots, 8 * PREP_SLOTS * sizeof(uint64_t), hipMemcpyDeviceToHost, st));
+        ACC_HIP(hipMemcpyAsync(hs, gslots, PREP_ROW * PREP_SLOTS * sizeof(uint64_t), hipMemcpyDeviceToHost, st));
         ctx->sync();
         for (uint32_t r = 0; r < PREP_SLOTS; ++r) {
-            for (int w = 0; w < 7; ++w) hg[w] |= hs[8 * r + w];
-            hg[7] += hs[8 * r + 7];
+            for (int w = 0; w < 7; ++w) hg[w] |= hs[PREP_ROW * r + w];
+            hg[7] += hs[PREP_ROW * r + 7];
+            nbc += hs[PREP_ROW * r + 8];
         }
     }
     check_errors(hg[4]);
-    const bool batch_sorted = hg[5] == 0;
-
     const TsPlan plan = ts_plan(hg);
     const size_t m = 2 * (size_t)n;
-    uint32_t *rank = ctx->get<uint32_t>("rank", m);
-    uint32_t *txn_of_rank = ctx->get<uint32_t>("txn_of_rank", m);
-    const uint64_t nb = hg[7];
-    bool fast_dict = batch_sorted && plan.b0 + plan.b1 + plan.b2 <= 64 && nb < n;
+    out.rank = ctx->get<uint32_t>("rank", m);
+    out.txn_of_rank = ctx->get<uint32_t>("txn_of_rank", m);
+    out.rbits = bits_for(m - 1);
+    out.batch_sorted = hg[5] == 0;
+    out.fast_ok = out.batch_sorted && plan.b0 + plan.b1 + plan.b2 <= 64 && hg[7] < n;
+    out.fast = false;
+    out.ties_pending = false;
+    out.nbc = nbc;
+    out.nb = 0;
+    out.sb_vals = out.bsrc = nullptr;
+    memcpy(out.hg, hg, sizeof hg);
+}
+
+void build_dictionary(acc_ctx *ctx, uint32_t n, const uint64_t *tm, const uint64_t *tl, const int32_t *tn,
+                      const uint64_t *em, const uint64_t *el, const int32_t *en, uint64_t *g, Dictionary &out, bool defer_ties)
+{
+    const TsPlan plan = ts_plan(out.hg);
+    uint32_t *rank = out.rank, *txn_of_rank = out.txn_of_rank;
+    const uint64_t nb = out.hg[7];
+    bool fast_dict = out.fast_ok;
+    if (ctx->launch_stream && !(fast_dict && defer_ties)) fail(ACC_E_STATE, "internal: this dictionary syncs the context stream");
     out.ties_pending = false;
     if (fast_dict) {
+        const uint32_t *bflag = ctx->get<uint32_t>("bflag", n);
         uint32_t *bidx = ctx->get<uint32_t>("bidx", (size_t)n + 1);
         scan<uint32_t, OpAdd<uint32_t>>(ctx, bflag, bidx, n, true, bidx + n);
         uint64_t *bkey = ctx->get<uint64_t>("bkey", nb);
@@ -509,9 +534,13 @@
                (const uint64_t *)tkey, (const uint64_t *)sb.keys, (const uint32_t *)bflag, rank, txn_of_rank, g);
         launch(ctx, "rank_b_sorted", k_rank_b_sorted, dim3(grid_for(nb, BLOCK)), dim3(BLOCK), 0, n, (uint32_t)nb,
                (const uint64_t *)tkey, (const uint64_t *)sb.keys, (const uint32_t *)sb.vals, (const uint32_t *)bsrc, rank, g);
+        out.nb = (uint32_t)nb;
+        out.sb_vals = sb.vals;
+        out.bsrc = bsrc;
         if (defer_ties) {
             out.ties_pending = true;
         } else {
+            hipStream_t st = ctx->stream;
             ACC_HIP(hipMemcpyAsync(ctx->pinned, g + 6, sizeof(uint64_t), hipMemcpyDeviceToHost, st));
             ctx->sync();
             if (ctx->pinned[0]) {
@@ -522,12 +551,16 @@
     }
     if (!fast_dict) general_ranks(ctx, n, tm, tl, tn, em, el, en, plan, g, rank, txn_of_rank);
     ctx->stat("keydeps.fast_dictionary", fast_dict ? 1 : 0);
-    out.rank = rank;
-    out.txn_of_rank = txn_of_rank;
-    out.rbits = bits_for(m - 1);
-    out.batch_sorted = batch_sorted;
     out.fast = fast_dict;
-    memcpy(out.hg, hg, sizeof hg);
-}
-
-}
+}
+
+void prep_dictionary(acc_ctx *ctx, uint32_t n, size_t P, const uint64_t *tm, const uint64_t *tl, const int32_t *tn,
+                     const uint64_t *em, const uint64_t *el, const int32_t *en, const uint8_t *status,
+                     const uint32_t *key_off, const uint64_t *key_code, uint32_t *owner, uint64_t *g, Dictionary &out,
+                     bool defer_ties)
+{
+    prep_batch(ctx, n, P, tm, tl, tn, em, el, en, status, key_off, key_code, owner, g, out);
+    build_dictionary(ctx, n, tm, tl, tn, em, el, en, g, out, defer_ties);
+}
+
+}
diff --git a/cassandra-accord_amd/csrc/keydeps.hip b/cassandra-accord_amd/csrc/keydeps.hip
--- a/cassandra-accord_amd/csrc/keydeps.hip
+++ b/cassandra-accord_amd/csrc/keydeps.hip
@@ -90,10 +90,6 @@
 constexpr int NRD = 8;
 __device__ __forceinline__ bool cnt_is_max(int q) { return q == 7; }
 
-__device__ __forceinline__ uint32_t kind_class(uint32_t kind)
-{
-    return kind == 0 ? 0u : kind == 1 ? 1u : (kind == 3 || kind == 4) ? 2u : 3u;
-}
 __device__ __forceinline__ uint32_t wk_classes(uint32_t wk)
 {
     return (wk & 1u) | (((wk >> 1) & 1u) << 1) | (((wk >> 3) & 1u) << 2);
@@ -350,7 +346,7 @@
             o.bc_exec[b] = e;
             o.bc_kind[b] = (uint8_t)(s_info[p] >> 3);
             o.bc_pm_in[b] = ((uint64_t)seg << 32) | ((uint64_t)e + 1);
-            o.bc_key[b] = ((uint64_t)seg << rbits) | e;
+            if (o.bc_key) o.bc_key[b] = ((uint64_t)seg << rbits) | e;
         }
         if ((code[i] >> 4) & 1u) run[7] = (uint32_t)p + 1;
         if (p == P - 1 && P % RD_W == 0) {
@@ -371,6 +367,52 @@
     if (i >= nbc) return;
     bcs_exec[i] = (uint32_t)(skeys[i] & rmask);
     lastw_in[i] = bc_kind[svals[i]] == 1 ? i + 1 : 0;
+}
+
+
+__global__ __launch_bounds__(BLOCK) void k_bcx_counts(uint32_t nb, const uint32_t *__restrict__ sperm, const uint32_t *__restrict__ bsrc,
+                                                      const uint8_t *__restrict__ status, const uint64_t *__restrict__ tl,
+                                                      const uint32_t *__restrict__ key_off, uint32_t *__restrict__ bt,
+                                                      uint32_t *__restrict__ cnt)
+{
+    const uint32_t k = blockIdx.x * BLOCK + threadIdx.x;
+    if (k >= nb) return;
+    const uint32_t t = bsrc[sperm[k]];
+    bt[k] = t;
+    cnt[k] = bumped_committed(status[t], (uint32_t)(tl[t] >> 1) & 7u, true) ? key_off[t + 1] - key_off[t] : 0u;
+}
+
+__global__ __launch_bounds__(BLOCK) void k_bcx_expand(uint32_t nb, uint32_t n, const uint32_t *__restrict__ bt, const uint32_t *__restrict__ off,
+                                                      const uint32_t *__restrict__ key_off, const uint64_t *__restrict__ key_code,
+                                                      const uint32_t *__restrict__ rank, const uint64_t *__restrict__ tl, Runs rk,
+                                                      int rbits, uint64_t nout, uint64_t *__restrict__ out)
+{
+    __shared__ uint32_t so[BLOCK + 1], st[BLOCK];
+    const uint32_t tid = threadIdx.x, k0 = blockIdx.x * BLOCK;
+    if (k0 >= nb) return;
+    const uint32_t cnt = min((uint32_t)BLOCK, nb - k0);
+    if (tid < cnt) { so[tid] = off[k0 + tid]; st[tid] = bt[k0 + tid]; }
+    if (tid == 0) so[cnt] = off[k0 + cnt];
+    __syncthreads();
+    const uint64_t hi = min((uint64_t)so[cnt], nout);
+    for (uint64_t j = (uint64_t)so[0] + tid; j < hi; j += BLOCK) {
+        uint32_t lo = 0, up = cnt;
+        while (up - lo > 1) { const uint32_t m = (lo + up) >> 1; if (so[m] <= j) lo = m; else up = m; }
+        const uint32_t t = st[lo];
+        const uint64_t kc = pext_runs(key_code[key_off[t] + (uint32_t)(j - so[lo])], rk);
+        const uint64_t w = ((uint32_t)(tl[t] >> 1) & 7u) == 1u ? 1u : 0u;
+        out[j] = (kc << (rbits + 1)) | ((uint64_t)rank[n + t] << 1) | w;
+    }
+}
+
+__global__ __launch_bounds__(BLOCK) void k_bcx_cols(uint32_t nbc, const uint64_t *__restrict__ skeys, uint64_t rmask,
+                                                    uint32_t *__restrict__ bcs_exec, uint64_t *__restrict__ lastw_in)
+{
+    const uint32_t i = blockIdx.x * BLOCK + threadIdx.x;
+    if (i >= nbc) return;
+    const uint64_t x = skeys[i];
+    bcs_exec[i] = (uint32_t)((x >> 1) & rmask);
+    lastw_in[i] = (x & 1u) ? i + 1 : 0;
 }
 
 __device__ __forceinline__ uint32_t rd_cbc(const uint4 *rdir, uint32_t p);
@@ -2165,6 +2207,42 @@
 }
 
 
+static bool pair_plan(CfkBuild &cb)
+{
+    PairPlan &pp = cb.pp;
+    pp.rk = make_runs(cb.dict.hg[3]);
+    pp.rbits = cb.dict.rbits;
+    pp.sb = std::max(1, bits_for(cb.dict.hg[6]));
+    return cb.dict.batch_sorted && pp.rk.bits <= 32;
+}
+
+static void bc_from_txns(acc_ctx *ctx, CfkBuild &cb)
+{
+    const uint32_t n = cb.n, nb = cb.dict.nb;
+    const uint64_t nbc = cb.dict.nbc;
+    const PairPlan &pp = cb.pp;
+    const int rbits = cb.dict.rbits;
+    uint32_t *bt = ctx->get<uint32_t>("bcx_txn", nb);
+    uint32_t *cnt = ctx->get<uint32_t>("bcx_cnt", nb);
+    uint32_t *off = ctx->get<uint32_t>("bcx_off", (size_t)nb + 1);
+    uint64_t *keys = ctx->get<uint64_t>("bcx_key", nbc);
+    cb.bcs_exec = ctx->get<uint32_t>("v2_bcs_exec", nbc);
+    uint64_t *lw_in = ctx->get<uint64_t>("v2_bcs_lw_in64", nbc);
+    cb.bcs_lastw64 = ctx->get<uint64_t>("v2_bcs_lastw64", nbc);
+    cb.bc_side = true;
+    if (nbc == 0) return;
+    ctx->stat("keydeps.bc_sort_passes", (uint64_t)((pp.rk.bits + 7) / 8));
+    launch(ctx, "bcx_counts", k_bcx_counts, dim3(grid_for(nb, BLOCK)), dim3(BLOCK), 0, nb, cb.dict.sb_vals, cb.dict.bsrc, cb.status,
+           cb.tl, cb.key_off, bt, cnt);
+    scan<uint32_t, OpAdd<uint32_t>>(ctx, cnt, off, nb, true, off + nb);
+    launch(ctx, "bcx_expand", k_bcx_expand, dim3(grid_for(nb, BLOCK)), dim3(BLOCK), 0, nb, n, (const uint32_t *)bt,
+           (const uint32_t *)off, cb.key_off, cb.key_code, (const uint32_t *)cb.dict.rank, cb.tl, pp.rk, rbits, nbc, keys);
+    const uint64_t *sk = radix_sort_keys(ctx, "rs_bcx", keys, nbc, rbits + 1, pp.rk.bits);
+    launch(ctx, "bcx_cols", k_bcx_cols, dim3(grid_for(nbc, BLOCK)), dim3(BLOCK), 0, (uint32_t)nbc, sk,
+           (uint64_t)((1ull << rbits) - 1), cb.bcs_exec, lw_in);
+    scan<uint64_t, OpMax<uint64_t>>(ctx, lw_in, cb.bcs_lastw64, nbc, false);
+}
+
 struct PairSort {
     Sorted ps{ nullptr, nullptr };
     const uint64_t *sp_m4 = nullptr;
@@ -2174,7 +2252,7 @@
     bool tinfo_done = false;
 };
 
-static PairSort sort_pairs(acc_ctx *ctx, CfkBuild &cb)
+static PairSort sort_pairs(acc_ctx *ctx, CfkBuild &cb, bool keys_only)
 {
     const uint32_t n = cb.n;
     const size_t P = cb.P;
@@ -2183,9 +2261,6 @@
     const uint32_t *owner = cb.owner, *rank = cb.dict.rank;
     const int rbits = cb.dict.rbits;
     PairPlan &pp = cb.pp;
-    pp.rk = make_runs(cb.dict.hg[3]);
-    pp.rbits = rbits;
-    pp.sb = std::max(1, bits_for(cb.dict.hg[6]));
     uint64_t *pkey = ctx->get<uint64_t>("pair_key", P);
     const unsigned gP = grid_for(P, BLOCK);
     PairSort s;
@@ -2194,10 +2269,10 @@
         const bool m4 = bits_for((uint64_t)n - 1) + pp.sb <= 32;
         pp.mode = m4 ? 4 : 3;
         TxnInfoArgs ti;
-        ti.n = n; ti.status = cb.status; ti.tl = cb.tl; ti.tinfo = cb.tinfo; ti.bigflag = cb.bigflag;
+        if (!keys_only) { ti.n = n; ti.status = cb.status; ti.tl = cb.tl; ti.tinfo = cb.tinfo; ti.bigflag = cb.bigflag; }
         launch(ctx, "pair_keys", k_pair_keys, dim3(grid_for(std::max<size_t>(P, n), BLOCK)), dim3(BLOCK), 0, P, key_code,
                owner, key_off, rank, (const uint32_t *)nullptr, pp, 0, pkey, ti);
-        s.tinfo_done = true;
+        s.tinfo_done = !keys_only;
         const uint64_t *sp = radix_sort_keys(ctx, "rs_pair", pkey, P, 32, pp.rk.bits);
         uint32_t *perm = ctx->get<uint32_t>("pair_perm", P + V2_ITEMS);
         if (m4) s.sp_m4 = sp;
@@ -2228,7 +2303,7 @@
     return s;
 }
 
-static void build_columns(acc_ctx *ctx, CfkBuild &cb, const PairSort &s, bool tinfo_done)
+static void build_columns(acc_ctx *ctx, CfkBuild &cb, const PairSort &s, bool tinfo_done, bool lane_open)
 {
     const uint32_t n = cb.n;
     const size_t P = cb.P;
@@ -2242,6 +2317,7 @@
     uint32_t *totals = ctx->get<uint32_t>("v2_totals", 16);
     uint64_t rk_mask = 0;
     for (int r = 0; r < pp.rk.n; ++r) rk_mask |= (pp.rk.len[r] >= 64 ? ~0ull : ((1ull << pp.rk.len[r]) - 1)) << pp.rk.lo[r];
+    if (lane_open) ctx->lane_wait();
     if (!tinfo_done)
         launch(ctx, "txn_info", k_txn_info, dim3(grid_for(n, BLOCK)), dim3(BLOCK), 0, n, rank, cb.status, cb.tl, cb.key_off,
                cb.tinfo, cb.bigflag);
@@ -2305,12 +2381,23 @@
 
     cb.g = ctx->get<uint64_t>("g", PREP_G_WORDS);
     cb.owner = ctx->get<uint32_t>("owner", P);
-    prep_dictionary(ctx, n, P, cb.tm, cb.tl, cb.tn, cb.em, cb.el, cb.en, cb.status, cb.key_off, cb.key_code, cb.owner, cb.g,
-                    cb.dict, true);
+    prep_batch(ctx, n, P, cb.tm, cb.tl, cb.tn, cb.em, cb.el, cb.en, cb.status, cb.key_off, cb.key_code, cb.owner, cb.g, cb.dict);
+    const bool overlap = pair_plan(cb) && cb.dict.fast_ok && cb.pp.rk.bits + cb.dict.rbits + 1 <= 64;
+    ctx->stat("keydeps.build_overlap", overlap ? 1 : 0);
+    ctx->stat("keydeps.bc_sort_passes", 0);
+    if (overlap) ctx->lane_fork();
+    else build_dictionary(ctx, n, cb.tm, cb.tl, cb.tn, cb.em, cb.el, cb.en, cb.g, cb.dict, true);
 
     cb.tinfo = ctx->get<uint4>("tinfo", n);
     cb.bigflag = ctx->get<uint32_t>("v3_bigflag", n);
-    const PairSort ps = sort_pairs(ctx, cb);
+    const PairSort ps = sort_pairs(ctx, cb, overlap);
+    if (overlap) {
+        ctx->launch_stream = ctx->aux[0];
+        build_dictionary(ctx, n, cb.tm, cb.tl, cb.tn, cb.em, cb.el, cb.en, cb.g, cb.dict, true);
+        ctx->lane_mark();
+        bc_from_txns(ctx, cb);
+        ctx->launch_stream = nullptr;
+    }
     cb.perm = ps.ps.vals;
     if (!ps.flags_done)
         launch(ctx, "seg_flags", k_seg_flags, dim3(grid_for(P, BLOCK)), dim3(BLOCK), 0, P, (const uint64_t *)ps.ps.keys,
@@ -2331,19 +2418,27 @@
     cb.cols.bc_exec = ctx->get<uint32_t>("v2_bc_exec", P);
     cb.cols.bc_kind = ctx->get<uint8_t>("v2_bc_kind", P);
     cb.cols.bc_pm_in = ctx->get<uint64_t>("v2_bc_pm_in", P);
-    cb.cols.bc_key = ctx->get<uint64_t>("v2_bc_key", P);
+    cb.cols.bc_key = cb.bc_side ? nullptr : ctx->get<uint64_t>("v2_bc_key", P);
     cb.tot = ctx->get<uint64_t>("v3_tot", 4);
     cb.gstat = ctx->get<uint64_t>("v2_gstat", GSTAT_N + 6);
-    build_columns(ctx, cb, ps, ps.tinfo_done);
+    build_columns(ctx, cb, ps, ps.tinfo_done, overlap);
     if (cb.dict.ties_pending && ctx->pinned[6]) {
         check_errors(ctx->pinned[4]);
+        ctx->lane_join();
         redo_general_dictionary(ctx, n, cb.tm, cb.tl, cb.tn, cb.em, cb.el, cb.en, cb.g, cb.dict);
-        build_columns(ctx, cb, ps, false);
+        if (cb.bc_side) {
+            cb.bc_side = false;
+            cb.cols.bc_key = ctx->get<uint64_t>("v2_bc_key", P);
+            ctx->stat("keydeps.bc_sort_passes", 0);
+        }
+        build_columns(ctx, cb, ps, false, false);
     }
     cb.dict.ties_pending = false;
     memcpy(cb.htot, ctx->pinned, sizeof cb.htot);
     check_errors(ctx->pinned[4]);
     cb.ties = ctx->pinned[6] != 0;
+    if (cb.bc_side && !cb.ties && (uint64_t)cb.htot[6] != cb.dict.nbc)
+        fail(ACC_E_STATE, "internal: bumped committed count of the prep pass differs from the columns'");
     ctx->stat("keydeps.path_replay", cb.ties || (ctx->flags & ACC_OPT_FORCE_REPLAY) ? 1 : 0);
     ctx->stat("keydeps.exec_ties", cb.ties ? 1 : 0);
     ctx->stat("keydeps.batch_sorted", cb.dict.batch_sorted ? 1 : 0);
@@ -2408,14 +2503,23 @@
     uint32_t *const bigflag = cb.bigflag;
     uint64_t *const tot = cb.tot, *const gstat = cb.gstat;
     const uint32_t nbc = cb.htot[6];
-    if (segbits + rbits > 64) fail(ACC_E_ARG, "batch too large for the (segment, executeAt) composite key");
-    Sorted bcs = radix_sort(ctx, "rs_bc", cols.bc_key, nullptr, nbc, segbits + rbits);
-    uint32_t *bcs_exec = ctx->get<uint32_t>("v2_bcs_exec", nbc);
-    uint64_t *bcs_lw_in = ctx->get<uint64_t>("v2_bcs_lw_in64", nbc), *bcs_lw64 = ctx->get<uint64_t>("v2_bcs_lastw64", nbc);
-    launch(ctx, "v2_bcs_cols", k_v2_bcs_cols, dim3(grid_for(nbc, BLOCK)), dim3(BLOCK), 0, nbc, (const uint64_t *)bcs.keys,
-           (const uint32_t *)bcs.vals, (const uint8_t *)cols.bc_kind, (uint64_t)((1ull << rbits) - 1), bcs_exec, bcs_lw_in);
+    uint32_t *bcs_exec = cb.bcs_exec;
+    uint64_t *bcs_lw64 = cb.bcs_lastw64;
     uint64_t *bc_pm64 = ctx->get<uint64_t>("v2_bc_pm64", nbc);
-    {
+    if (cb.bc_side) {
+        ctx->lane_join();
+        scan<uint64_t, OpMax<uint64_t>>(ctx, cols.bc_pm_in, bc_pm64, nbc, false);
+    } else {
+        ctx->lane_join();
+        if (segbits + rbits > 64) fail(ACC_E_ARG, "batch too large for the (segment, executeAt) composite key");
+        if (!cols.bc_key) fail(ACC_E_STATE, "internal: no bumped committed sort keys");
+        Sorted bcs = radix_sort(ctx, "rs_bc", cols.bc_key, nullptr, nbc, segbits + rbits);
+        ctx->stat("keydeps.bc_sort_passes", nbc ? (uint64_t)((segbits + rbits + 7) / 8) : 0);
+        bcs_exec = ctx->get<uint32_t>("v2_bcs_exec", nbc);
+        uint64_t *bcs_lw_in = ctx->get<uint64_t>("v2_bcs_lw_in64", nbc);
+        bcs_lw64 = ctx->get<uint64_t>("v2_bcs_lastw64", nbc);
+        launch(ctx, "v2_bcs_cols", k_v2_bcs_cols, dim3(grid_for(nbc, BLOCK)), dim3(BLOCK), 0, nbc, (const uint64_t *)bcs.keys,
+               (const uint32_t *)bcs.vals, (const uint8_t *)cols.bc_kind, (uint64_t)((1ull << rbits) - 1), bcs_exec, bcs_lw_in);
         const uint64_t *si[2] = { bcs_lw_in, cols.bc_pm_in };
         uint64_t *so[2] = { bcs_lw64, bc_pm64 };
         const size_t sn[2] = { nbc, nbc };
@@ -2673,6 +2777,7 @@
     if (!cb.cfk) {
         *view = ctx->kd_view;
     } else if (cb.ties || (ctx->flags & ACC_OPT_FORCE_REPLAY)) {
+        ctx->lane_join();
         need_pair_pos(ctx, cb);
         keydeps_replay(ctx, cb, view);
     } else {
@@ -2700,6 +2805,7 @@
     CfkOpts opts;
     opts.seg_keys = true;
     CfkBuild cb = build_cfk(ctx, in, opts);
+    ctx->lane_join();
     ctx->kd_valid = false;
     if (cb.cfk) cb.nseg = cfk_nseg(ctx, cb);
     return cb;
diff --git a/cassandra-accord_amd/csrc/keydeps.hpp b/cassandra-accord_amd/csrc/keydeps.hpp
--- a/cassandra-accord_amd/csrc/keydeps.hpp
+++ b/cassandra-accord_amd/csrc/keydeps.hpp
@@ -184,6 +184,9 @@
     uint4 *tinfo = nullptr;
     uint32_t *bigflag = nullptr;
     uint32_t htot[16] = {};
+    bool bc_side = false;
+    uint32_t *bcs_exec = nullptr;
+    uint64_t *bcs_lastw64 = nullptr;
     V2Cols cols{};
     uint32_t *bases = nullptr;
     uint64_t *tot = nullptr;
diff --git a/cassandra-accord_amd/csrc/prims.hpp b/cassandra-accord_amd/csrc/prims.hpp
--- a/cassandra-accord_amd/csrc/prims.hpp
+++ b/cassandra-accord_amd/csrc/prims.hpp
@@ -321,7 +321,7 @@
     int m = 0;
     for (int i = 0; i < k; ++i) {
         if (n[i] == 0) {
-            if (total_out && total_out[i]) ACC_HIP(hipMemsetAsync(total_out[i], 0, sizeof(T), ctx->stream));
+            if (total_out && total_out[i]) ACC_HIP(hipMemsetAsync(total_out[i], 0, sizeof(T), ctx->cur()));
             continue;
         }
         a.in[m] = in[i]; a.out[m] = out[i]; a.total[m] = total_out ? total_out[i] : nullptr; a.n[m] = n[i];
@@ -333,27 +333,30 @@
     if (m == 0) return;
     a.k = m;
     for (int i = m; i <= SCAN_MAXA; ++i) a.cum[i] = (uint32_t)nb;
-    if (ctx->launch_stream) fail(ACC_E_STATE, "internal: scan launched on a side stream");
+    const int lane = ctx->scan_lane();
+    if (lane < 0) fail(ACC_E_STATE, "internal: scan launched on a side stream other than the side lane");
+    acc_ctx::ScanState &ss = ctx->scan_st[lane];
+    const char *const bn[2] = { lane ? "scan_lane_status0" : "scan_status0", lane ? "scan_lane_status1" : "scan_status1" };
     const size_t need = nb + 1;
     uint64_t *buf[2];
-    if (need > ctx->scan_cap) {
+    if (need > ss.cap) {
         for (int i = 0; i < 2; ++i) {
-            buf[i] = ctx->get_raw<uint64_t>(i ? "scan_status1" : "scan_status0", need);
-            ACC_HIP(hipMemsetAsync(buf[i], 0, need * sizeof(uint64_t), ctx->stream));
-        }
-        ctx->scan_cap = need;
-        ctx->scan_dirty[0] = ctx->scan_dirty[1] = 0;
+            buf[i] = ctx->get_raw<uint64_t>(bn[i], need);
+            ACC_HIP(hipMemsetAsync(buf[i], 0, need * sizeof(uint64_t), ctx->cur()));
+        }
+        ss.cap = need;
+        ss.dirty[0] = ss.dirty[1] = 0;
     } else {
-        for (int i = 0; i < 2; ++i) buf[i] = ctx->get_raw<uint64_t>(i ? "scan_status1" : "scan_status0", need);
-    }
-    const int p = ctx->scan_par;
+        for (int i = 0; i < 2; ++i) buf[i] = ctx->get_raw<uint64_t>(bn[i], need);
+    }
+    const int p = ss.par;
     uint64_t *status = buf[p];
     uint32_t *ticket = reinterpret_cast<uint32_t *>(status + nb);
     launch(ctx, "scan", k_scan_1p<T, Op, ITEMS>, dim3((unsigned)nb), dim3(BLOCK), 0, a, (int)exclusive, ticket, status,
-           buf[p ^ 1], (uint32_t)ctx->scan_dirty[p ^ 1]);
-    ctx->scan_dirty[p] = need;
-    ctx->scan_dirty[p ^ 1] = 0;
-    ctx->scan_par = p ^ 1;
+           buf[p ^ 1], (uint32_t)ss.dirty[p ^ 1]);
+    ss.dirty[p] = need;
+    ss.dirty[p ^ 1] = 0;
+    ss.par = p ^ 1;
 }
 
 template <class T, class Op>
@@ -375,7 +378,7 @@
 
 inline void sum_u32(acc_ctx *ctx, const uint32_t *in, size_t n, uint64_t *out)
 {
-    ACC_HIP(hipMemsetAsync(out, 0, 8, ctx->stream));
+    ACC_HIP(hipMemsetAsync(out, 0, 8, ctx->cur()));
     if (n) launch(ctx, "sum_u32", k_sum_u32, dim3((unsigned)std::min<size_t>(1024, (n + BLOCK - 1) / BLOCK)), dim3(BLOCK), 0,
                   in, n, out);
 }
@@ -748,7 +751,7 @@
 };
 static inline OsWords os_words(acc_ctx *ctx, const char *tag, size_t words)
 {
-    if (ctx->launch_stream) fail(ACC_E_STATE, "internal: radix sort launched on a side stream");
+    if (ctx->scan_lane() < 0) fail(ACC_E_STATE, "internal: radix sort launched on a side stream other than the side lane");
     if (words >= 0xFFFFFFFFull) fail(ACC_E_CAP, "internal: radix sort status beyond 2^32 words");
     acc_ctx::OsState &s = ctx->os_state[ctx->ns + tag];
     char n0[56], n1[56];
@@ -756,7 +759,7 @@
     snprintf(n1, sizeof n1, "%s_os1", tag);
     uint32_t *b[2] = { ctx->get<uint32_t>(n0, std::max(words, s.cap)), ctx->get<uint32_t>(n1, std::max(words, s.cap)) };
     if (words > s.cap) {
-        for (int i = 0; i < 2; ++i) ACC_HIP(hipMemsetAsync(b[i], 0, words * sizeof(uint32_t), ctx->stream));
+        for (int i = 0; i < 2; ++i) ACC_HIP(hipMemsetAsync(b[i], 0, words * sizeof(uint32_t), ctx->cur()));
         s.cap = words;
         s.dirty[0] = s.dirty[1] = 0;
     }
@@ -776,8 +779,8 @@
     int passes = (bits + 7) / 8;
     if (n == 0) return { k[0], v[0] };
     if (passes == 0) {
-        ACC_HIP(hipMemcpyAsync(k[0], keys, n * sizeof(uint64_t), hipMemcpyDeviceToDevice, ctx->stream));
-        if (vals) ACC_HIP(hipMemcpyAsync(v[0], vals, n * sizeof(uint32_t), hipMemcpyDeviceToDevice, ctx->stream));
+        ACC_HIP(hipMemcpyAsync(k[0], keys, n * sizeof(uint64_t), hipMemcpyDeviceToDevice, ctx->cur()));
+        if (vals) ACC_HIP(hipMemcpyAsync(v[0], vals, n * sizeof(uint32_t), hipMemcpyDeviceToDevice, ctx->cur()));
         else launch(ctx, "iota", k_iota, dim3(grid_for(n, BLOCK)), dim3(BLOCK), 0, v[0], n);
         return { k[0], v[0] };
     }
diff --git a/cassandra-accord_amd/csrc/ts.hpp b/cassandra-accord_amd/csrc/ts.hpp
--- a/cassandra-accord_amd/csrc/ts.hpp
+++ b/cassandra-accord_amd/csrc/ts.hpp
@@ -29,4 +29,14 @@
     }
 }
 
+__device__ __forceinline__ uint32_t kind_class(uint32_t kind)
+{
+    return kind == 0 ? 0u : kind == 1 ? 1u : (kind == 3 || kind == 4) ? 2u : 3u;
 }
+
+__device__ __forceinline__ bool bumped_committed(uint32_t status, uint32_t kind, bool bumped)
+{
+    return bumped && status >= 4 && status <= 6 && kind_class(kind) < 3;
+}
+
+}
```

New measurement: 3.536 billion txn-key pairs/s, median of 6. +7.9%, better.
